# BoloniniD/CSWin-UNet

Measured on AMD Instinct MI355X. Metric: training images/sec (224x224, cswin_tiny), higher is better.
Workload: dtype f32; 1 GPU; cswin_tiny_224_lite, synthetic 224x224 9-class, bs=24/GPU, fp32 matmul, fwd + 0.4CE+0.6Dice + bwd + SGD(momentum) step, drop_path 0.2; global_batch=24, img_size=224, parallelism=dp1, hip_graph=True

## Files before the change

cswin_unet_amd/_lib.py:

```python
import ctypes
import os
from ctypes import c_char_p, c_double, c_float, c_int, c_long, c_size_t, c_void_p

import torch

_HERE = os.path.dirname(os.path.abspath(__file__))
LIB_PATH = os.path.join(_HERE, "libcswin_hip.so")

P, I, F, SZ, L, D = c_void_p, c_int, c_float, c_size_t, c_long, c_double

ABI_VERSION = 4

SIGNATURES = {
    "cswin_last_error": (c_char_p, []),
    "cswin_abi_version": (I, []),
    "cswin_device_ok": (I, []),
    "cswin_attn_fwd": (I, [P, P, P, P, P, P, I, I, I, I, P, P, I, F, F, ctypes.c_ulonglong, P, I, P]),
    "cswin_attn_bwd_workspace": (SZ, [I, I, I, I, P, P, I]),
    "cswin_attn_bwd": (I, [P, P, P, P, P, P, P, P, P, P, SZ, I, I, I, I, P, P, I, F, P, F, ctypes.c_ulonglong, P, I, P]),
    "cswin_img2windows": (I, [P, P, I, I, I, I, I, I, P]),
    "cswin_windows2img": (I, [P, P, I, I, I, I, I, I, P]),
    "cswin_layernorm_fwd": (I, [P, P, P, P, P, P, I, I, F, I, P]),
    "cswin_layernorm_bwd_workspace": (SZ, [I, I]),
    "cswin_layernorm_bwd": (I, [P, P, P, P, P, P, P, P, P, P, SZ, I, I, P, P, P]),
    "cswin_linear_fwd": (I, [P, P, I, P, P, P, P, P, P, I, I, I, I, I, I, P]),
    "cswin_linear_bwd_data": (I, [P, P, P, P, I, P, P, I, P, I, I, I, I, I, P]),
    "cswin_linear_bwd_weight_workspace": (SZ, [I, I, I]),
    "cswin_linear_bwd_weight": (I, [P, P, P, I, P, I, P, P, P, SZ, I, I, I, P, I, P]),
    "cswin_linear_bwd_weight_batch": (I, [P, I, P, P, I, P]),
    "cswin_linear_bwd_tail": (I, [P, P, P, I, I, I, P, I, P, P, I, P]),
    "cswin_rows_sum_multi": (I, [P, I, P]),
    "cswin_conv_tok_fwd": (I, [P, P, P, P, I, I, I, I, I, I, I, I, I, P]),
    "cswin_conv_tok_bwd_data": (I, [P, P, P, I, I, I, I, I, I, I, I, I, P]),
    "cswin_conv_tok_bwd_weight_workspace": (SZ, [I, I, I, I, I, I, I, I]),
    "cswin_conv_tok_bwd_weight": (I, [P, P, P, P, P, SZ, I, I, I, I, I, I, I, I, I, P, I, P]),
    "cswin_conv_weight_permute": (I, [P, P, P, I, I, I, I, P]),
    "cswin_conv_weight_unpermute": (I, [P, P, I, I, I, I, P]),
    "cswin_conv_weight_flipT": (I, [P, P, I, I, I, P]),
    "cswin_nchw_to_tokens": (I, [P, P, I, I, I, I, I, P]),
    "cswin_tokens_to_nchw": (I, [P, P, I, I, I, I, I, P]),
    "cswin_carafe_fwd": (I, [P, P, P, P, P, I, I, I, I, I, P]),
    "cswin_carafe_bwd_workspace": (SZ, [I, I, I, I, I]),
    "cswin_carafe_bwd": (I, [P, P, P, P, P, P, P, SZ, I, I, I, I, I, P, P]),
    "cswin_loss_workspace": (SZ, [I, I, L]),
    "cswin_loss_sums": (I, [P, P, P, P, SZ, I, I, L, I, P]),
    "cswin_loss_finalize": (I, [P, P, P, D, I, F, F, P, P]),
    "cswin_loss_bwd": (I, [P, P, P, P, P, F, F, I, I, L, I, P]),
    "cswin_dropout": (I, [P, P, P, P, L, L, F, ctypes.c_ulonglong, P, P]),
    "cswin_sgd_flat": (I, [P, P, P, L, P, F, F, F, P, P]),
    "cswin_multi_copy": (I, [P, I, P]),
    "cswin_pack_bf16": (I, [P, P, L, P]),
    "cswin_pack_bf16_scaled": (I, [P, P, L, F, P]),
    "cswin_unpack_bf16": (I, [P, P, L, P]),
}



class WgradDesc(ctypes.Structure):
    _fields_ = [("dy", c_void_p), ("x", c_void_p), ("row_scale", c_void_p), ("dw", c_void_p), ("dbias", c_void_p),
                ("workspace", c_void_p), ("ws_bytes", c_size_t), ("rows_per_sample", c_int), ("M", c_int), ("N", c_int),
                ("K", c_int), ("precision", c_int), ("io_bf16", c_int)]


class ReduceJob(ctypes.Structure):
    _fields_ = [("part", c_void_p), ("out", c_void_p), ("out2", c_void_p), ("n_first", ctypes.c_longlong),
                ("n", ctypes.c_longlong), ("stride", ctypes.c_longlong), ("rows", c_int), ("reserved", c_int),
                ("conv_kk", c_int), ("conv_cin", c_int)]


_lib = None

PREC_FP32, PREC_BF16 = 0, 1
_state = {"precision": PREC_FP32, "act_bf16": True}


def precision():
    return _state["precision"]


def act_bf16():
    return _state["precision"] == PREC_BF16 and _state["act_bf16"]


def set_act_bf16(on):
    prev = _state["act_bf16"]
    _state["act_bf16"] = bool(on)
    return prev


_shadows = []


class _Shadow:

    def __init__(self, owner_obj, owner, seen):
        import weakref
        self.ref = weakref.ref(owner_obj)
        self.base, self.nbytes, self.seen = owner.data_ptr(), owner.numel() * 4, seen


def register_shadow(owner_obj, owner):
    _shadows[:] = [e for e in _shadows if e.ref() is not None and e.base != owner.data_ptr()]
    _shadows.append(_Shadow(owner_obj, owner, {p.data_ptr(): p._version for p in owner_obj.params}))


def shadow_ptr(w):
    if not _shadows or w is None:
        return None
    a = w.data_ptr()
    for e in _shadows:
        if e.base <= a < e.base + e.nbytes:
            opt = e.ref()
            if opt is None:
                return None
            if e.seen.get(a) != w._version:
                opt.refresh_shadow()
                e.seen.clear()
                e.seen.update({p.data_ptr(): p._version for p in opt.params})
                e.seen[a] = w._version
            return c_void_p(opt.flat_param16.data_ptr() + (a - e.base) // 2)
    return None


def shadows_current(opt):
    if _state["precision"] != PREC_BF16:
        return
    for e in _shadows:
        if e.ref() is opt:
            if any(e.seen.get(p.data_ptr()) != p._version for p in opt.params):
                opt.refresh_shadow()
                e.seen.clear()
                e.seen.update({p.data_ptr(): p._version for p in opt.params})
            return


def set_precision(mode):
    prev = _state["precision"]
    _state["precision"] = int(mode)
    if int(mode) == PREC_BF16 and prev != PREC_BF16:
        for e in _shadows:
            opt = e.ref()
            if opt is not None:
                opt.refresh_shadow()
    return prev


class CswinHipError(RuntimeError):
    pass


def lib():
    global _lib
    if _lib is None:
        if not os.path.exists(LIB_PATH):
            raise CswinHipError(f"{LIB_PATH} not found: build it with `python -c 'import __graft_entry__ as g; g.build()'` "
                                f"(or `make -C cswin_unet_amd/csrc`). There is no fallback path.")
        handle = ctypes.CDLL(LIB_PATH)
        for name, (res, args) in SIGNATURES.items():
            try:
                fn = getattr(handle, name)
            except AttributeError as e:
                raise CswinHipError(f"{LIB_PATH} does not export {name}") from e
            fn.restype, fn.argtypes = res, args
        have = handle.cswin_abi_version()
        if have != ABI_VERSION:
            raise CswinHipError(f"{LIB_PATH} was built for C ABI version {have}, this package binds version {ABI_VERSION}: rebuild it "
                                f"(`make -C cswin_unet_amd/csrc`)")
        _lib = handle
    return _lib


def call(name, *args):
    h = lib()
    rc = getattr(h, name)(*args)
    if rc != 0:
        raise CswinHipError(f"{name} failed ({rc}): {h.cswin_last_error().decode()}")


def ptr(t):
    return None if t is None else c_void_p(t.data_ptr())


def stream():
    return c_void_p(torch.cuda.current_stream().cuda_stream)


def dev_f32(t, what="tensor"):
    if t is None:
        return None
    if not t.is_cuda:
        raise CswinHipError(f"{what} is on {t.device}: the cswin_unet_amd ops run on a HIP device only (no CPU fallback)")
    if t.dtype != torch.float32:
        raise CswinHipError(f"{what} has dtype {t.dtype}; the HIP path computes in fp32")
    return t if t.is_contiguous() else t.contiguous()
```

cswin_unet_amd/csrc/carafe.hip:

```cpp
#include "common.h"
#include <stdlib.h>

namespace {

__host__ __device__ inline int carafe_lpr(int Cz) {
    int l = 1;
    while (2 * l <= Cz / 4 && 2 * l <= 64) l *= 2;
    return l;
}

template <int S>
__global__ __launch_bounds__(256) void carafe_fwd_kernel(const float* __restrict__ e, const float* __restrict__ z,
                                                          const float* __restrict__ bias, float* __restrict__ out,
                                                          float* __restrict__ wt_save, int B, int H, int W, int Cz) {
    constexpr int S2 = S * S;
    const int lpr = carafe_lpr(Cz);
    const int groups = 256 / lpr;
    const int sub = threadIdx.x % lpr, grp = threadIdx.x / lpr;
    const long items = (long)B * H * W * S2;
    for (long it = (long)blockIdx.x * groups + grp; it < items; it += (long)gridDim.x * groups) {
        const int s = (int)(it % S2);
        const long pix = it / S2;
        const int w = (int)(pix % W);
        const int h = (int)((pix / W) % H);
        const int b = (int)(pix / ((long)W * H));
        float wt[9];
        float mx = -INFINITY;
#pragma unroll
        for (int k = 0; k < 9; ++k) {
            wt[k] = e[pix * (9 * S2) + k * S2 + s];
            mx = fmaxf(mx, wt[k]);
        }
        float sum = 0.f;
#pragma unroll
        for (int k = 0; k < 9; ++k) {
            wt[k] = __expf(wt[k] - mx);
            sum += wt[k];
        }
        const float inv = 1.0f / sum;
#pragma unroll
        for (int k = 0; k < 9; ++k) wt[k] *= inv;
        if (wt_save && sub == 0) {
#pragma unroll
            for (int k = 0; k < 9; ++k) wt_save[pix * (9 * S2) + k * S2 + s] = wt[k];
        }
        const int sy = s / S, sx = s - sy * S;
        const long orow = ((long)b * H * S + h * S + sy) * (W * S) + w * S + sx;
        for (int c = 4 * sub; c < Cz; c += 4 * lpr) {
            f32x4 acc = bias ? *reinterpret_cast<const f32x4*>(bias + c) : f32x4{0.f, 0.f, 0.f, 0.f};
#pragma unroll
            for (int k = 0; k < 9; ++k) {
                const int hh = h + k / 3 - 1, ww = w + k % 3 - 1;
                if ((unsigned)hh < (unsigned)H && (unsigned)ww < (unsigned)W)
                    acc += wt[k] * *reinterpret_cast<const f32x4*>(z + (((long)b * H + hh) * W + ww) * Cz + c);
            }
            *reinterpret_cast<f32x4*>(out + orow * Cz + c) = acc;
        }
    }
}

template <int S>
__global__ __launch_bounds__(256) void carafe_bwd_e_kernel(const float* __restrict__ dout, const float* __restrict__ z,
                                                            const float* __restrict__ wt_save, float* __restrict__ de,
                                                            float* __restrict__ dbias_part, int B, int H, int W, int Cz) {
    __shared__ float bred[2 * 1024];
    f32x4 bacc[2] = {{0.f, 0.f, 0.f, 0.f}, {0.f, 0.f, 0.f, 0.f}};
    constexpr int S2 = S * S;
    const int lpr = carafe_lpr(Cz);
    const int groups = 256 / lpr;
    const int sub = threadIdx.x % lpr, grp = threadIdx.x / lpr;
    const long items = (long)B * H * W * S2;
    const long items_pad = (items + groups - 1) / groups * groups;
    for (long it0 = (long)blockIdx.x * groups + grp; it0 < items_pad; it0 += (long)gridDim.x * groups) {
        const bool live = it0 < items;
        const long it = live ? it0 : items - 1;
        const int s = (int)(it % S2);
        const long pix = it / S2;
        const int w = (int)(pix % W);
        const int h = (int)((pix / W) % H);
        const int b = (int)(pix / ((long)W * H));
        const int sy = s / S, sx = s - sy * S;
        const long orow = ((long)b * H * S + h * S + sy) * (W * S) + w * S + sx;
        float dwt[9];
#pragma unroll
        for (int k = 0; k < 9; ++k) dwt[k] = 0.f;
        int ci = 0;
        for (int c = 4 * sub; c < Cz; c += 4 * lpr, ++ci) {
            const f32x4 g = *reinterpret_cast<const f32x4*>(dout + orow * Cz + c);
            if (live && dbias_part) {
                if (ci == 0) bacc[0] += g;
                else bacc[1] += g;
            }
#pragma unroll
            for (int k = 0; k < 9; ++k) {
                const int hh = h + k / 3 - 1, ww = w + k % 3 - 1;
                if ((unsigned)hh < (unsigned)H && (unsigned)ww < (unsigned)W) {
                    const f32x4 zv = *reinterpret_cast<const f32x4*>(z + (((long)b * H + hh) * W + ww) * Cz + c);
                    dwt[k] += g[0] * zv[0] + g[1] * zv[1] + g[2] * zv[2] + g[3] * zv[3];
                }
            }
        }
#pragma unroll
        for (int k = 0; k < 9; ++k)
            for (int o = lpr >> 1; o > 0; o >>= 1) dwt[k] += __shfl_xor(dwt[k], o, 64);
        if (sub == 0 && live) {
            float wt[9], dot = 0.f;
#pragma unroll
            for (int k = 0; k < 9; ++k) {
                wt[k] = wt_save[pix * (9 * S2) + k * S2 + s];
                dot += wt[k] * dwt[k];
            }
#pragma unroll
            for (int k = 0; k < 9; ++k) de[pix * (9 * S2) + k * S2 + s] = wt[k] * (dwt[k] - dot);
        }
    }
    if (dbias_part) {
        const int span = 4 * lpr;
#pragma unroll
        for (int q = 0; q < 2; ++q)
#pragma unroll
            for (int e = 0; e < 4; ++e) bred[(q * groups + grp) * span + 4 * sub + e] = bacc[q][e];
        __syncthreads();
        for (int c = threadIdx.x; c < Cz; c += 256) {
            const int q = c / span, cc = c - q * span;
            float t = 0.f;
            for (int g2 = 0; g2 < groups; ++g2) t += bred[(q * groups + g2) * span + cc];
            dbias_part[(long)blockIdx.x * Cz + c] = t;
        }
    }
}

template <int S>
__global__ __launch_bounds__(256) void carafe_bwd_z_kernel(const float* __restrict__ dout,
                                                            const float* __restrict__ wt_save, float* __restrict__ dz,
                                                            int B, int H, int W, int Cz) {
    constexpr int S2 = S * S;
    const int lpr = carafe_lpr(Cz);
    const int groups = 256 / lpr;
    const int sub = threadIdx.x % lpr, grp = threadIdx.x / lpr;
    const long items = (long)B * H * W;
    for (long pix = (long)blockIdx.x * groups + grp; pix < items; pix += (long)gridDim.x * groups) {
        const int w = (int)(pix % W);
        const int h = (int)((pix / W) % H);
        const int b = (int)(pix / ((long)W * H));
        for (int c = 4 * sub; c < Cz; c += 4 * lpr) {
            f32x4 acc = {0.f, 0.f, 0.f, 0.f};
#pragma unroll
            for (int k = 0; k < 9; ++k) {
                const int h2 = h - (k / 3 - 1), w2 = w - (k % 3 - 1);
                if ((unsigned)h2 < (unsigned)H && (unsigned)w2 < (unsigned)W) {
                    const long p2 = ((long)b * H + h2) * W + w2;
#pragma unroll
                    for (int s = 0; s < S2; ++s) {
                        const float wv = wt_save[p2 * (9 * S2) + k * S2 + s];
                        const long orow = ((long)b * H * S + h2 * S + s / S) * (W * S) + w2 * S + s % S;
                        acc += wv * *reinterpret_cast<const f32x4*>(dout + orow * Cz + c);
                    }
                }
            }
            *reinterpret_cast<f32x4*>(dz + pix * Cz + c) = acc;
        }
    }
}

constexpr int C4_T = 8;
constexpr int C4_HALO = C4_T + 2;
constexpr int C4_NP = C4_HALO * C4_HALO;

__device__ __forceinline__ f32x4 carafe_mfma4(float a, float b, f32x4 c) { return __builtin_amdgcn_mfma_f32_16x16x4f32(a, b, c, 0, 0, 0); }

constexpr int C4_WAVES = 8;

__global__ __launch_bounds__(64 * C4_WAVES) void carafe4_bwd_fused_kernel(const float* __restrict__ dout, const float* __restrict__ z,
                                                                 const float* __restrict__ wt_save, float* __restrict__ de,
                                                                 float* __restrict__ dz, float* __restrict__ dbias_part,
                                                                 int B, int H, int W, int tiles_x, int tiles_y) {
    constexpr int S = 4, S2 = 16, Cz = 16;
    __shared__ __attribute__((aligned(16))) float Gs[C4_NP * 9 * Cz];
    __shared__ __attribute__((aligned(16))) float zt[C4_NP * Cz];
    __shared__ float bred[C4_WAVES][Cz];
    const int tid = threadIdx.x, lane = tid & 63, wave = tid >> 6;
    const int li = lane & 15, kq = lane >> 4;
    int t = blockIdx.x;
    const int tx = t % tiles_x; t /= tiles_x;
    const int ty = t % tiles_y;
    const int b = t / tiles_y;
    const int h0 = ty * C4_T - 1, w0 = tx * C4_T - 1;

    for (int i = tid; i < C4_NP * (Cz / 4); i += 64 * C4_WAVES) {
        const int pl = i >> 2, c4 = i & 3;
        const int h = h0 + pl / C4_HALO, w = w0 + pl % C4_HALO;
        f32x4 v = {0.f, 0.f, 0.f, 0.f};
        if ((unsigned)h < (unsigned)H && (unsigned)w < (unsigned)W)
            v = *reinterpret_cast<const f32x4*>(z + (((long)b * H + h) * W + w) * Cz + 4 * c4);
        *reinterpret_cast<f32x4*>(&zt[pl * Cz + 4 * c4]) = v;
    }
    __syncthreads();

    float bsum = 0.f;
    constexpr int PB = 4;
    for (int pl0 = wave * PB; pl0 < C4_NP; pl0 += C4_WAVES * PB) {
        bool inside[PB], interior[PB];
        long pix[PB];
        float av[PB][4], dv[PB][4], wv[PB][4];
        f32x4 db[PB];
#pragma unroll
        for (int u = 0; u < PB; ++u) {
            const int pl = pl0 + u;
            const int ph = pl / C4_HALO, pw = pl - ph * C4_HALO;
            const int h = h0 + ph, w = w0 + pw;
            inside[u] = pl < C4_NP && (unsigned)h < (unsigned)H && (unsigned)w < (unsigned)W;
            interior[u] = inside[u] && ph >= 1 && ph <= C4_T && pw >= 1 && pw <= C4_T;
            pix[u] = ((long)b * H + h) * W + w;
            db[u] = f32x4{0.f, 0.f, 0.f, 0.f};
#pragma unroll
            for (int j = 0; j < 4; ++j) av[u][j] = dv[u][j] = wv[u][j] = 0.f;
            if (!inside[u]) continue;
            const float* wp = wt_save + pix[u] * (9 * S2);
            const float* drow = dout + (((long)b * H * S + h * S) * (W * S) + w * S) * Cz;
            const long hstride = (long)W * S * Cz;
#pragma unroll
            for (int j = 0; j < 4; ++j) {
                if (li < 9) av[u][j] = wp[li * S2 + 4 * j + kq];
                dv[u][j] = drow[j * hstride + kq * Cz + li];
            }
            if (interior[u]) {
                db[u] = *reinterpret_cast<const f32x4*>(drow + (li >> 2) * hstride + (li & 3) * Cz + 4 * kq);
#pragma unroll
                for (int r = 0; r < 4; ++r)
                    if (4 * kq + r < 9) wv[u][r] = wp[(4 * kq + r) * S2 + li];
            }
        }
#pragma unroll
        for (int u = 0; u < PB; ++u) {
            const int pl = pl0 + u;
            if (pl >= C4_NP) continue;
            float* Gp = &Gs[pl * 9 * Cz];
            if (!inside[u]) {
                for (int i = lane; i < 9 * Cz; i += 64) Gp[i] = 0.f;
                continue;
            }
            f32x4 g = {0.f, 0.f, 0.f, 0.f};
#pragma unroll
            for (int j = 0; j < 4; ++j) g = carafe_mfma4(av[u][j], dv[u][j], g);
#pragma unroll
            for (int r = 0; r < 4; ++r)
                if (4 * kq + r < 9) Gp[(4 * kq + r) * Cz + li] = g[r];
            if (!interior[u]) continue;
            bsum += dv[u][0] + dv[u][1] + dv[u][2] + dv[u][3];
            const int ph = pl / C4_HALO, pw = pl - ph * C4_HALO;
            f32x4 za = {0.f, 0.f, 0.f, 0.f};
            if (li < 9) {
                const int nh = ph + li / 3 - 1, nw = pw + li % 3 - 1;
                za = *reinterpret_cast<const f32x4*>(&zt[(nh * C4_HALO + nw) * Cz + 4 * kq]);
            }
            f32x4 dw = {0.f, 0.f, 0.f, 0.f};
#pragma unroll
            for (int j = 0; j < 4; ++j) dw = carafe_mfma4(za[j], db[u][j], dw);
            float dot = 0.f;
#pragma unroll
            for (int r = 0; r < 4; ++r) dot += wv[u][r] * dw[r];
            dot += __shfl_xor(dot, 16, 64);
            dot += __shfl_xor(dot, 32, 64);
            float* dep = de + pix[u] * (9 * S2);
#pragma unroll
            for (int r = 0; r < 4; ++r)
                if (4 * kq + r < 9) dep[(4 * kq + r) * S2 + li] = wv[u][r] * (dw[r] - dot);
        }
    }
    bsum += __shfl_xor(bsum, 16, 64);
    bsum += __shfl_xor(bsum, 32, 64);
    if (lane < Cz) bred[wave][lane] = bsum;
    __syncthreads();
    if (tid < Cz && dbias_part) {
        float t2 = 0.f;
#pragma unroll
        for (int k = 0; k < C4_WAVES; ++k) t2 += bred[k][tid];
        dbias_part[(long)blockIdx.x * Cz + tid] = t2;
    }

    if (tid < 256) {
        const int n = tid >> 2, c4 = tid & 3;
        const int ph = 1 + n / C4_T, pw = 1 + n % C4_T;
        const int h = h0 + ph, w = w0 + pw;
        if (h < H && w < W) {
            f32x4 acc = {0.f, 0.f, 0.f, 0.f};
#pragma unroll
            for (int k = 0; k < 9; ++k) {
                const int sh = ph - (k / 3 - 1), sw = pw - (k % 3 - 1);
                acc += *reinterpret_cast<const f32x4*>(&Gs[((sh * C4_HALO + sw) * 9 + k) * Cz + 4 * c4]);
            }
            *reinterpret_cast<f32x4*>(dz + (((long)b * H + h) * W + w) * Cz + 4 * c4) = acc;
        }
    }
}

__global__ __launch_bounds__(256) void colsum_partial_kernel(const float* __restrict__ x, float* __restrict__ partial,
                                                              long rows, int C) {
    __shared__ float red[256];
    const int lanes = min(C, 256);
    const int rgroups = 256 / lanes;
    const int c0 = threadIdx.x % lanes, rg = threadIdx.x / lanes;
    for (int c = c0; c < C; c += lanes) {
        float s = 0.f;
        if (rg < rgroups)
            for (long r = (long)blockIdx.x * rgroups + rg; r < rows; r += (long)gridDim.x * rgroups) s += x[r * C + c];
        red[threadIdx.x] = s;
        __syncthreads();
        if (rg == 0) {
            float t = 0.f;
            for (int k = 0; k < rgroups; ++k) t += red[k * lanes + c0];
            partial[(long)blockIdx.x * C + c] = t;
        }
        __syncthreads();
    }
}

int colsum_blocks(long rows, int C) {
    int lanes = C < 256 ? C : 256;
    int rg = 256 / lanes;
    long b = (rows + rg * 64 - 1) / (rg * 64);
    return (int)(b < 1 ? 1 : (b > 512 ? 512 : b));
}

int grid_for(long items, int groups) {
    long b = (items + groups - 1) / groups;
    return (int)(b < 1 ? 1 : (b > 8192 ? 8192 : b));
}

bool carafe_args_ok(int B, int H, int W, int Cz, int S) {
    if (B <= 0 || H <= 0 || W <= 0 || Cz <= 0 || (S != 2 && S != 4)) return false;
    return Cz % 4 == 0 && Cz >= 4;
}

}

extern "C" {

int cswin_carafe_fwd(const float* e, const float* z, const float* bias, float* out, float* wt_save, int B, int H, int W,
                     int Cz, int S, void* stream) {
    CSWIN_REQUIRE(e && z && out, CSWIN_ERR_SHAPE, "carafe_fwd: null pointer");
    CSWIN_REQUIRE(carafe_args_ok(B, H, W, Cz, S), CSWIN_ERR_UNSUPPORTED, "carafe_fwd: unsupported shape B=%d H=%d W=%d Cz=%d S=%d (Cz %% 4 == 0, S in {2,4})", B, H, W, Cz, S);
    const int groups = 256 / carafe_lpr(Cz);
    hipStream_t st = (hipStream_t)stream;
    const long items = (long)B * H * W * S * S;
    if (S == 2) hipLaunchKernelGGL(carafe_fwd_kernel<2>, dim3(grid_for(items, groups)), dim3(256), 0, st, e, z, bias, out, wt_save, B, H, W, Cz);
    else hipLaunchKernelGGL(carafe_fwd_kernel<4>, dim3(grid_for(items, groups)), dim3(256), 0, st, e, z, bias, out, wt_save, B, H, W, Cz);
    CSWIN_LAUNCH_CHECK();
    return CSWIN_OK;
}

static bool carafe4_fused_ok(int H, int W, int Cz, int S) { return S == 4 && Cz == 16 && H % C4_T == 0 && W % C4_T == 0; }

size_t cswin_carafe_bwd_workspace(int B, int H, int W, int Cz, int S) {
    size_t generic = (size_t)colsum_blocks((long)B * H * W * S * S, Cz) * Cz * sizeof(float);
    size_t in_e = Cz <= 512 ? (size_t)grid_for((long)B * H * W * S * S, 256 / carafe_lpr(Cz)) * Cz * sizeof(float) : 0;
    if (in_e > generic) generic = in_e;
    size_t fused = carafe4_fused_ok(H, W, Cz, S) ? (size_t)B * (H / C4_T) * (W / C4_T) * Cz * sizeof(float) : 0;
    return generic > fused ? generic : fused;
}

int cswin_carafe_bwd(const float* dout, const float* z, const float* wt_save, float* de, float* dz, float* dbias,
                     void* workspace, size_t ws_bytes, int B, int H, int W, int Cz, int S, cswin_reduce_job* deferred, void* stream) {
    if (deferred) *deferred = cswin_reduce_job{};
    CSWIN_REQUIRE(dout && z && wt_save && de && dz, CSWIN_ERR_SHAPE, "carafe_bwd: null pointer");
    CSWIN_REQUIRE(carafe_args_ok(B, H, W, Cz, S), CSWIN_ERR_UNSUPPORTED, "carafe_bwd: unsupported shape");
    CSWIN_REQUIRE(!dbias || (workspace && ws_bytes >= cswin_carafe_bwd_workspace(B, H, W, Cz, S)), CSWIN_ERR_WORKSPACE, "carafe_bwd: workspace too small");
    const int groups = 256 / carafe_lpr(Cz);
    hipStream_t st = (hipStream_t)stream;
    const long items = (long)B * H * W * S * S, pixels = (long)B * H * W;
    const bool no_fused = cswin_tuning().carafe_generic != 0;
    if (carafe4_fused_ok(H, W, Cz, S) && !no_fused) {
        const int tx = W / C4_T, ty = H / C4_T, nblk = B * tx * ty;
        hipLaunchKernelGGL(carafe4_bwd_fused_kernel, dim3(nblk), dim3(64 * C4_WAVES), 0, st, dout, z, wt_save, de, dz,
                           dbias ? (float*)workspace : nullptr, B, H, W, tx, ty);
        CSWIN_LAUNCH_CHECK();
        if (dbias) {
            reduce_now_or_defer(cswin_reduce_job{(const float*)workspace, dbias, nullptr, 0, Cz, Cz, nblk, 0, 0, 0}, deferred, st);
            CSWIN_LAUNCH_CHECK();
        }
        return CSWIN_OK;
    }
    const bool bias_in_e = dbias && Cz <= 512;
    float* bpart = bias_in_e ? (float*)workspace : nullptr;
    const int eblk = grid_for(items, groups);
    if (S == 2) {
        hipLaunchKernelGGL(carafe_bwd_e_kernel<2>, dim3(eblk), dim3(256), 0, st, dout, z, wt_save, de, bpart, B, H, W, Cz);
        hipLaunchKernelGGL(carafe_bwd_z_kernel<2>, dim3(grid_for(pixels, groups)), dim3(256), 0, st, dout, wt_save, dz, B, H, W, Cz);
    } else {
        hipLaunchKernelGGL(carafe_bwd_e_kernel<4>, dim3(eblk), dim3(256), 0, st, dout, z, wt_save, de, bpart, B, H, W, Cz);
        hipLaunchKernelGGL(carafe_bwd_z_kernel<4>, dim3(grid_for(pixels, groups)), dim3(256), 0, st, dout, wt_save, dz, B, H, W, Cz);
    }
    CSWIN_LAUNCH_CHECK();
    if (bias_in_e) {
        reduce_now_or_defer(cswin_reduce_job{(const float*)workspace, dbias, nullptr, 0, Cz, Cz, eblk, 0, 0, 0}, deferred, st);
        CSWIN_LAUNCH_CHECK();
    } else if (dbias) {
        int nblk = colsum_blocks(items, Cz);
        hipLaunchKernelGGL(colsum_partial_kernel, dim3(nblk), dim3(256), 0, st, dout, (float*)workspace, items, Cz);
        reduce_now_or_defer(cswin_reduce_job{(const float*)workspace, dbias, nullptr, 0, Cz, Cz, nblk, 0, 0, 0}, deferred, st);
        CSWIN_LAUNCH_CHECK();
    }
    return CSWIN_OK;
}

}
```

cswin_unet_amd/csrc/common.h:

```cpp
#pragma once
#include "tuning.h"
#include <hip/hip_runtime.h>
#include <stddef.h>
#include <stdint.h>
#include <stdio.h>

typedef float f32x4 __attribute__((ext_vector_type(4)));
typedef unsigned u32x2 __attribute__((ext_vector_type(2)));
typedef unsigned u32x4 __attribute__((ext_vector_type(4)));
typedef float f32x16 __attribute__((ext_vector_type(16)));

#define CSWIN_ABI_VERSION 4
#define CSWIN_OK 0
#define CSWIN_ERR_SHAPE (-1)
#define CSWIN_ERR_ALIGN (-2)
#define CSWIN_ERR_WORKSPACE (-3)
#define CSWIN_ERR_HIP (-4)
#define CSWIN_ERR_UNSUPPORTED (-5)

void cswin_set_error(const char* fmt, ...);

#define CSWIN_REQUIRE(cond, code, ...)          \
    do {                                        \
        if (!(cond)) {                          \
            cswin_set_error(__VA_ARGS__);       \
            return (code);                      \
        }                                       \
    } while (0)

#define CSWIN_LAUNCH_CHECK()                                                   \
    do {                                                                       \
        hipError_t e__ = hipGetLastError();                                    \
        if (e__ != hipSuccess) {                                               \
            cswin_set_error("%s:%d HIP launch error: %s", __FILE__, __LINE__,  \
                            hipGetErrorString(e__));                           \
            return CSWIN_ERR_HIP;                                              \
        }                                                                      \
    } while (0)

static inline int cdiv(long a, long b) { return (int)((a + b - 1) / b); }

__device__ __forceinline__ float wave_sum(float v) {
#pragma unroll
    for (int o = 32; o > 0; o >>= 1) v += __shfl_xor(v, o, 64);
    return v;
}
__device__ __forceinline__ float wave_max(float v) {
#pragma unroll
    for (int o = 32; o > 0; o >>= 1) v = fmaxf(v, __shfl_xor(v, o, 64));
    return v;
}

__device__ __forceinline__ void gelu_parts(float x, float& cdf, float& e) {
    const float u = fabsf(x) * 0.70710678118654752f;
    const float t = __builtin_amdgcn_rcpf(fmaf(0.3275911f, u, 1.0f));
    e = __expf(-u * u);
    const float poly = t * fmaf(t, fmaf(t, fmaf(t, fmaf(t, 1.061405429f, -1.453152027f), 1.421413741f), -0.284496736f), 0.254829592f);
    const float pe = poly * e;
    cdf = x < 0.f ? 0.5f * pe : fmaf(-0.5f, pe, 1.0f);
}
__device__ __forceinline__ float gelu_f(float x) {
    float cdf, e;
    gelu_parts(x, cdf, e);
    return x * cdf;
}
__device__ __forceinline__ float gelu_grad_f(float x) {
    float cdf, e;
    gelu_parts(x, cdf, e);
    return fmaf(x * 0.3989422804014327f, e, cdf);
}

extern "C" {
typedef struct cswin_reduce_job {
    const float* part;
    float* out;
    float* out2;
    long long n_first, n, stride;
    int rows, reserved;
    int conv_kk, conv_cin;
} cswin_reduce_job;
}

static inline int reduce_job_vec_ok(const cswin_reduce_job& j) {
    return ((uintptr_t)j.part % 16 == 0) && j.stride % 4 == 0 && j.n % 4 == 0 && (!j.out2 || j.n_first % 4 == 0);
}

constexpr int RS_COLS = 64, RS_G = 16;
__device__ __forceinline__ void rows_sum_block(const cswin_reduce_job& job, long blk, float (*red)[RS_COLS + 1]) {
    const int c4 = threadIdx.x & 15, g = threadIdx.x >> 4;
    const long i0 = blk * RS_COLS + 4 * c4;
    f32x4 s0 = {0.f, 0.f, 0.f, 0.f}, s1 = s0, s2 = s0, s3 = s0;
    if (i0 < job.n) {
        const float* base = job.part + i0;
        if (job.reserved & 1) {
            int r = g;
            for (; r + 3 * RS_G < job.rows; r += 4 * RS_G) {
                s0 += *reinterpret_cast<const f32x4*>(base + (long)r * job.stride);
                s1 += *reinterpret_cast<const f32x4*>(base + (long)(r + RS_G) * job.stride);
                s2 += *reinterpret_cast<const f32x4*>(base + (long)(r + 2 * RS_G) * job.stride);
                s3 += *reinterpret_cast<const f32x4*>(base + (long)(r + 3 * RS_G) * job.stride);
            }
            for (; r < job.rows; r += RS_G) s0 += *reinterpret_cast<const f32x4*>(base + (long)r * job.stride);
        } else {
            for (int r = g; r < job.rows; r += RS_G)
#pragma unroll
                for (int e = 0; e < 4; ++e)
                    if (i0 + e < job.n) s0[e] += base[(long)r * job.stride + e];
        }
    }
    s0 = (s0 + s1) + (s2 + s3);
#pragma unroll
    for (int e = 0; e < 4; ++e) red[g][4 * c4 + e] = s0[e];
    __syncthreads();
    const long i = blk * RS_COLS + threadIdx.x;
    if (threadIdx.x < RS_COLS && i < job.n) {
        float t = 0.f;
#pragma unroll
        for (int k = 0; k < RS_G; ++k) t += red[k][threadIdx.x];
        if (job.out2 && i >= job.n_first) job.out2[i - job.n_first] = t;
        else job.out[i] = t;
    }
}

__device__ __forceinline__ void rows_sum_conv_block(const cswin_reduce_job& j, long blk, float (*red)[RS_COLS + 1]) {
    const int kk = j.conv_kk, Cin = j.conv_cin;
    float* out = j.out;
    const int c4 = threadIdx.x & 15, g = threadIdx.x >> 4;
    const long i0 = blk * RS_COLS + 4 * c4;
    f32x4 s0 = {0.f, 0.f, 0.f, 0.f}, s1 = s0;
    if (i0 < j.n) {
        const float* base = j.part + i0;
        if (j.reserved & 1) {
            int r = g;
            for (; r + RS_G < j.rows; r += 2 * RS_G) {
                s0 += *reinterpret_cast<const f32x4*>(base + (long)r * j.stride);
                s1 += *reinterpret_cast<const f32x4*>(base + (long)(r + RS_G) * j.stride);
            }
            for (; r < j.rows; r += RS_G) s0 += *reinterpret_cast<const f32x4*>(base + (long)r * j.stride);
        } else {
            for (int r = g; r < j.rows; r += RS_G)
#pragma unroll
                for (int e = 0; e < 4; ++e)
                    if (i0 + e < j.n) s0[e] += base[(long)r * j.stride + e];
        }
    }
    s0 += s1;
#pragma unroll
    for (int e = 0; e < 4; ++e) red[g][4 * c4 + e] = s0[e];
    __syncthreads();
    const long i = blk * RS_COLS + threadIdx.x;
    if (threadIdx.x < RS_COLS && i < j.n) {
        float t = 0.f;
#pragma unroll
        for (int k = 0; k < RS_G; ++k) t += red[k][threadIdx.x];
        if (j.out2 && i >= j.n_first) j.out2[i - j.n_first] = t;
        else if (i < j.n_first) {
            const long co = i / ((long)kk * Cin);
            const int rem = (int)(i - co * kk * Cin), tap = rem / Cin, ci = rem - tap * Cin;
            out[(co * Cin + ci) * kk + tap] = t;
        }
    }
}

extern "C" {
typedef struct cswin_wgrad_desc {
    const float* dy;
    const float* x;
    const float* row_scale;
    float* dw;
    float* dbias;
    void* workspace;
    size_t ws_bytes;
    int rows_per_sample, M, N, K;
    int precision;
    int io_bf16;
} cswin_wgrad_desc;
}

constexpr int CSWIN_MAX_REDUCE_JOBS = 48;
struct ReduceJobs {
    cswin_reduce_job j[CSWIN_MAX_REDUCE_JOBS];
    int first_block[CSWIN_MAX_REDUCE_JOBS + 1];
    int njobs;
};

constexpr int RS_FEW_ROWS = 16, RS_FEW_COLS = 1024;
__device__ __forceinline__ void rows_sum_few(const cswin_reduce_job& job, long blk) {
    const long i0 = blk * RS_FEW_COLS + 4 * threadIdx.x;
    if (i0 >= job.n) return;
    const float* base = job.part + i0;
    f32x4 s0 = {0.f, 0.f, 0.f, 0.f}, s1 = s0;
    int r = 0;
    for (; r + 1 < job.rows; r += 2) {
        s0 += *reinterpret_cast<const f32x4*>(base + (long)r * job.stride);
        s1 += *reinterpret_cast<const f32x4*>(base + (long)(r + 1) * job.stride);
    }
    if (r < job.rows) s0 += *reinterpret_cast<const f32x4*>(base + (long)r * job.stride);
    s0 += s1;
    if (job.out2 && i0 >= job.n_first) *reinterpret_cast<f32x4*>(job.out2 + (i0 - job.n_first)) = s0;
    else *reinterpret_cast<f32x4*>(job.out + i0) = s0;
}
static inline int reduce_job_few_ok(const cswin_reduce_job& j) {
    return !j.conv_kk && reduce_job_vec_ok(j) && j.rows <= RS_FEW_ROWS && j.n >= 4 * RS_FEW_COLS && ((uintptr_t)j.out % 16 == 0) &&
           (!j.out2 || ((uintptr_t)j.out2 % 16 == 0));
}

static __global__ __launch_bounds__(256) void rows_sum_kernel(cswin_reduce_job job) {
    __shared__ float red[RS_G][RS_COLS + 1];
    if (job.conv_kk) rows_sum_conv_block(job, blockIdx.x, red);
    else if (job.reserved & 2) rows_sum_few(job, blockIdx.x);
    else rows_sum_block(job, blockIdx.x, red);
}

static inline void launch_rows_sum(const float* part, float* out, float* out2, long n_first, long n, int rows, long stride,
                                   hipStream_t st) {
    cswin_reduce_job job = {part, out, out2, n_first, n, stride, rows, 0, 0, 0};
    const int few = reduce_job_few_ok(job);
    job.reserved = reduce_job_vec_ok(job) | (few ? 2 : 0);
    const long cols = few ? RS_FEW_COLS : RS_COLS;
    hipLaunchKernelGGL(rows_sum_kernel, dim3((unsigned)((n + cols - 1) / cols)), dim3(256), 0, st, job);
}

__device__ __forceinline__ void rows_sum_dispatch(const cswin_reduce_job* j, const int* first_block, int njobs, int blk,
                                                  float (*red)[RS_COLS + 1]) {
    int lo = 0, hi = njobs - 1;
    while (lo < hi) {
        const int mid = (lo + hi + 1) >> 1;
        if (blk >= first_block[mid]) lo = mid;
        else hi = mid - 1;
    }
    const int k = lo;
    if (j[k].conv_kk) rows_sum_conv_block(j[k], blk - first_block[k], red);
    else if (j[k].reserved & 2) rows_sum_few(j[k], blk - first_block[k]);
    else rows_sum_block(j[k], blk - first_block[k], red);
}

static __global__ __launch_bounds__(256) void rows_sum_multi_kernel(ReduceJobs J) {
    __shared__ float red[RS_G][RS_COLS + 1];
    rows_sum_dispatch(J.j, J.first_block, J.njobs, (int)blockIdx.x, red);
}

constexpr int CSWIN_TAIL_RIDER_JOBS = 16;
struct ReduceRiders {
    cswin_reduce_job j[CSWIN_TAIL_RIDER_JOBS];
    int first_block[CSWIN_TAIL_RIDER_JOBS + 1];
    int njobs;
};
static inline int fill_reduce_table(const cswin_reduce_job* jobs, int njobs, cswin_reduce_job* out, int* first_block) {
    int blocks = 0;
    for (int i = 0; i < njobs; ++i) {
        if (!(jobs[i].part && jobs[i].out && jobs[i].n > 0 && jobs[i].rows > 0)) return -1;
        if ((jobs[i].conv_kk == 0) != (jobs[i].conv_cin == 0) || jobs[i].conv_kk < 0) return -1;
        out[i] = jobs[i];
        const int few = reduce_job_few_ok(jobs[i]);
        out[i].reserved = reduce_job_vec_ok(jobs[i]) | (few ? 2 : 0);
        first_block[i] = blocks;
        blocks += few ? (int)((jobs[i].n + RS_FEW_COLS - 1) / RS_FEW_COLS) : (int)((jobs[i].n + RS_COLS - 1) / RS_COLS);
    }
    first_block[njobs] = blocks;
    return blocks;
}

static inline void reduce_now_or_defer(const cswin_reduce_job& job, cswin_reduce_job* deferred, hipStream_t st) {
    if (deferred) *deferred = job;
    else launch_rows_sum(job.part, job.out, job.out2, (long)job.n_first, (long)job.n, job.rows, (long)job.stride, st);
}
```

cswin_unet_amd/csrc/gemm.hip:

```cpp
#include <stdlib.h>

#include <type_traits>
#include "common.h"
#include "gemm_epilogue.h"

int cswin_gemm16(int mode, int epi_mode, const void* A, const void* B, const void* epilogue, int M, int NO, int R, void* stream);
int cswin_wgrad16_batch(const cswin_wgrad_desc* d, int n, const int* splits, const int* rows_per_split, const cswin_reduce_job* pending,
                        int npending, void* stream, long long* stamps);

namespace {

constexpr int BKMAX = 64;

typedef __bf16 bf16x8 __attribute__((ext_vector_type(8)));
typedef __bf16 bf16x4 __attribute__((ext_vector_type(4)));

#define CSWIN_CHECK_PRECISION(p, who) CSWIN_REQUIRE((p) == 0 || (p) == 1, CSWIN_ERR_UNSUPPORTED, who ": precision %d (0 = fp32, 1 = bf16 operands)", (p))

struct PlainSrc {
    const float* p; long ld; int rows, cols;
    const float* row_scale; int rows_per_sample;
    int bf16;
    struct Row { const float* base; float s; };
    __device__ Row row(int i) const {
// ... 709 lines not shown
    choose_split(M, N, K, &s0, &rps);
    choose_split(M, N, K, &s1, &rps, 1024);
    return (size_t)(s0 > s1 ? s0 : s1) * ((size_t)N * K + N) * sizeof(float);
}

int cswin_linear_bwd_weight_batch(const cswin_wgrad_desc* d, int n, cswin_reduce_job* deferred, const cswin_reduce_job* pending, int npending,
                                  void* stream);
int cswin_rows_sum_multi(const cswin_reduce_job* jobs, int njobs, void* stream);
}
namespace {
struct TailExtras { const float* dy; const float* w; float* dx; int M, N, K; const cswin_reduce_job* jobs; int njobs; };
int wgrad_batch_impl(const cswin_wgrad_desc* d, int n, cswin_reduce_job* deferred, const TailExtras* extra, void* stream);
}
extern "C" {

int cswin_linear_bwd_weight(const float* dy, const float* x, const float* x2, int k_split, const float* row_scale,
                            int rows_per_sample, float* dw, float* dbias, void* workspace, size_t ws_bytes, int M,
                            int N, int K, cswin_reduce_job* deferred, int precision, void* stream) {
    CSWIN_CHECK_PRECISION(precision, "linear_bwd_weight");
    CSWIN_REQUIRE(dy && x && dw && M > 0 && N > 0 && K > 0, CSWIN_ERR_SHAPE, "linear_bwd_weight: bad arguments");
    CSWIN_REQUIRE(!x2 || (k_split > 0 && k_split < K), CSWIN_ERR_SHAPE, "linear_bwd_weight: bad concat split");
    CSWIN_REQUIRE(!row_scale || rows_per_sample > 0, CSWIN_ERR_SHAPE, "linear_bwd_weight: rows_per_sample must be > 0");
    size_t need = cswin_linear_bwd_weight_workspace(M, N, K);
    CSWIN_REQUIRE(workspace && ws_bytes >= need, CSWIN_ERR_WORKSPACE, "linear_bwd_weight: workspace %zu < %zu", ws_bytes, need);
    hipStream_t st = (hipStream_t)stream;
    if (precision == 1 && !x2 && N % 4 == 0 && K % 4 == 0 && aligned16(dy) && aligned16(x) && aligned16(workspace)) {
        cswin_wgrad_desc d1 = {dy, x, row_scale, dw, dbias, workspace, ws_bytes, rows_per_sample, M, N, K, 1, 0};
        cswin_reduce_job job;
        int rc = cswin_linear_bwd_weight_batch(&d1, 1, &job, nullptr, 0, stream);
        if (rc) return rc;
        reduce_now_or_defer(job, deferred, st);
        CSWIN_LAUNCH_CHECK();
        return CSWIN_OK;
    }
    int splits, rps;
    choose_split(M, N, K, &splits, &rps);
    float* slab = (float*)workspace;
    const long slab_stride = (long)N * K + N;
    Epilogue e = plain_epilogue(slab, K);
    e.split_stride = slab_stride;
    e.colsum = dbias ? slab + (long)N * K : nullptr;
    e.colsum_stride = (int)slab_stride;
    PlainSrc A = {dy, N, M, N, row_scale, rows_per_sample};
    if (x2) {
        ConcatSrc B = {x, x2, k_split, K - k_split, M, K, k_split};
        bool vec = (N % 4 == 0) && (K % 4 == 0) && (k_split % 4 == 0) && aligned16(dy) && aligned16(x) && aligned16(x2);
        if (vec) launch_gemm<false, false, 4, EPI_PLAIN, true>(A, B, e, N, K, M, splits, rps, precision, st);
        else launch_gemm<false, false, 1, EPI_PLAIN, true>(A, B, e, N, K, M, splits, rps, precision, st);
    } else {
        PlainSrc B = {x, K, M, K, nullptr, 1};
        bool vec = (N % 4 == 0) && (K % 4 == 0) && aligned16(dy) && aligned16(x);
        if (row_scale) {
            if (vec) launch_gemm<false, false, 4, EPI_PLAIN, true>(A, B, e, N, K, M, splits, rps, precision, st);
            else launch_gemm<false, false, 1, EPI_PLAIN, true>(A, B, e, N, K, M, splits, rps, precision, st);
        } else {
            if (vec) launch_gemm<false, false, 4, EPI_PLAIN, false>(A, B, e, N, K, M, splits, rps, precision, st);
            else launch_gemm<false, false, 1, EPI_PLAIN, false>(A, B, e, N, K, M, splits, rps, precision, st);
        }
    }
    CSWIN_LAUNCH_CHECK();
    long n = (long)N * K;
    cswin_reduce_job job = {slab, dw, dbias, n, n + (dbias ? N : 0), slab_stride, splits, 0};
    reduce_now_or_defer(job, deferred, st);
    CSWIN_LAUNCH_CHECK();
    return CSWIN_OK;
}

int cswin_linear_bwd_weight_batch(const cswin_wgrad_desc* d, int n, cswin_reduce_job* deferred, const cswin_reduce_job* pending, int npending,
                                  void* stream) {
    CSWIN_REQUIRE(npending >= 0 && npending <= CSWIN_TAIL_RIDER_JOBS && (npending == 0 || pending), CSWIN_ERR_SHAPE,
                  "linear_bwd_weight_batch: 0..%d pending reductions", CSWIN_TAIL_RIDER_JOBS);
    TailExtras r = {nullptr, nullptr, nullptr, 0, 0, 0, pending, npending};
    return wgrad_batch_impl(d, n, deferred, npending > 0 ? &r : nullptr, stream);
}

int cswin_linear_bwd_tail(const float* dy, const float* w, float* dx, int M, int N, int K, const cswin_wgrad_desc* d, int n,
                          cswin_reduce_job* deferred, const cswin_reduce_job* pending, int npending, void* stream) {
    CSWIN_REQUIRE(dy && w && dx && M > 0 && N > 0 && K > 0, CSWIN_ERR_SHAPE, "linear_bwd_tail: bad data-gradient arguments");
    CSWIN_REQUIRE(npending >= 0 && npending <= CSWIN_TAIL_RIDER_JOBS && (npending == 0 || pending), CSWIN_ERR_SHAPE,
                  "linear_bwd_tail: 0..%d pending reductions", CSWIN_TAIL_RIDER_JOBS);
    TailExtras r = {dy, w, dx, M, N, K, pending, npending};
    return wgrad_batch_impl(d, n, deferred, &r, stream);
}

}
namespace {
int wgrad_batch_impl(const cswin_wgrad_desc* d, int n, cswin_reduce_job* deferred, const TailExtras* extra, void* stream) {
    CSWIN_REQUIRE(d && deferred && n >= 1 && n <= WGRAD_BATCH, CSWIN_ERR_SHAPE, "linear_bwd_weight_batch: 1..%d problems and their deferred slots", WGRAD_BATCH);
    bool fast = true;
    const int precision = d[0].precision;
    CSWIN_CHECK_PRECISION(precision, "linear_bwd_weight_batch");
    for (int i = 0; i < n; ++i) {
        CSWIN_REQUIRE(d[i].precision == precision, CSWIN_ERR_UNSUPPORTED, "linear_bwd_weight_batch: problems of one launch share one precision");
        CSWIN_REQUIRE(d[i].io_bf16 == 0 || (precision == 1 && (d[i].io_bf16 & ~3) == 0), CSWIN_ERR_UNSUPPORTED, "linear_bwd_weight_batch: bf16 storage needs precision 1");
        CSWIN_REQUIRE(d[i].dy && d[i].x && d[i].dw && d[i].M > 0 && d[i].N > 0 && d[i].K > 0, CSWIN_ERR_SHAPE, "linear_bwd_weight_batch: bad problem %d", i);
        CSWIN_REQUIRE(!d[i].row_scale || d[i].rows_per_sample > 0, CSWIN_ERR_SHAPE, "linear_bwd_weight_batch: rows_per_sample must be > 0");
        size_t need = cswin_linear_bwd_weight_workspace(d[i].M, d[i].N, d[i].K);
        CSWIN_REQUIRE(d[i].workspace && d[i].ws_bytes >= need, CSWIN_ERR_WORKSPACE, "linear_bwd_weight_batch: workspace %zu < %zu", d[i].ws_bytes, need);
        fast = fast && d[i].N % 4 == 0 && d[i].K % 4 == 0 && aligned16(d[i].dy) && aligned16(d[i].x) && aligned16(d[i].workspace);
    }
    const bool has_dgrad = extra && extra->dy;
    const bool merge_on = cswin_tuning().gemm_tail_merge != 0;
    const bool ride = extra && merge_on && fast && precision == 0 &&
                      (!has_dgrad || (extra->N % 4 == 0 && extra->K % 4 == 0 && aligned16(extra->dy) && aligned16(extra->w) && aligned16(extra->dx)));
    const bool w16_path = fast && precision == 1 && (cswin_tuning().wgrad16_on || d[0].io_bf16 || (n > 1 && d[1].io_bf16) || (n > 2 && d[2].io_bf16) || (n > 3 && d[3].io_bf16));
    const bool jobs_ride16 = extra && merge_on && w16_path && extra->njobs > 0;
    if (extra && !ride) {
        if (has_dgrad) {
            int rc = cswin_linear_bwd_data(extra->dy, extra->w, extra->dx, nullptr, 0, nullptr, nullptr, 1, nullptr, extra->M, extra->N,
                                           extra->K, precision == 1 ? 1 : 0, 0, stream);
            if (rc) return rc;
        }
        if (extra->njobs > 0 && !jobs_ride16) {
            int rc = cswin_rows_sum_multi(extra->jobs, extra->njobs, stream);
            if (rc) return rc;
        }
    }
    if (!fast) {
        for (int i = 0; i < n; ++i) CSWIN_REQUIRE(d[i].io_bf16 == 0, CSWIN_ERR_ALIGN, "linear_bwd_weight_batch: bf16 storage needs N, K multiples of 4 and 16-B alignment");
        for (int i = 0; i < n; ++i) {
            int rc = cswin_linear_bwd_weight(d[i].dy, d[i].x, nullptr, 0, d[i].row_scale, d[i].rows_per_sample, d[i].dw, d[i].dbias,
                                             d[i].workspace, d[i].ws_bytes, d[i].M, d[i].N, d[i].K, &deferred[i], precision, stream);
            if (rc) return rc;
        }
        return CSWIN_OK;
    }
    if (w16_path) {
        int splits[WGRAD_BATCH], rps[WGRAD_BATCH];
        double work_total = 0.0;
        for (int i = 0; i < n; ++i) work_total += (double)d[i].M * cdiv(d[i].N, 128) * cdiv(d[i].K, 128);
        for (int i = 0; i < n; ++i) {
            const int M = d[i].M, N = d[i].N, K = d[i].K;
            const long slab = ((long)N * K + N) * (long)sizeof(float);
            const int tiles = cdiv(N, 128) * cdiv(K, 128);
            const int w16_wgs = cswin_tuning().w16_wgs, w16_even = cswin_tuning().w16_even;
            int s = w16_even ? (w16_wgs / n) / tiles : (int)(w16_wgs * ((double)M * tiles / work_total) / tiles + 0.5);
            const int cap = (int)(d[i].ws_bytes / slab);
            if (s > cap) s = cap;
            if (s > M / 64) s = M / 64;
            if (s < 1) s = 1;
            rps[i] = cdiv(cdiv(M, s), 32) * 32;
            splits[i] = cdiv(M, rps[i]);
            const long nk = (long)N * K;
            deferred[i] = cswin_reduce_job{(const float*)d[i].workspace, d[i].dw, d[i].dbias, nk, nk + (d[i].dbias ? N : 0), nk + N, splits[i], 0};
        }
        CSWIN_REQUIRE(cswin_wgrad16_batch(d, n, splits, rps, jobs_ride16 ? extra->jobs : nullptr, jobs_ride16 ? extra->njobs : 0, stream, g_stamps) == 0,
                      CSWIN_ERR_SHAPE, "linear_bwd_weight_batch: bad pending reduction");
        CSWIN_LAUNCH_CHECK();
        return CSWIN_OK;
    }
    WgradBatch b = {};
    int blocks = 0;
    for (int i = 0; i < n; ++i) {
        const int M = d[i].M, N = d[i].N, K = d[i].K;
        int splits, rps;
        const int batch_env = cswin_tuning().gemm_batch_wgs;
        const int batch_even = cswin_tuning().gemm_batch_even;
        const int total_wgs = batch_env > 0 ? (batch_env < 1024 ? batch_env : 1024) * n : 1024;
        int batch_target = total_wgs / n;
        if (!batch_even) {
            double work = 0.0;
            for (int j = 0; j < n; ++j) work += (double)d[j].M * cdiv(d[j].N, 64) * cdiv(d[j].K, 64);
            batch_target = (int)(total_wgs * ((double)M * cdiv(N, 64) * cdiv(K, 64) / work) + 0.5);
            if (batch_target > 1024) batch_target = 1024;
            if (batch_target < 1) batch_target = 1;
        }
        choose_split(M, N, K, &splits, &rps, batch_target);
        CSWIN_REQUIRE((size_t)splits * ((size_t)N * K + N) * sizeof(float) <= d[i].ws_bytes, CSWIN_ERR_WORKSPACE,
                      "linear_bwd_weight_batch: %d slabs do not fit problem %d's workspace", splits, i);
        float* slab = (float*)d[i].workspace;
        const long slab_stride = (long)N * K + N;
        Epilogue e = plain_epilogue(slab, K);
        e.split_stride = slab_stride;
        e.colsum = d[i].dbias ? slab + (long)N * K : nullptr;
        e.colsum_stride = (int)slab_stride;
        e.vec_store = epilogue_vec_ok(e, K);
        b.A[i] = PlainSrc{d[i].dy, N, M, N, d[i].row_scale, d[i].row_scale ? d[i].rows_per_sample : 1};
        b.B[i] = PlainSrc{d[i].x, K, M, K, nullptr, 1};
        b.e[i] = e;
        b.M[i] = N; b.N[i] = K; b.R[i] = M; b.rps[i] = rps;
        b.tm[i] = cdiv(N, 64); b.tn[i] = cdiv(K, 64);
        b.first[i] = blocks;
        blocks += b.tm[i] * b.tn[i] * splits;
        const long nk = (long)N * K;
        deferred[i] = cswin_reduce_job{slab, d[i].dw, d[i].dbias, nk, nk + (d[i].dbias ? N : 0), slab_stride, splits, 0};
    }
    b.first[n] = blocks;
    b.n = n;
    if (ride) {
        BlockTail t = {};
        if (has_dgrad) {
            Epilogue e = plain_epilogue(extra->dx, extra->K);
            e.vec_store = epilogue_vec_ok(e, extra->K);
            t.dA = PlainSrc{extra->dy, extra->N, extra->M, extra->N, nullptr, 1, 0};
            t.dB = PlainSrc{extra->w, extra->K, extra->N, extra->K, nullptr, 1, 0};
            t.de = e;
            t.dM = extra->M; t.dN = extra->K; t.dR = extra->N; t.drps = cdiv(extra->N, BKMAX) * BKMAX;
            t.dtm = cdiv(extra->M, 64); t.dtn = cdiv(extra->K, 64);
            t.nd = t.dtm * t.dtn;
        }
        t.w = b;
        int rblocks = 0;
        if (extra->njobs > 0) {
            rblocks = fill_reduce_table(extra->jobs, extra->njobs, t.r.j, t.r.first_block);
            CSWIN_REQUIRE(rblocks >= 0, CSWIN_ERR_SHAPE, "linear_bwd_tail: bad pending reduction");
            t.r.njobs = extra->njobs;
        }
        static_assert(sizeof(BlockTail) <= 4096, "kernel argument block");
        hipLaunchKernelGGL(gemm_block_tail_kernel, dim3(blocks + t.nd + rblocks), dim3(512), 0, (hipStream_t)stream, t);
    } else if (precision == 1) {
        hipLaunchKernelGGL(gemm_wgrad_batch_kernel<1>, dim3(blocks), dim3(512), 0, (hipStream_t)stream, b);
    } else {
        hipLaunchKernelGGL(gemm_wgrad_batch_kernel<0>, dim3(blocks), dim3(512), 0, (hipStream_t)stream, b);
    }
    CSWIN_LAUNCH_CHECK();
    return CSWIN_OK;
}
}
extern "C" {

int cswin_conv_tok_fwd(const float* x, const float* w_perm, const float* bias, float* y, int B, int H, int W, int Cin,
                       int Cout, int ks, int stride, int pad, int precision, void* stream) {
    CSWIN_CHECK_PRECISION(precision, "conv_tok_fwd");
    CSWIN_REQUIRE(x && w_perm && y && B > 0 && H > 0 && W > 0 && Cin > 0 && Cout > 0, CSWIN_ERR_SHAPE, "conv_tok_fwd: bad arguments");
    CSWIN_REQUIRE(Cin % 4 == 0 && aligned16(x) && aligned16(w_perm), CSWIN_ERR_ALIGN, "conv_tok_fwd: Cin %% 4 and 16-B alignment required");
    int OH = (H + 2 * pad - ks) / stride + 1, OW = (W + 2 * pad - ks) / stride + 1;
    int M = B * OH * OW, R = ks * ks * Cin;
    ConvSrc A = {x, B, H, W, Cin, OH, OW, ks, stride, pad, M, R};
    PlainSrc Bm = {w_perm, R, Cout, R, nullptr, 1};
    Epilogue e = plain_epilogue(y, Cout);
    e.bias = bias;
    launch_gemm<true, true, 4, EPI_PLAIN, false>(A, Bm, e, M, Cout, R, 1, cdiv(R, BKMAX) * BKMAX, precision, (hipStream_t)stream);
    CSWIN_LAUNCH_CHECK();
    return CSWIN_OK;
}

int cswin_conv_tok_bwd_data(const float* dy, const float* w_permT, float* dx, int B, int H, int W, int Cin, int Cout,
                            int ks, int stride, int pad, int precision, void* stream) {
    CSWIN_CHECK_PRECISION(precision, "conv_tok_bwd_data");
    CSWIN_REQUIRE(dy && w_permT && dx, CSWIN_ERR_SHAPE, "conv_tok_bwd_data: null pointer");
    CSWIN_REQUIRE(Cin % 4 == 0 && Cout % 4 == 0 && aligned16(dy) && aligned16(w_permT), CSWIN_ERR_ALIGN, "conv_tok_bwd_data: channels %% 4 and 16-B alignment required");
    int OH = (H + 2 * pad - ks) / stride + 1, OW = (W + 2 * pad - ks) / stride + 1;
    if (ks == 3 && stride == 2 && pad == 1) {
        GemmBatch<ConvTS2Src, TapRowsSrc> b = {};
        int blocks = 0, n = 0, rmax = 0;
        for (int py = 0; py < 2; ++py)
            for (int px = 0; px < 2; ++px) {
                const int H2 = (H - py + 1) / 2, W2 = (W - px + 1) / 2;
                if (H2 <= 0 || W2 <= 0) continue;
                int kys = 0, kxs = 0, taps = 0, nt = 0;
                for (int ky = (py ? 0 : 1); ky < 3; ky += 2)
                    for (int kx = (px ? 0 : 1); kx < 3; kx += 2) {
                        kys |= ky << (2 * nt);
                        kxs |= kx << (2 * nt);
                        taps |= (ky * 3 + kx) << (4 * nt);
                        ++nt;
                    }
                const int Mc = B * H2 * W2, Rc = nt * Cout;
                b.A[n] = ConvTS2Src{dy, B, H, W, Cout, OH, OW, py, px, H2, W2, kys, kxs, Mc, Rc};
                b.B[n] = TapRowsSrc{w_permT, Cout, Cin, taps, Rc, Cin};
                Epilogue e = plain_epilogue(dx, Cin);
                e.rm_on = 1; e.rm_H = H; e.rm_W = W; e.rm_H2 = H2; e.rm_W2 = W2; e.rm_py = py; e.rm_px = px;
                e.vec_store = epilogue_vec_ok(e, Cin);
                b.e[n] = e;
                b.M[n] = Mc; b.N[n] = Cin; b.R[n] = Rc; b.rps[n] = cdiv(Rc, BKMAX) * BKMAX;
                b.tm[n] = cdiv(Mc, 64); b.tn[n] = cdiv(Cin, 64);
                b.first[n] = blocks;
                blocks += b.tm[n] * b.tn[n];
                rmax = Rc > rmax ? Rc : rmax;
                ++n;
            }
        if (n > 0) {
            b.first[n] = blocks;
            b.n = n;
            hipStream_t st = (hipStream_t)stream;
            const int kw = (blocks < 320 && rmax >= 512) ? 4 : ((blocks < 640 && rmax >= 256) ? 2 : 1);
            if (precision == 1) {
                hipLaunchKernelGGL((gemm_conv_s2_dgrad_batch_kernel<2, 1>), dim3(blocks), dim3(512), 0, st, b);
            } else if (kw == 4) {
                hipLaunchKernelGGL((gemm_conv_s2_dgrad_batch_kernel<4, 0>), dim3(blocks), dim3(1024), 0, st, b);
            } else if (kw == 2) {
                hipLaunchKernelGGL((gemm_conv_s2_dgrad_batch_kernel<2, 0>), dim3(blocks), dim3(512), 0, st, b);
            } else {
                hipLaunchKernelGGL((gemm_conv_s2_dgrad_batch_kernel<1, 0>), dim3(blocks), dim3(256), 0, st, b);
            }
        }
        CSWIN_LAUNCH_CHECK();
        return CSWIN_OK;
    }
    int M = B * H * W, R = ks * ks * Cout;
    ConvTSrc A = {dy, B, H, W, Cout, OH, OW, ks, stride, pad, M, R};
    PlainSrc Bm = {w_permT, Cin, R, Cin, nullptr, 1};
    Epilogue e = plain_epilogue(dx, Cin);
    launch_gemm<true, false, 4, EPI_PLAIN, false>(A, Bm, e, M, Cin, R, 1, cdiv(R, BKMAX) * BKMAX, precision, (hipStream_t)stream);
    CSWIN_LAUNCH_CHECK();
    return CSWIN_OK;
}

size_t cswin_conv_tok_bwd_weight_workspace(int B, int H, int W, int Cin, int Cout, int ks, int stride, int pad) {
    int OH = (H + 2 * pad - ks) / stride + 1, OW = (W + 2 * pad - ks) / stride + 1;
    return cswin_linear_bwd_weight_workspace(B * OH * OW, Cout, ks * ks * Cin);
}

int cswin_conv_tok_bwd_weight(const float* dy, const float* x, float* dw_perm, float* dbias, void* workspace,
                              size_t ws_bytes, int B, int H, int W, int Cin, int Cout, int ks, int stride, int pad,
                              int torch_layout, cswin_reduce_job* deferred, int precision, void* stream) {
    CSWIN_CHECK_PRECISION(precision, "conv_tok_bwd_weight");
    CSWIN_REQUIRE(dy && x && dw_perm, CSWIN_ERR_SHAPE, "conv_tok_bwd_weight: null pointer");
    CSWIN_REQUIRE(Cin % 4 == 0 && Cout % 4 == 0 && aligned16(dy) && aligned16(x), CSWIN_ERR_ALIGN, "conv_tok_bwd_weight: channels %% 4 and 16-B alignment required");
    int OH = (H + 2 * pad - ks) / stride + 1, OW = (W + 2 * pad - ks) / stride + 1;
    int M = B * OH * OW, K = ks * ks * Cin;
    size_t need = cswin_linear_bwd_weight_workspace(M, Cout, K);
    CSWIN_REQUIRE(workspace && ws_bytes >= need, CSWIN_ERR_WORKSPACE, "conv_tok_bwd_weight: workspace %zu < %zu", ws_bytes, need);
    hipStream_t st = (hipStream_t)stream;
    int splits, rps;
    choose_split(M, Cout, K, &splits, &rps);
    float* slab = (float*)workspace;
    const long slab_stride = (long)Cout * K + Cout;
    Epilogue e = plain_epilogue(slab, K);
    e.split_stride = slab_stride;
    e.colsum = dbias ? slab + (long)Cout * K : nullptr;
    e.colsum_stride = (int)slab_stride;
    PlainSrc A = {dy, Cout, M, Cout, nullptr, 1};
    ConvSrc Bm = {x, B, H, W, Cin, OH, OW, ks, stride, pad, M, K};
    launch_gemm<false, false, 4, EPI_PLAIN, false>(A, Bm, e, Cout, K, M, splits, rps, precision, st);
    CSWIN_LAUNCH_CHECK();
    long n = (long)Cout * K;
    cswin_reduce_job job = {slab, dw_perm, dbias, n, n + (dbias ? Cout : 0), slab_stride, splits, 0, torch_layout ? ks * ks : 0, torch_layout ? Cin : 0};
    if (deferred) {
        *deferred = job;
        return CSWIN_OK;
    }
    if (torch_layout) {
        job.reserved = reduce_job_vec_ok(job);
        hipLaunchKernelGGL(rows_sum_kernel, dim3((unsigned)((job.n + RS_COLS - 1) / RS_COLS)), dim3(256), 0, st, job);
    } else {
        launch_rows_sum(slab, dw_perm, dbias, n, n + (dbias ? Cout : 0), splits, slab_stride, st);
    }
    CSWIN_LAUNCH_CHECK();
    return CSWIN_OK;
}

int cswin_rows_sum_multi(const cswin_reduce_job* jobs, int njobs, void* stream) {
    CSWIN_REQUIRE(jobs && njobs > 0 && njobs <= CSWIN_MAX_REDUCE_JOBS, CSWIN_ERR_SHAPE, "rows_sum_multi: 1..%d jobs", CSWIN_MAX_REDUCE_JOBS);
    ReduceJobs J = {};
    const int blocks = fill_reduce_table(jobs, njobs, J.j, J.first_block);
    CSWIN_REQUIRE(blocks >= 0, CSWIN_ERR_SHAPE, "rows_sum_multi: bad job (part / out / n / rows, or conv_kk without conv_cin)");
    J.njobs = njobs;
    hipLaunchKernelGGL(rows_sum_multi_kernel, dim3(blocks), dim3(256), 0, (hipStream_t)stream, J);
    CSWIN_LAUNCH_CHECK();
    return CSWIN_OK;
}

}
```

cswin_unet_amd/csrc/layout.hip:

```cpp
#include "common.h"

namespace {

__global__ void nchw_to_tok_kernel(const float* __restrict__ x, float* __restrict__ y, int B, int C, long HW, int Cpad) {
    const long total = (long)B * HW * Cpad;
    for (long o = (long)blockIdx.x * blockDim.x + threadIdx.x; o < total; o += (long)gridDim.x * blockDim.x) {
        const int c = (int)(o % Cpad);
        const long bp = o / Cpad;
        const long p = bp % HW, b = bp / HW;
        y[o] = c < C ? x[(b * C + c) * HW + p] : 0.f;
    }
}

__global__ __launch_bounds__(256) void tok_to_nchw_kernel(const float* __restrict__ x, float* __restrict__ y, int B, int C,
                                                           long HW, int Cpad) {
    __shared__ float tile[64][17];
    const long ptiles = (HW + 63) / 64;
    for (long t = blockIdx.x; t < (long)B * ptiles; t += gridDim.x) {
        const long b = t / ptiles, p0 = (t % ptiles) * 64;
        for (int c0 = 0; c0 < C; c0 += 16) {
            for (int i = threadIdx.x; i < 64 * 16; i += 256) {
                const int pp = i / 16, cc = i % 16;
                tile[pp][cc] = (p0 + pp < HW && c0 + cc < Cpad) ? x[(b * HW + p0 + pp) * Cpad + c0 + cc] : 0.f;
            }
            __syncthreads();
            for (int i = threadIdx.x; i < 64 * 16; i += 256) {
                const int cc = i / 64, pp = i % 64;
                if (p0 + pp < HW && c0 + cc < C) y[(b * C + c0 + cc) * HW + p0 + pp] = tile[pp][cc];
            }
            __syncthreads();
        }
    }
}

__global__ void conv_w_permute_kernel(const float* __restrict__ w, float* __restrict__ wp, float* __restrict__ wpt,
                                      int Cout, int Cin, int kk, int Cpad) {
    const long total = (long)Cout * kk * Cpad;
    for (long o = (long)blockIdx.x * blockDim.x + threadIdx.x; o < total; o += (long)gridDim.x * blockDim.x) {
        const int ci = (int)(o % Cpad);
        const int tap = (int)((o / Cpad) % kk);
        const int co = (int)(o / ((long)Cpad * kk));
        const float v = ci < Cin ? w[((long)co * Cin + ci) * kk + tap] : 0.f;
        if (wp) wp[o] = v;
        if (wpt) wpt[((long)tap * Cout + co) * Cpad + ci] = v;
    }
}

__global__ void conv_w_unpermute_kernel(const float* __restrict__ dwp, float* __restrict__ dw, int Cout, int Cin, int kk,
                                        int Cpad) {
    const long total = (long)Cout * Cin * kk;
    for (long o = (long)blockIdx.x * blockDim.x + threadIdx.x; o < total; o += (long)gridDim.x * blockDim.x) {
        const int tap = (int)(o % kk);
        const int ci = (int)((o / kk) % Cin);
        const int co = (int)(o / ((long)kk * Cin));
        dw[o] = dwp[((long)co * kk + tap) * Cpad + ci];
    }
}

__global__ void conv_w_flipT_kernel(const float* __restrict__ w, float* __restrict__ wf, int Cout, int Cin, int kk) {
    const long total = (long)Cin * kk * Cout;
    for (long o = (long)blockIdx.x * blockDim.x + threadIdx.x; o < total; o += (long)gridDim.x * blockDim.x) {
        const int co = (int)(o % Cout);
        const int tap = (int)((o / Cout) % kk);
        const int ci = (int)(o / ((long)Cout * kk));
        wf[o] = w[((long)co * Cin + ci) * kk + (kk - 1 - tap)];
    }
}

int grid1d(long total) {
    long b = (total + 255) / 256;
    return (int)(b < 1 ? 1 : (b > 4096 ? 4096 : b));
}

__device__ __forceinline__ unsigned long long mix64(unsigned long long z) {
    z += 0x9E3779B97F4A7C15ull;
    z = (z ^ (z >> 30)) * 0xBF58476D1CE4E5B9ull;
    z = (z ^ (z >> 27)) * 0x94D049BB133111EBull;
    return z ^ (z >> 31);
}

__global__ __launch_bounds__(256) void dropout_kernel(const float* __restrict__ x, const float* __restrict__ residual,
                                                       const float* __restrict__ row_scale, float* __restrict__ y, long n,
                                                       long elems_per_sample, float p, unsigned long long seed,
                                                       const unsigned long long* __restrict__ epoch) {
    if (epoch) seed += *epoch;
    const unsigned thr = (unsigned)(p * 65536.0f);
    const float inv_keep = 1.0f / (1.0f - p);
    const long n4 = n / 4;
    for (long i = (long)blockIdx.x * 256 + threadIdx.x; i < n4; i += (long)gridDim.x * 256) {
        const unsigned long long r = mix64(mix64(seed) ^ (unsigned long long)i);
        const f32x4 xv = reinterpret_cast<const f32x4*>(x)[i];
        f32x4 o = residual ? reinterpret_cast<const f32x4*>(residual)[i] : f32x4{0.f, 0.f, 0.f, 0.f};
        const float rs = (row_scale ? row_scale[(4 * i) / elems_per_sample] : 1.0f) * inv_keep;
#pragma unroll
        for (int e = 0; e < 4; ++e) o[e] += (((unsigned)(r >> (16 * e)) & 0xFFFFu) >= thr) ? rs * xv[e] : 0.f;
        reinterpret_cast<f32x4*>(y)[i] = o;
    }
}

}

extern "C" {

int cswin_dropout(const float* x, const float* residual, const float* row_scale, float* y, long n, long elems_per_sample,
                  float p, unsigned long long seed, const unsigned long long* seed_epoch, void* stream) {
    CSWIN_REQUIRE(x && y && n > 0 && n % 4 == 0 && elems_per_sample > 0 && elems_per_sample % 4 == 0, CSWIN_ERR_SHAPE,
                  "dropout: n and elems_per_sample must be positive multiples of 4");
    CSWIN_REQUIRE(p >= 0.f && p < 1.f, CSWIN_ERR_SHAPE, "dropout: p = %f outside [0, 1)", p);
    CSWIN_REQUIRE(((((uintptr_t)x) | ((uintptr_t)y) | ((uintptr_t)residual)) & 15) == 0, CSWIN_ERR_ALIGN, "dropout: 16-B alignment required");
    long b = (n / 4 + 255) / 256;
    hipLaunchKernelGGL(dropout_kernel, dim3((int)(b > 8192 ? 8192 : b)), dim3(256), 0, (hipStream_t)stream, x, residual, row_scale, y, n,
                       elems_per_sample, p, seed, seed_epoch);
    CSWIN_LAUNCH_CHECK();
    return CSWIN_OK;
}


int cswin_nchw_to_tokens(const float* x, float* y, int B, int C, int H, int W, int Cpad, void* stream) {
    CSWIN_REQUIRE(x && y && B > 0 && C > 0 && Cpad >= C && H > 0 && W > 0, CSWIN_ERR_SHAPE, "nchw_to_tokens: bad arguments");
    hipLaunchKernelGGL(nchw_to_tok_kernel, dim3(grid1d((long)B * H * W * Cpad)), dim3(256), 0, (hipStream_t)stream, x, y, B, C, (long)H * W, Cpad);
    CSWIN_LAUNCH_CHECK();
    return CSWIN_OK;
}

int cswin_tokens_to_nchw(const float* x, float* y, int B, int C, int H, int W, int Cpad, void* stream) {
    CSWIN_REQUIRE(x && y && B > 0 && C > 0 && Cpad >= C && H > 0 && W > 0, CSWIN_ERR_SHAPE, "tokens_to_nchw: bad arguments");
    long tiles = (long)B * (((long)H * W + 63) / 64);
    hipLaunchKernelGGL(tok_to_nchw_kernel, dim3((int)(tiles > 8192 ? 8192 : tiles)), dim3(256), 0, (hipStream_t)stream, x, y, B, C, (long)H * W, Cpad);
    CSWIN_LAUNCH_CHECK();
    return CSWIN_OK;
}

int cswin_conv_weight_permute(const float* w, float* w_perm, float* w_permT, int Cout, int Cin, int ks, int Cpad, void* stream) {
    CSWIN_REQUIRE(w && (w_perm || w_permT) && Cout > 0 && Cin > 0 && ks > 0 && Cpad >= Cin, CSWIN_ERR_SHAPE, "conv_weight_permute: bad arguments");
    hipLaunchKernelGGL(conv_w_permute_kernel, dim3(grid1d((long)Cout * ks * ks * Cpad)), dim3(256), 0, (hipStream_t)stream, w, w_perm, w_permT, Cout, Cin, ks * ks, Cpad);
    CSWIN_LAUNCH_CHECK();
    return CSWIN_OK;
}

int cswin_conv_weight_flipT(const float* w, float* wf, int Cout, int Cin, int ks, void* stream) {
    CSWIN_REQUIRE(w && wf && Cout > 0 && Cin > 0 && ks > 0, CSWIN_ERR_SHAPE, "conv_weight_flipT: bad arguments");
    hipLaunchKernelGGL(conv_w_flipT_kernel, dim3(grid1d((long)Cout * Cin * ks * ks)), dim3(256), 0, (hipStream_t)stream, w, wf, Cout, Cin, ks * ks);
    CSWIN_LAUNCH_CHECK();
    return CSWIN_OK;
}

int cswin_conv_weight_unpermute(const float* dw_perm, float* dw, int Cout, int Cin, int ks, int Cpad, void* stream) {
    CSWIN_REQUIRE(dw_perm && dw && Cout > 0 && Cin > 0 && ks > 0 && Cpad >= Cin, CSWIN_ERR_SHAPE, "conv_weight_unpermute: bad arguments");
    hipLaunchKernelGGL(conv_w_unpermute_kernel, dim3(grid1d((long)Cout * Cin * ks * ks)), dim3(256), 0, (hipStream_t)stream, dw_perm, dw, Cout, Cin, ks * ks, Cpad);
    CSWIN_LAUNCH_CHECK();
    return CSWIN_OK;
}

}
```

cswin_unet_amd/networks/cswin_unet.py:

```python
import math

import numpy as np
import torch
import torch.nn as nn
import torch.utils.checkpoint as checkpoint

from .. import ops
from ..layers import DropPath, TokenRearrange, trunc_normal_


def _square_side(n_tokens):
    side = int(math.isqrt(n_tokens))
    if side * side != n_tokens:
        raise ValueError(f"token count {n_tokens} is not a square map")
    return side


class Mlp(nn.Module):
    def __init__(self, in_features, hidden_features=None, out_features=None, act_layer=nn.GELU, drop=0.):
        super().__init__()
        out_features = out_features or in_features
        hidden_features = hidden_features or in_features
        self.fc1 = nn.Linear(in_features, hidden_features)
        self.act = act_layer()
        self.fc2 = nn.Linear(hidden_features, out_features)
        self.drop = nn.Dropout(drop)
        if not isinstance(self.act, nn.GELU) or getattr(self.act, "approximate", "none") != "none":
            raise NotImplementedError("the HIP Mlp kernel fuses the exact (erf) GELU only")

    def forward(self, x, residual=None, row_scale=None):
        p = self.drop.p if self.training else 0.0
        return ops.mlp(x, self.fc1.weight, self.fc1.bias, self.fc2.weight, self.fc2.bias, residual, row_scale, drop_p=p)


class LePEAttention(nn.Module):

    def __init__(self, dim, resolution, idx, split_size, dim_out=None, num_heads=9, attn_drop=0., proj_drop=0.,
                 qk_scale=None):
        super().__init__()
        if idx not in (-1, 0, 1):
            raise ValueError(f"ERROR MODE {idx}")
        self.dim, self.dim_out = dim, dim_out or dim
        self.resolution, self.split_size, self.num_heads, self.idx = resolution, split_size, num_heads, idx
        self.scale = qk_scale or (dim // num_heads) ** -0.5
        self.H_sp = resolution if idx in (-1, 0) else split_size
        self.W_sp = resolution if idx in (-1, 1) else split_size
        self.get_v = nn.Conv2d(dim, dim, kernel_size=3, stride=1, padding=1, groups=dim)
        self.attn_drop = nn.Dropout(attn_drop)

    def forward(self, qkv):
        q, k, v = qkv[0], qkv[1], qkv[2]
        if q.shape[1] != self.resolution * self.resolution:
            raise AssertionError("flatten img_tokens has wrong size")
        packed = torch.cat([q, k, v], dim=-1)
        return ops.stripe_attention(packed, self.resolution, self.split_size, [self.idx], [self.num_heads],
                                    [self.get_v.weight], [self.get_v.bias], self.scale,
                                    attn_drop=self.attn_drop.p if self.training else 0.0)


class CSWinBlock(nn.Module):
    def __init__(self, dim, reso, num_heads, split_size, mlp_ratio=4., qkv_bias=False, qk_scale=None, drop=0.,
                 attn_drop=0., drop_path=0., act_layer=nn.GELU, norm_layer=nn.LayerNorm, last_stage=False):
        super().__init__()
        self.dim, self.num_heads, self.patches_resolution = dim, num_heads, reso
        self.split_size, self.mlp_ratio = split_size, mlp_ratio
        self.qkv = nn.Linear(dim, dim * 3, bias=qkv_bias)
        self.norm1 = norm_layer(dim)
        single = last_stage or reso == split_size
        self.branch_num = 1 if single else 2
        self.proj = nn.Linear(dim, dim)
        self.proj_drop = nn.Dropout(drop)
        bdim, bheads = (dim, num_heads) if single else (dim // 2, num_heads // 2)
        self.attns = nn.ModuleList(
            LePEAttention(bdim, resolution=reso, idx=(-1 if single else i), split_size=split_size, num_heads=bheads,
                          dim_out=bdim, qk_scale=qk_scale, attn_drop=attn_drop, proj_drop=drop)
            for i in range(self.branch_num))
        self.drop_path = DropPath(drop_path) if drop_path > 0. else nn.Identity()
        self.mlp = Mlp(in_features=dim, hidden_features=int(dim * mlp_ratio), out_features=dim, act_layer=act_layer,
                       drop=drop)
        self.norm2 = norm_layer(dim)

    def _keep_scales(self, x):
        dp = self.drop_path
        if isinstance(dp, DropPath) and self.training and dp.drop_prob > 0.:
            preset = getattr(self, "_dp_preset", None)
            if preset:
                return preset[0], preset[1]
            return dp.sample_scale(x.shape[0], x.device), dp.sample_scale(x.shape[0], x.device)
        return None, None

    def forward(self, x):
        B, L, C = x.shape
        if L != self.patches_resolution ** 2:
            raise AssertionError("flatten img_tokens has wrong size")
        a = self.attns
        ad = a[0].attn_drop.p if self.training else 0.0
        if type(self.norm1) is not nn.LayerNorm or type(self.norm2) is not nn.LayerNorm:
            raise NotImplementedError("the HIP block fuses nn.LayerNorm only")
        rs1, rs2 = self._keep_scales(x)
        if self.training and (self.proj_drop.p > 0 or self.mlp.drop.p > 0):
            n1, n2 = self.norm1, self.norm2
            qkv = ops.linear(ops.layer_norm(x, n1.weight, n1.bias, n1.eps), self.qkv.weight, self.qkv.bias)
            att = ops.stripe_attention(qkv, self.patches_resolution, self.split_size, [m.idx for m in a], [m.num_heads for m in a],
                                       [m.get_v.weight for m in a], [m.get_v.bias for m in a], a[0].scale, attn_drop=ad)
            x = ops.dropout(ops.linear(att, self.proj.weight, self.proj.bias), self.proj_drop.p, residual=x, row_scale=rs1)
            return self.mlp(ops.layer_norm(x, n2.weight, n2.bias, n2.eps), residual=x, row_scale=rs2)
        return ops.cswin_block(x, self.patches_resolution, self.split_size, [m.idx for m in a], [m.num_heads for m in a],
                               a[0].scale, self.norm1, self.qkv, self.proj, self.norm2, self.mlp.fc1, self.mlp.fc2,
                               [m.get_v.weight for m in a], [m.get_v.bias for m in a], rs1, rs2, attn_drop=ad)


def img2windows(img, H_sp, W_sp):
    return ops.img2windows(img, H_sp, W_sp)


def windows2img(img_splits_hw, H_sp, W_sp, H, W):
    return ops.windows2img(img_splits_hw, H_sp, W_sp, H, W)


class Merge_Block(nn.Module):
    def __init__(self, dim, dim_out, norm_layer=nn.LayerNorm):
        super().__init__()
        self.conv = nn.Conv2d(dim, dim_out, 3, 2, 1)
        self.norm = norm_layer(dim_out)

    def forward(self, x):
        side = _square_side(x.shape[1])
        y = ops.conv_tokens(x, self.conv.weight, self.conv.bias, side, side, 2, 1)
        return ops.layer_norm(y, self.norm.weight, self.norm.bias, self.norm.eps)


class _CarafeBase(nn.Module):
    def __init__(self, dim, dim_out, kernel_size, up_factor):
        super().__init__()
        if kernel_size != 3:
            raise NotImplementedError("the HIP reassembly kernel is written for the 3x3 neighbourhood the reference uses")
        self.kernel_size, self.up_factor = kernel_size, up_factor
        self.down = nn.Conv2d(dim, dim // 4, 1)
        self.encoder = nn.Conv2d(dim // 4, up_factor ** 2 * kernel_size ** 2, kernel_size, 1, kernel_size // 2)
        self.out = nn.Conv2d(dim, dim_out, 1)

    def kernel_logits(self, x, side):
        mid = ops.linear(x, self.down.weight.flatten(1), self.down.bias)
        return ops.conv_tokens(mid, self.encoder.weight, self.encoder.bias, side, side, 1, 1)

    def forward(self, x):
        side = _square_side(x.shape[1])
        mid, z = ops.linear_pair(x, self.down.weight.flatten(1), self.down.bias, self.out.weight.flatten(1), None)
        e = ops.conv_tokens(mid, self.encoder.weight, self.encoder.bias, side, side, 1, 1)
        return ops.carafe_reassemble(e, z, self.out.bias, side, side, self.up_factor)


class CARAFE(_CarafeBase):
    def __init__(self, dim, dim_out, kernel_size=3, up_factor=2):
        super().__init__(dim, dim_out, kernel_size, up_factor)


class CARAFE4(_CarafeBase):
    def __init__(self, dim, dim_out, kernel_size=3, up_factor=4):
        super().__init__(dim, dim_out, kernel_size, up_factor)


class _SumInputChannels(torch.autograd.Function):

    @staticmethod
    def forward(ctx, w):
        ctx.cin = w.shape[1]
        return w.sum(1, keepdim=True)

    @staticmethod
    def backward(ctx, g):
        return g.repeat(1, ctx.cin, 1, 1)


class _PatchEmbed(nn.Sequential):

    def forward(self, img):
        conv, norm = self[0], self[2]
        w = conv.weight
        if img.shape[1] == 1 and w.shape[1] > 1:
            w = _SumInputChannels.apply(w)
        tok = ops.patch_embed_conv(img, w, conv.bias, conv.stride[0], conv.padding[0])
        return ops.layer_norm(tok, norm.weight, norm.bias, norm.eps)


class CSWinTransformer(nn.Module):

    def __init__(self, img_size=224, patch_size=16, in_chans=3, num_classes=8, embed_dim=64, depth=[1, 2, 9, 1],
                 split_size=[1, 2, 7, 7], num_heads=12, mlp_ratio=4., qkv_bias=True, qk_scale=None, drop_rate=0.,
                 attn_drop_rate=0., drop_path_rate=0, hybrid_backbone=None, norm_layer=nn.LayerNorm, use_chk=False):
        super().__init__()
        self.use_chk, self.num_classes = use_chk, num_classes
        self.num_features = self.embed_dim = embed_dim
        heads = num_heads
        E = embed_dim
        self.img_size = img_size

        self.stage1_conv_embed = _PatchEmbed(nn.Conv2d(in_chans, E, 7, 4, 2), TokenRearrange(), nn.LayerNorm(E))
        self.pos_drop = nn.Dropout(p=drop_rate)

        rates = torch.linspace(0, drop_path_rate, int(np.sum(depth))).tolist()
        first = np.concatenate([[0], np.cumsum(depth)]).astype(int)

        def make_stage(si, last=False):
            return nn.ModuleList(
                CSWinBlock(dim=E << si, num_heads=heads[si], reso=img_size // (4 << si), mlp_ratio=mlp_ratio,
                           qkv_bias=qkv_bias, qk_scale=qk_scale, split_size=split_size[si], drop=drop_rate,
                           attn_drop=attn_drop_rate, drop_path=rates[first[si] + i], norm_layer=norm_layer,
                           last_stage=last)
                for i in range(depth[si]))

        self.stage1 = make_stage(0)
        self.merge1 = Merge_Block(E, 2 * E)
        self.stage2 = make_stage(1)
        self.merge2 = Merge_Block(2 * E, 4 * E)
        self.stage3 = make_stage(2)
        self.merge3 = Merge_Block(4 * E, 8 * E)
        self.stage4 = make_stage(3, last=True)
        self.norm = norm_layer(8 * E)
        self.stage_up4 = make_stage(3, last=True)
        self.upsample4 = CARAFE(8 * E, 4 * E)
        self.concat_linear4 = nn.Linear(8 * E, 4 * E)
        self.stage_up3 = make_stage(2)
        self.upsample3 = CARAFE(4 * E, 2 * E)
        self.concat_linear3 = nn.Linear(4 * E, 2 * E)
        self.stage_up2 = make_stage(1)
        self.upsample2 = CARAFE(2 * E, E)
        self.concat_linear2 = nn.Linear(2 * E, E)
        self.stage_up1 = make_stage(0)
        self.upsample1 = CARAFE4(E, E)
        self.norm_up = norm_layer(E)
        self.output = nn.Conv2d(in_channels=E, out_channels=self.num_classes, kernel_size=1, bias=False)

        self.apply(self._init_weights)

    def _init_weights(self, m):
        if isinstance(m, nn.Linear):
            trunc_normal_(m.weight, std=.02)
            if m.bias is not None:
                nn.init.constant_(m.bias, 0)
        elif isinstance(m, (nn.LayerNorm, nn.BatchNorm2d)):
            nn.init.constant_(m.bias, 0)
            nn.init.constant_(m.weight, 1.0)

    @torch.jit.ignore
    def no_weight_decay(self):
        return {'pos_embed', 'cls_token'}

    @torch.jit.ignore
    def no_weight_decay_keywords(self):
        return {'relative_position_bias_table'}

    def _run(self, blocks, x):
        for blk in blocks:
            x = checkpoint.checkpoint(blk, x, use_reentrant=False) if self.use_chk else blk(x)
        return x

    def _predraw_drop_path(self, batch, device):
        blocks = [b for st in (self.stage1, self.stage2, self.stage3, self.stage4, self.stage_up4, self.stage_up3,
                               self.stage_up2, self.stage_up1) for b in st]
        live = [b for b in blocks if isinstance(b.drop_path, DropPath) and b.drop_path.drop_prob > 0.]
        for b in blocks:
            b._dp_preset = None
        if not (self.training and live):
            return
        cache = getattr(self, "_dp_keep", None)
        if cache is None or cache.device != device or cache.shape[0] != 2 * len(live):
            cache = torch.tensor([1.0 - b.drop_path.drop_prob for b in live for _ in (0, 1)], dtype=torch.float32,
                                 device=device)[:, None]
            self._dp_keep = cache
        keep = cache
        scales = (torch.rand(keep.shape[0], batch, device=device) < keep).to(torch.float32) / keep
        for i, b in enumerate(live):
            b._dp_preset = [scales[2 * i], scales[2 * i + 1]]

    def forward_features(self, x):
        self._predraw_drop_path(x.shape[0], x.device)
        ops.clear_twins()
        x = self.stage1_conv_embed(x)
        if self.pos_drop.p > 0 and self.training:
            x = ops.dropout(x, self.pos_drop.p)
        x = self._run(self.stage1, x)
        self.x1 = x
        x = self._run(self.stage2, self.merge1(x))
        self.x2 = x
        self.enc_mid_in = None
        if getattr(self, "detach_decoder_inputs", False) and torch.is_grad_enabled():
            x = x.detach().requires_grad_()
            self.enc_mid_in = x
        x = self._run(self.stage3, self.merge2(x))
        self.x3 = x
        x = self._run(self.stage4, self.merge3(x))
        return ops.layer_norm(x, self.norm.weight, self.norm.bias, self.norm.eps)

    def forward_up_features(self, x):
        _, s1, s2, s3 = getattr(self, "dec_in", None) or (None, self.x1, self.x2, self.x3)
        for blocks, up, cl, skip in ((self.stage_up4, self.upsample4, self.concat_linear4, s3),
                                    (self.stage_up3, self.upsample3, self.concat_linear3, s2),
                                    (self.stage_up2, self.upsample2, self.concat_linear2, s1)):
            x = up(self._run(blocks, x))
            x = ops.linear(skip, cl.weight, cl.bias, x2=x)
        x = self._run(self.stage_up1, x)
        return ops.layer_norm(x, self.norm_up.weight, self.norm_up.bias, self.norm_up.eps)

    def up_x4(self, x):
        up, head = self.upsample1, self.output
        side = _square_side(x.shape[1])
        ncls = head.out_channels
        cpad = max(16, 1 << (ncls - 1).bit_length())
        w_head = head.weight.flatten(1)
        w_fused = ops.matmul_nn(w_head, up.out.weight.flatten(1))
        b_fused = ops.linear(up.out.bias[None, :], w_head)[0]
        w_fused = nn.functional.pad(w_fused, (0, 0, 0, cpad - ncls))
        b_fused = nn.functional.pad(b_fused, (0, cpad - ncls))
        mid, z = ops.linear_pair(x, up.down.weight.flatten(1), up.down.bias, w_fused, None)
        e = ops.conv_tokens(mid, up.encoder.weight, up.encoder.bias, side, side, 1, 1)
        tok = ops.carafe_reassemble(e, z, b_fused, side, side, up.up_factor)
        return ops.tokens_to_nchw(tok, ncls, up.up_factor * side, up.up_factor * side)

    def forward(self, x):
        x = self.forward_features(x)
        self.xb = x
        bound = [x, self.x1, self.x2, self.x3]
        if getattr(self, "detach_decoder_inputs", False) and torch.is_grad_enabled():
            bound = [t.detach().requires_grad_() for t in bound]
        self.dec_in = bound
        x = self.forward_up_features(bound[0])
        return self.up_x4(x)
```

cswin_unet_amd/ops.py:

```python
import ctypes
import math

import torch
from torch.autograd import Function
from torch.autograd.function import once_differentiable

from ._lib import CswinHipError, ReduceJob, WgradDesc, act_bf16, call, dev_f32, lib, precision, ptr, shadow_ptr, stream

__all__ = ["layer_norm", "linear", "linear_pair", "mlp", "stripe_attention", "cswin_block", "conv_tokens", "patch_embed_conv", "carafe_reassemble",
           "tokens_to_nchw", "matmul_nn", "ce_dice_loss", "dropout", "img2windows", "windows2img"]


MAX_REDUCE_JOBS = 48
TAIL_RIDER_JOBS = 16


class engine_backward:

    def __init__(self, opt=None):
        self._flat = opt.flat_grad if opt is not None else None
        self._slots = {p.data_ptr(): (o, p.numel()) for p, o in zip(opt.params, opt.offsets)} if opt is not None else {}
        self._queue = []
        self._given = set()

    def __enter__(self):
        global _pass
        self._outer, _pass = _pass, self
        return self

    def __exit__(self, *exc):
        global _pass
        _pass = self._outer
        if exc[0] is None:
            self.flush()
        return False

    def grad(self, param_key, shape, device):
        n = math.prod(shape)
        o, numel = self._slots.get(param_key, (0, -1)) if param_key else (0, -1)
        if numel != n:
            return torch.empty(tuple(shape), dtype=torch.float32, device=device)
        if o in self._given:
            raise CswinHipError(f"engine_backward: two ops of one backward pass use the leaf parameter at offset {o} of flat_grad; "
                                f"the first gradient is already placed there and its reduction may still be waiting")
        self._given.add(o)
        return self._flat[o:o + n].view(shape)

    def _in_flat(self, address):
        return self._flat is not None and 0 <= address - self._flat.data_ptr() < 4 * self._flat.numel()

    def reduce(self, jobs, reads):
        now = []
        for j in jobs:
            if j.part and all(self._in_flat(a) for a in (j.out, j.out2) if a):
                self._queue.append((ReduceJob.from_buffer_copy(j), reads))
            elif j.part:
                now.append(j)
        if now:
            arr = (ReduceJob * len(now))(*now)
            call("cswin_rows_sum_multi", _job_ptr(arr), len(now), stream())

    def queued_outputs(self):
        return [a for j, _ in self._queue for a in (j.out, j.out2) if a]

    def take_pending(self, maxn=TAIL_RIDER_JOBS):
        taken, self._queue = self._queue[:maxn], self._queue[maxn:]
        arr = (ReduceJob * len(taken))(*[j for j, _ in taken])
        return (_job_ptr(arr) if taken else None), len(taken), (arr, taken)

    def flush(self):
        while self._queue:
            jobs, n, _owner = self.take_pending(MAX_REDUCE_JOBS)
            call("cswin_rows_sum_multi", jobs, n, stream())


_pass = engine_backward()


def _param_keys(*ts):
    return tuple(t.data_ptr() if t is not None and t.is_leaf else 0 for t in ts)


def _job_ptr(jobs, i=0):
    return ctypes.c_void_p(ctypes.addressof(jobs) + i * ctypes.sizeof(ReduceJob))


def _fill_wgrad(d, dy, x, row_scale, dw, dbias, workspace, ws_bytes, rows_per_sample, M, N, K, io_bf16=0):
    d.dy, d.x, d.row_scale, d.dw, d.dbias = (t.data_ptr() if t is not None else None for t in (dy, x, row_scale, dw, dbias))
    d.workspace, d.ws_bytes, d.rows_per_sample, d.M, d.N, d.K = workspace, ws_bytes, rows_per_sample, M, N, K
    d.precision, d.io_bf16 = precision(), io_bf16


def _ws(nbytes, device):
    return torch.empty(max(int(nbytes), 16) // 4 + 4, dtype=torch.float32, device=device)


def _int_array(vals):
    return (ctypes.c_int * len(vals))(*vals)


def _ptr_array(tensors):
    return (ctypes.c_void_p * len(tensors))(*[t.data_ptr() for t in tensors])


class _LayerNorm(Function):
    @staticmethod
    def forward(ctx, x, gamma, beta, eps):
        x, gamma, beta = dev_f32(x, "layer_norm input"), dev_f32(gamma), dev_f32(beta)
        C = x.shape[-1]
        M = x.numel() // C
        y = torch.empty_like(x)
        mean = torch.empty(M, dtype=torch.float32, device=x.device)
        rstd = torch.empty_like(mean)
        call("cswin_layernorm_fwd", ptr(x), ptr(gamma), ptr(beta), ptr(y), ptr(mean), ptr(rstd), M, C, eps, 0, stream())
        ctx.save_for_backward(x, gamma, mean, rstd)
        ctx.keys = _param_keys(gamma, beta)
        return y

    @staticmethod
    @once_differentiable
    def backward(ctx, dy):
        x, gamma, mean, rstd = ctx.saved_tensors
        dy = dev_f32(dy)
        C = x.shape[-1]
        M = x.numel() // C
        dx = torch.empty_like(x)
        dg, db = (_pass.grad(k, gamma.shape, gamma.device) for k in ctx.keys)
        nbytes = lib().cswin_layernorm_bwd_workspace(M, C)
        ws = _ws(nbytes, x.device)
        job = (ReduceJob * 1)()
        call("cswin_layernorm_bwd", ptr(dy), ptr(x), ptr(mean), ptr(rstd), ptr(gamma), None, ptr(dx), ptr(dg), ptr(db),
             ptr(ws), nbytes, M, C, _job_ptr(job), None, stream())
        _pass.reduce(job, (ws,))
        return dx, dg, db, None


def layer_norm(x, gamma, beta, eps=1e-5):
    return _LayerNorm.apply(x, gamma, beta, eps)


def _rows_per_sample(x):
    return x.numel() // (x.shape[0] * x.shape[-1])


_twins = {}


def _twin_put(t, t16):
    _twins[t.data_ptr()] = (t, t16)


def _twin_take(t):
    e = _twins.pop(t.data_ptr(), None)
    return e[1] if e is not None and e[0]._cdata == t._cdata else None


def clear_twins():
    _twins.clear()


def _wsrc(w):
    if act_bf16() and w.shape[0] % 4 == 0 and w.shape[1] % 4 == 0:
        sp = shadow_ptr(w)
        if sp is not None:
            return sp, 4
    return ptr(w), 0


class _Linear(Function):
    @staticmethod
    def forward(ctx, x, w, b, x2, residual, row_scale):
        x, w = dev_f32(x, "linear input"), dev_f32(w, "linear weight")
        b, x2, residual, row_scale = dev_f32(b), dev_f32(x2), dev_f32(residual), dev_f32(row_scale)
        K1 = x.shape[-1]
        K = K1 + (x2.shape[-1] if x2 is not None else 0)
        N = w.shape[0]
        assert w.shape[1] == K, f"linear: weight {tuple(w.shape)} vs input features {K}"
        M = x.numel() // K1
        y = torch.empty(x.shape[:-1] + (N,), dtype=torch.float32, device=x.device)
        rps = _rows_per_sample(x) if row_scale is not None else 1
        pw, fw = _wsrc(w)
        call("cswin_linear_fwd", ptr(x), ptr(x2), K1 if x2 is not None else 0, pw, ptr(b), ptr(y), None, ptr(residual),
             ptr(row_scale), rps, M, N, K, precision(), fw, stream())
        ctx.save_for_backward(x, w, x2, row_scale)
        ctx.has_bias, ctx.has_res, ctx.rps, ctx.keys = b is not None, residual is not None, rps, _param_keys(w, b)
        return y

    @staticmethod
    @once_differentiable
    def backward(ctx, dy):
        x, w, x2, row_scale = ctx.saved_tensors
        dy = dev_f32(dy)
        K1 = x.shape[-1]
        N, K = w.shape
        M = x.numel() // K1
        need = ctx.needs_input_grad
        dx = dx2 = dw = db = None
        if need[0] or (x2 is not None and need[3]):
            dx = torch.empty_like(x)
            dx2 = torch.empty_like(x2) if x2 is not None else None
            pw, fw = _wsrc(w)
            call("cswin_linear_bwd_data", ptr(dy), pw, ptr(dx), ptr(dx2), K1 if x2 is not None else 0, None,
                 ptr(row_scale), ctx.rps, None, M, N, K, precision(), fw, stream())
        if need[1]:
            dw = _pass.grad(ctx.keys[0], w.shape, w.device)
            db = _pass.grad(ctx.keys[1], (N,), w.device) if ctx.has_bias else None
            nbytes = lib().cswin_linear_bwd_weight_workspace(M, N, K)
            ws = _ws(nbytes, w.device)
            job = (ReduceJob * 1)()
            call("cswin_linear_bwd_weight", ptr(dy), ptr(x), ptr(x2), K1 if x2 is not None else 0, ptr(row_scale), ctx.rps,
                 ptr(dw), ptr(db), ptr(ws), nbytes, M, N, K, _job_ptr(job), precision(), stream())
            _pass.reduce(job, (ws,))
        dres = dy if ctx.has_res else None
        return dx, dw, db, dx2, dres, None


def linear(x, w, b=None, x2=None, residual=None, row_scale=None):
    return _Linear.apply(x, w, b, x2, residual, row_scale)


class _LinearPair(Function):

    @staticmethod
    def forward(ctx, x, w1, b1, w2, b2):
        x, w1, b1, w2, b2 = (dev_f32(t) for t in (x, w1, b1, w2, b2))
        K = x.shape[-1]
        M = x.numel() // K
        ys = []
        for w, b in ((w1, b1), (w2, b2)):
            assert w.shape[1] == K
            y = torch.empty(x.shape[:-1] + (w.shape[0],), dtype=torch.float32, device=x.device)
            call("cswin_linear_fwd", ptr(x), None, 0, ptr(w), ptr(b), ptr(y), None, None, None, 1, M, w.shape[0], K, precision(), 0, stream())
            ys.append(y)
        ctx.save_for_backward(x, w1, w2)
        ctx.has_b = (b1 is not None, b2 is not None)
        ctx.keys = _param_keys(w1, b1, w2, b2)
        return tuple(ys)

    @staticmethod
    @once_differentiable
    def backward(ctx, dy1, dy2):
        x, w1, w2 = ctx.saved_tensors
        dy1, dy2 = dev_f32(dy1), dev_f32(dy2)
        K = x.shape[-1]
        M = x.numel() // K
        st = stream()
        dx = None
        if ctx.needs_input_grad[0]:
            dx = torch.empty_like(x)
            call("cswin_linear_bwd_data", ptr(dy1), ptr(w1), ptr(dx), None, 0, None, None, 1, None, M, w1.shape[0], K, precision(), 0, st)
            call("cswin_linear_bwd_data", ptr(dy2), ptr(w2), ptr(dx), None, 0, None, None, 1, ptr(dx), M, w2.shape[0], K, precision(), 0, st)
        grads, keep = [], []
        wg, jobs = (WgradDesc * 2)(), (ReduceJob * 2)()
        for i, (dy, w, has_b) in enumerate(((dy1, w1, ctx.has_b[0]), (dy2, w2, ctx.has_b[1]))):
            N = w.shape[0]
            dw = _pass.grad(ctx.keys[2 * i], w.shape, w.device)
            db = _pass.grad(ctx.keys[2 * i + 1], (N,), w.device) if has_b else None
            nbytes = lib().cswin_linear_bwd_weight_workspace(M, N, K)
            ws = _ws(nbytes, w.device)
            keep.append(ws)
            _fill_wgrad(wg[i], dy, x, None, dw, db, ws.data_ptr(), nbytes, 1, M, N, K)
            grads += [dw, db]
        call("cswin_linear_bwd_weight_batch", ctypes.cast(wg, ctypes.c_void_p), 2, _job_ptr(jobs), None, 0, st)
        _pass.reduce(jobs, keep)
        return (dx,) + tuple(grads)


def linear_pair(x, w1, b1, w2, b2):
    return _LinearPair.apply(x, w1, b1, w2, b2)


class _Mlp(Function):

    @staticmethod
    def forward(ctx, x, w1, b1, w2, b2, residual, row_scale, drop_p, seeds):
        x, w1, b1, w2, b2 = (dev_f32(t) for t in (x, w1, b1, w2, b2))
        residual, row_scale = dev_f32(residual), dev_f32(row_scale)
        K = x.shape[-1]
        Hd, N = w1.shape[0], w2.shape[0]
        M = x.numel() // K
        pre = torch.empty(x.shape[:-1] + (Hd,), dtype=torch.float32, device=x.device)
        act = torch.empty_like(pre)
        (p1, f1), (p2, f2) = _wsrc(w1), _wsrc(w2)
        call("cswin_linear_fwd", ptr(x), None, 0, p1, ptr(b1), ptr(pre), ptr(act), None, None, 1, M, Hd, K, precision(), f1, stream())
        y = torch.empty(x.shape[:-1] + (N,), dtype=torch.float32, device=x.device)
        rps = _rows_per_sample(x) if row_scale is not None else 1
        if drop_p > 0:
            call("cswin_dropout", ptr(act), None, None, ptr(act), act.numel(), act.numel() // act.shape[0], drop_p, seeds[0], ptr(dropout_epoch(act.device)), stream())
            call("cswin_linear_fwd", ptr(act), None, 0, p2, ptr(b2), ptr(y), None, None, None, 1, M, N, Hd, precision(), f2, stream())
            call("cswin_dropout", ptr(y), ptr(residual), ptr(row_scale), ptr(y), y.numel(), y.numel() // y.shape[0], drop_p, seeds[1], ptr(dropout_epoch(y.device)), stream())
        else:
            call("cswin_linear_fwd", ptr(act), None, 0, p2, ptr(b2), ptr(y), None, ptr(residual), ptr(row_scale), rps,
                 M, N, Hd, precision(), f2, stream())
        ctx.save_for_backward(x, w1, w2, pre, act, row_scale)
        ctx.has_res, ctx.rps, ctx.has_b1, ctx.has_b2 = residual is not None, rps, b1 is not None, b2 is not None
        ctx.keys = _param_keys(w1, b1, w2, b2)
        ctx.drop = (float(drop_p), seeds)
        return y

    @staticmethod
    @once_differentiable
    def backward(ctx, dy):
        x, w1, w2, pre, act, row_scale = ctx.saved_tensors
        dy = dev_f32(dy)
        K = x.shape[-1]
        Hd, N = w1.shape[0], w2.shape[0]
        M = x.numel() // K
        dev = x.device
        st = stream()
        drop_p, seeds = ctx.drop
        dyl, rs_gemm = dy, row_scale
        if drop_p > 0:
            dyl = torch.empty_like(dy)
            call("cswin_dropout", ptr(dy), None, ptr(row_scale), ptr(dyl), dy.numel(), dy.numel() // dy.shape[0], drop_p, seeds[1], ptr(dropout_epoch(dy.device)), st)
            rs_gemm = None
        dpre = torch.empty_like(pre)
        call("cswin_linear_bwd_data", ptr(dyl), ptr(w2), ptr(dpre), None, 0, ptr(pre), ptr(rs_gemm), ctx.rps, None, M, N,
             Hd, precision(), 0, st)
        if drop_p > 0:
            call("cswin_dropout", ptr(dpre), None, None, ptr(dpre), dpre.numel(), dpre.numel() // dpre.shape[0], drop_p, seeds[0], ptr(dropout_epoch(dpre.device)), st)
        dx = None
        if ctx.needs_input_grad[0]:
            dx = torch.empty_like(x)
            call("cswin_linear_bwd_data", ptr(dpre), ptr(w1), ptr(dx), None, 0, None, None, 1, None, M, Hd, K, precision(), 0, st)
        k1, kb1, k2, kb2 = ctx.keys
        dw2 = _pass.grad(k2, w2.shape, dev)
        db2 = _pass.grad(kb2, (N,), dev) if ctx.has_b2 else None
        nbytes = max(lib().cswin_linear_bwd_weight_workspace(M, N, Hd), lib().cswin_linear_bwd_weight_workspace(M, Hd, K))
        ws, ws1 = _ws(nbytes, dev), _ws(nbytes, dev)
        jobs = (ReduceJob * 2)()
        call("cswin_linear_bwd_weight", ptr(dyl), ptr(act), None, 0, ptr(rs_gemm), ctx.rps, ptr(dw2), ptr(db2), ptr(ws),
             nbytes, M, N, Hd, _job_ptr(jobs, 0), precision(), stream())
        dw1 = _pass.grad(k1, w1.shape, dev)
        db1 = _pass.grad(kb1, (Hd,), dev) if ctx.has_b1 else None
        call("cswin_linear_bwd_weight", ptr(dpre), ptr(x), None, 0, None, 1, ptr(dw1), ptr(db1), ptr(ws1), nbytes, M, Hd, K,
             _job_ptr(jobs, 1), precision(), stream())
        _pass.reduce(jobs, (ws, ws1))
        return dx, dw1, db1, dw2, db2, (dy if ctx.has_res else None), None, None, None


_epoch = {}


def dropout_epoch(device):
    t = _epoch.get(device)
    if t is None:
        t = _epoch[device] = torch.zeros(1, dtype=torch.int64, device=device)
    return t


def advance_dropout_epoch(device):
    dropout_epoch(device).add_(1)


def _draw_seeds(n):
    return tuple(int(v) for v in torch.randint(0, 2 ** 62, (n,)).tolist())


def mlp(x, w1, b1, w2, b2, residual=None, row_scale=None, drop_p=0.0):
    return _Mlp.apply(x, w1, b1, w2, b2, residual, row_scale, float(drop_p), _draw_seeds(2) if drop_p > 0 else (0, 0))


class _MatmulNN(Function):

    @staticmethod
    def forward(ctx, a, b):
        a, b = dev_f32(a), dev_f32(b)
        M, N = a.shape
        K = b.shape[1]
        c = torch.empty(M, K, dtype=torch.float32, device=a.device)
        call("cswin_linear_bwd_data", ptr(a), ptr(b), ptr(c), None, 0, None, None, 1, None, M, N, K, precision(), 0, stream())
        ctx.save_for_backward(a, b)
        return c

    @staticmethod
    @once_differentiable
    def backward(ctx, dc):
        a, b = ctx.saved_tensors
        dc = dev_f32(dc)
        M, N = a.shape
        K = b.shape[1]
        da = torch.empty_like(a)
        call("cswin_linear_fwd", ptr(dc), None, 0, ptr(b), None, ptr(da), None, None, None, 1, M, N, K, precision(), 0, stream())
        db = torch.empty_like(b)
        nbytes = lib().cswin_linear_bwd_weight_workspace(M, N, K)
        ws = _ws(nbytes, a.device)
        job = (ReduceJob * 1)()
        call("cswin_linear_bwd_weight", ptr(a), ptr(dc), None, 0, None, 1, ptr(db), None, ptr(ws), nbytes, M, N, K,
             _job_ptr(job), precision(), stream())
        _pass.reduce(job, (ws,))
        return da, db


def matmul_nn(a, b):
    return _MatmulNN.apply(a, b)


class _StripeAttention(Function):
    @staticmethod
    def forward(ctx, qkv, reso, split, idx, heads, scale, drop, *wb):
        q16 = qkv.dtype == torch.bfloat16 and qkv.is_cuda
        qkv = qkv.contiguous() if q16 else dev_f32(qkv, "attention qkv")
        nb = len(idx)
        ws_ = [dev_f32(t).view(t.shape[0], 9) for t in wb[:nb]]
        bs_ = [dev_f32(t) for t in wb[nb:]]
        B, L, C3 = qkv.shape
        C = C3 // 3
        if L != reso * reso:
            raise ValueError("flatten img_tokens has wrong size")
        y = torch.empty(B, L, C, dtype=torch.float32, device=qkv.device)
        y0 = torch.empty_like(y) if any(ctx.needs_input_grad) else None
        lse = torch.empty(B, sum(heads), L, dtype=torch.float32, device=qkv.device)
        call("cswin_attn_fwd", ptr(qkv), _ptr_array(ws_), _ptr_array(bs_), ptr(y), ptr(y0), ptr(lse), B, reso, C, nb,
             _int_array(heads), _int_array(idx), split, float(scale or 0.0), drop[0], drop[1], ptr(dropout_epoch(qkv.device)) if drop[0] > 0 else None,
             int(q16), stream())
        ctx.save_for_backward(qkv, lse, y0, *ws_, *bs_)
        ctx.keys = _param_keys(*wb)
        ctx.meta = (reso, split, tuple(idx), tuple(heads), float(scale or 0.0), drop)
        return y

    @staticmethod
    @once_differentiable
    def backward(ctx, dy):
        qkv, lse, y0, *wb_ = ctx.saved_tensors
        reso, split, idx, heads, scale, drop = ctx.meta
        dy = dev_f32(dy)
        nb = len(idx)
        ws_, bs_ = wb_[:nb], wb_[nb:]
        B, L, C3 = qkv.shape
        C = C3 // 3
        dqkv = torch.empty_like(qkv)
        dws = [_pass.grad(k, t.shape, t.device) for k, t in zip(ctx.keys[:nb], ws_)]
        dbs = [_pass.grad(k, t.shape, t.device) for k, t in zip(ctx.keys[nb:], bs_)]
        ha, ia = _int_array(heads), _int_array(idx)
        nbytes = lib().cswin_attn_bwd_workspace(B, reso, C, nb, ha, ia, split)
        ws = _ws(nbytes, qkv.device)
        jobs = (ReduceJob * 2)()
        call("cswin_attn_bwd", ptr(qkv), _ptr_array(ws_), _ptr_array(bs_), ptr(lse), ptr(y0), ptr(dy), ptr(dqkv), _ptr_array(dws),
             _ptr_array(dbs), ptr(ws), nbytes, B, reso, C, nb, ha, ia, split, scale, _job_ptr(jobs), drop[0], drop[1],
             ptr(dropout_epoch(qkv.device)) if drop[0] > 0 else None, int(qkv.dtype == torch.bfloat16), stream())
        _pass.reduce(jobs, (ws,))
        return (dqkv, None, None, None, None, None, None) + tuple(d.view(d.shape[0], 1, 3, 3) for d in dws) + tuple(dbs)


def _attn_drop(p):
    p = float(p)
    return (p, _draw_seeds(1)[0]) if p > 0 else (0.0, 0)


def stripe_attention(qkv, reso, split, idx, heads, lepe_w, lepe_b, scale=None, attn_drop=0.0):
    return _StripeAttention.apply(qkv, reso, split, tuple(idx), tuple(heads), scale, _attn_drop(attn_drop), *lepe_w, *lepe_b)


class _CSWinBlock(Function):

    @staticmethod
    def forward(ctx, x, reso, split, idx, heads, scale, eps1, eps2, rs1, rs2, drop, g1, b1, wqkv, bqkv, wp, bp, g2, b2, w1, bb1,
                w2, bb2, *lepe):
        x = dev_f32(x, "block input")
        B, L, C = x.shape
        if L != reso * reso:
            raise ValueError("flatten img_tokens has wrong size")
        M = B * L
        dev, st = x.device, stream()
        nb = len(idx)
        lw = [dev_f32(t).view(t.shape[0], 9) for t in lepe[:nb]]
        lb = [dev_f32(t) for t in lepe[nb:]]
        rs1, rs2 = dev_f32(rs1), dev_f32(rs2)
        E = lambda *shape: torch.empty(*shape, dtype=torch.float32, device=dev)
        s16 = act_bf16() and C % 4 == 0
        E16 = (lambda *shape: torch.empty(*shape, dtype=torch.bfloat16, device=dev)) if s16 else E
        (pq, fq), (pp, fp), (p1, f1), (p2, f2) = [_wsrc(w) if s16 else (ptr(w), 0) for w in (wqkv, wp, w1, w2)]
        io_x, io_xy = (1, 3) if s16 else (0, 0)
        h1, m1, r1 = E16(B, L, C), E(M), E(M)
        call("cswin_layernorm_fwd", ptr(x), ptr(g1), ptr(b1), ptr(h1), ptr(m1), ptr(r1), M, C, eps1, int(s16), st)
        qkv = E16(B, L, 3 * C)
        call("cswin_linear_fwd", ptr(h1), None, 0, pq, ptr(bqkv), ptr(qkv), None, None, None, 1, M, 3 * C, C, precision(), io_xy | fq, st)
        att, lse = E16(B, L, C), E(B, sum(heads), L)
        att0 = E16(B, L, C) if any(ctx.needs_input_grad) else None
        ha, ia = _int_array(heads), _int_array(idx)
        call("cswin_attn_fwd", ptr(qkv), _ptr_array(lw), _ptr_array(lb), ptr(att), ptr(att0), ptr(lse), B, reso, C, nb, ha, ia, split,
             float(scale or 0.0), drop[0], drop[1], ptr(dropout_epoch(dev)) if drop[0] > 0 else None, 7 if s16 else 0, st)
        x1 = torch.empty_like(x)
        call("cswin_linear_fwd", ptr(att), None, 0, pp, ptr(bp), ptr(x1), None, ptr(x), ptr(rs1), L, M, C, C, precision(), io_x | fp, st)
        h2, m2, r2 = E16(B, L, C), E(M), E(M)
        call("cswin_layernorm_fwd", ptr(x1), ptr(g2), ptr(b2), ptr(h2), ptr(m2), ptr(r2), M, C, eps2, int(s16), st)
        Hd = w1.shape[0]
        pre, act = E16(B, L, Hd), E16(B, L, Hd)
        call("cswin_linear_fwd", ptr(h2), None, 0, p1, ptr(bb1), ptr(pre), ptr(act), None, None, 1, M, Hd, C, precision(), io_xy | f1, st)
        y = torch.empty_like(x)
        call("cswin_linear_fwd", ptr(act), None, 0, p2, ptr(bb2), ptr(y), None, ptr(x1), ptr(rs2), L, M, C, Hd, precision(), io_x | f2, st)
        ctx.save_for_backward(x, m1, r1, h1, qkv, lse, att, att0, x1, m2, r2, h2, pre, act, rs1, rs2, g1, wqkv, wp, g2, w1, w2, *lw, *lb)
        ctx.meta = (reso, split, tuple(idx), tuple(heads), float(scale or 0.0), bqkv is not None, s16, drop)
        ctx.keys = _param_keys(g1, b1, wqkv, bqkv, wp, bp, g2, b2, w1, bb1, w2, bb2, *lepe)
        return y

    @staticmethod
    @once_differentiable
    def backward(ctx, dy):
        (x, m1, r1, h1, qkv, lse, att, att0, x1, m2, r2, h2, pre, act, rs1, rs2, g1, wqkv, wp, g2, w1, w2, *lwb) = ctx.saved_tensors
        reso, split, idx, heads, scale, has_qkv_bias, s16, drop = ctx.meta
        lw, lb = lwb[:len(idx)], lwb[len(idx):]
        dy = dev_f32(dy)
        B, L, C = x.shape
        M, Hd, nb = B * L, w1.shape[0], len(idx)
        dev, st, h = x.device, stream(), lib()
        E = lambda *shape: torch.empty(*shape, dtype=torch.float32, device=dev)
        sizes = [h.cswin_linear_bwd_weight_workspace(M, C, Hd), h.cswin_linear_bwd_weight_workspace(M, Hd, C),
                 h.cswin_layernorm_bwd_workspace(M, C), h.cswin_linear_bwd_weight_workspace(M, C, C),
                 h.cswin_linear_bwd_weight_workspace(M, 3 * C, C), h.cswin_layernorm_bwd_workspace(M, C)]
        sizes = [(n + 255) // 256 * 256 for n in sizes]
        ws = _ws(sum(sizes), dev)
        wsp = [ctypes.c_void_p(ws.data_ptr() + sum(sizes[:i])) for i in range(6)]
        jobs = (ReduceJob * 8)()
        (pq, fq), (pp, fp), (p1, f1), (p2, f2) = [_wsrc(w) if s16 else (ptr(w), 0) for w in (wqkv, wp, w1, w2)]
        E16 = lambda *shape: torch.empty(*shape, dtype=torch.bfloat16, device=dev)
        dy16 = _twin_take(dy) if s16 else None
        dpre = torch.empty_like(pre)
        call("cswin_linear_bwd_data", ptr(dy16 if dy16 is not None else dy), p2, ptr(dpre), None, 0, ptr(pre), ptr(rs2), L, None, M, C, Hd,
             precision(), ((10 if s16 else 0) | f2) | (1 if dy16 is not None else 0), st)
        wg = (WgradDesc * 4)()

        def defer_wgrad(slot, dy_, x_, rs_, dw_, db_, wsi, N_, K_, io=0):
            _fill_wgrad(wg[slot], dy_, x_, rs_, dw_, db_, wsp[wsi].value, sizes[wsi], L, M, N_, K_, io if s16 else 0)

        kg1, kb1, kwqkv, kbqkv, kwp, kbp, kg2, kb2, kw1, kbb1, kw2, kbb2, *klepe = ctx.keys
        G = lambda key, *shape: _pass.grad(key, shape, dev)
        dw2, db2 = G(kw2, *w2.shape), G(kbb2, C)
        if dy16 is not None:
            defer_wgrad(0, dy16, act, rs2, dw2, db2, 0, C, Hd, io=3)
        else:
            defer_wgrad(0, dy, act, rs2, dw2, db2, 0, C, Hd, io=2)
        dw1, db1 = G(kw1, *w1.shape), G(kbb1, Hd)
        defer_wgrad(1, dpre, h2, None, dw1, db1, 1, Hd, C, io=3)
        dh2 = torch.empty_like(x)
        call("cswin_linear_bwd_data", ptr(dpre), p1, ptr(dh2), None, 0, None, None, 1, None, M, Hd, C, precision(), (1 if s16 else 0) | f1, st)
        dx1, dg2, dbt2 = torch.empty_like(x), G(kg2, C), G(kb2, C)
        dx1_16 = E16(B, L, C) if s16 else None
        call("cswin_layernorm_bwd", ptr(dh2), ptr(x1), ptr(m2), ptr(r2), ptr(g2), ptr(dy), ptr(dx1), ptr(dg2), ptr(dbt2), wsp[2],
             sizes[2], M, C, _job_ptr(jobs, 2), ptr(dx1_16), st)
        datt = dh2
        call("cswin_linear_bwd_data", ptr(dx1_16 if s16 else dx1), pp, ptr(datt), None, 0, None, ptr(rs1), L, None, M, C, C, precision(),
             fp | (1 if s16 else 0), st)
        dwp, dbp = G(kwp, *wp.shape), G(kbp, C)
        defer_wgrad(2, dx1_16 if s16 else dx1, att, rs1, dwp, dbp, 3, C, C, io=3)
        dqkv = torch.empty_like(qkv)
        dlw = [G(k, *t.shape) for k, t in zip(klepe[:nb], lw)]
        dlb = [G(k, *t.shape) for k, t in zip(klepe[nb:], lb)]
        ha, ia = _int_array(heads), _int_array(idx)
        naw = h.cswin_attn_bwd_workspace(B, reso, C, nb, ha, ia, split)
        aws = _ws(naw, dev)
        call("cswin_attn_bwd", ptr(qkv), _ptr_array(lw), _ptr_array(lb), ptr(lse), ptr(att0), ptr(datt), ptr(dqkv),
             _ptr_array(dlw), _ptr_array(dlb), ptr(aws), naw, B, reso, C, nb, ha, ia, split, scale, _job_ptr(jobs, 6), drop[0], drop[1],
             ptr(dropout_epoch(dev)) if drop[0] > 0 else None, 7 if s16 else 0, st)
        dwqkv = G(kwqkv, *wqkv.shape)
        dbqkv = G(kbqkv, 3 * C) if has_qkv_bias else None
        defer_wgrad(3, dqkv, h1, None, dwqkv, dbqkv, 4, 3 * C, C, io=3)
        wjobs = (ReduceJob * 4)()
        dh1 = datt
        pend, npend, riders = _pass.take_pending()
        if precision() == 0:
            call("cswin_linear_bwd_tail", ptr(dqkv), pq, ptr(dh1), M, 3 * C, C, ctypes.cast(wg, ctypes.c_void_p), 4,
                 _job_ptr(wjobs), pend, npend, st)
        else:
            call("cswin_linear_bwd_weight_batch", ctypes.cast(wg, ctypes.c_void_p), 4, _job_ptr(wjobs), pend, npend, st)
            call("cswin_linear_bwd_data", ptr(dqkv), pq, ptr(dh1), None, 0, None, None, 1, None, M, 3 * C, C, precision(), (1 if s16 else 0) | fq, st)
        for slot, ji in enumerate((0, 1, 3, 4)):
            jobs[ji] = wjobs[slot]
        dx, dg1, dbt1 = torch.empty_like(x), G(kg1, C), G(kb1, C)
        dx16 = E16(B, L, C) if s16 else None
        call("cswin_layernorm_bwd", ptr(dh1), ptr(x), ptr(m1), ptr(r1), ptr(g1), ptr(dx1), ptr(dx), ptr(dg1), ptr(dbt1), wsp[5],
             sizes[5], M, C, _job_ptr(jobs, 5), ptr(dx16), st)
        if s16:
            _twin_put(dx, dx16)
        _pass.reduce(jobs, (ws, aws))
        grads = (dx, None, None, None, None, None, None, None, None, None, None, dg1, dbt1, dwqkv, dbqkv, dwp, dbp, dg2, dbt2, dw1, db1,
                 dw2, db2)
        return grads + tuple(d.view(d.shape[0], 1, 3, 3) for d in dlw) + tuple(dlb)


def cswin_block(x, reso, split, idx, heads, scale, norm1, qkv, proj, norm2, fc1, fc2, lepe_w, lepe_b, rs1=None, rs2=None, attn_drop=0.0):
    return _CSWinBlock.apply(x, reso, split, tuple(idx), tuple(heads), scale, norm1.eps, norm2.eps, rs1, rs2, _attn_drop(attn_drop),
                             norm1.weight, norm1.bias, qkv.weight, qkv.bias, proj.weight, proj.bias, norm2.weight,
                             norm2.bias, fc1.weight, fc1.bias, fc2.weight, fc2.bias, *lepe_w, *lepe_b)


def _permute_w(w, cpad, want_t):
    Cout, Cin, ks, _ = w.shape
    wp = torch.empty(Cout, ks * ks, cpad, dtype=torch.float32, device=w.device)
    wpt = torch.empty(ks * ks, Cout, cpad, dtype=torch.float32, device=w.device) if want_t else None
    call("cswin_conv_weight_permute", ptr(w), ptr(wp), ptr(wpt), Cout, Cin, ks, cpad, stream())
    return wp, wpt


class _ConvTokens(Function):
    @staticmethod
    def forward(ctx, x, w, b, H, W, stride, pad):
        x, w, b = dev_f32(x, "conv input"), dev_f32(w), dev_f32(b)
        B, L, Cin = x.shape
        assert L == H * W and w.shape[1] == Cin
        Cout, ks = w.shape[0], w.shape[2]
        OH, OW = (H + 2 * pad - ks) // stride + 1, (W + 2 * pad - ks) // stride + 1
        need_dx = ctx.needs_input_grad[0]
        same = stride == 1 and 2 * pad == ks - 1 and Cout % 4 == 0
        wp, wpt = _permute_w(w, Cin, need_dx and not same)
        y = torch.empty(B, OH * OW, Cout, dtype=torch.float32, device=x.device)
        call("cswin_conv_tok_fwd", ptr(x), ptr(wp), ptr(b), ptr(y), B, H, W, Cin, Cout, ks, stride, pad, precision(), stream())
        ctx.save_for_backward(x, w, wpt)
        ctx.meta = (H, W, stride, pad, b is not None)
        ctx.keys = _param_keys(w, b)
        return y

    @staticmethod
    @once_differentiable
    def backward(ctx, dy):
        x, w, wpt = ctx.saved_tensors
        H, W, stride, pad, has_b = ctx.meta
        dy = dev_f32(dy)
        B, L, Cin = x.shape
        Cout, ks = w.shape[0], w.shape[2]
        st = stream()
        dx = None
        if ctx.needs_input_grad[0]:
            dx = torch.empty_like(x)
            if stride == 1 and 2 * pad == ks - 1 and Cout % 4 == 0:
                wf = torch.empty(Cin, ks * ks, Cout, dtype=torch.float32, device=x.device)
                call("cswin_conv_weight_flipT", ptr(w), ptr(wf), Cout, Cin, ks, st)
                call("cswin_conv_tok_fwd", ptr(dy), ptr(wf), None, ptr(dx), B, H, W, Cout, Cin, ks, 1, pad, precision(), st)
            else:
                if wpt is None:
                    _, wpt = _permute_w(w, Cin, True)
                call("cswin_conv_tok_bwd_data", ptr(dy), ptr(wpt), ptr(dx), B, H, W, Cin, Cout, ks, stride, pad, precision(), st)
        dw = _pass.grad(ctx.keys[0], w.shape, x.device)
        db = _pass.grad(ctx.keys[1], (Cout,), x.device) if has_b else None
        nbytes = lib().cswin_conv_tok_bwd_weight_workspace(B, H, W, Cin, Cout, ks, stride, pad)
        ws = _ws(nbytes, x.device)
        job = (ReduceJob * 1)()
        call("cswin_conv_tok_bwd_weight", ptr(dy), ptr(x), ptr(dw), ptr(db), ptr(ws), nbytes, B, H, W, Cin, Cout, ks,
             stride, pad, 1, _job_ptr(job), precision(), stream())
        _pass.reduce(job, (ws,))
        return dx, dw, db, None, None, None, None


def conv_tokens(x, w, b, H, W, stride, pad):
    return _ConvTokens.apply(x, w, b, H, W, stride, pad)


class _PatchEmbedConv(Function):

    @staticmethod
    def forward(ctx, img, w, b, stride, pad):
        img, w, b = dev_f32(img, "image"), dev_f32(w), dev_f32(b)
        B, Cin, H, W = img.shape
        Cout, ks = w.shape[0], w.shape[2]
        cpad = (Cin + 3) // 4 * 4
        st = stream()
        x = torch.empty(B, H * W, cpad, dtype=torch.float32, device=img.device)
        call("cswin_nchw_to_tokens", ptr(img), ptr(x), B, Cin, H, W, cpad, st)
        wp, _ = _permute_w(w, cpad, False)
        OH, OW = (H + 2 * pad - ks) // stride + 1, (W + 2 * pad - ks) // stride + 1
        y = torch.empty(B, OH * OW, Cout, dtype=torch.float32, device=img.device)
        call("cswin_conv_tok_fwd", ptr(x), ptr(wp), ptr(b), ptr(y), B, H, W, cpad, Cout, ks, stride, pad, precision(), st)
        ctx.save_for_backward(x, w)
        ctx.meta = (H, W, stride, pad, cpad, b is not None)
        ctx.keys = _param_keys(w, b)
        return y

    @staticmethod
    @once_differentiable
    def backward(ctx, dy):
        x, w = ctx.saved_tensors
        H, W, stride, pad, cpad, has_b = ctx.meta
        dy = dev_f32(dy)
        B = x.shape[0]
        Cout, Cin, ks, _ = w.shape
        st = stream()
        dwp = torch.empty(Cout, ks * ks, cpad, dtype=torch.float32, device=x.device)
        db = _pass.grad(ctx.keys[1], (Cout,), x.device) if has_b else None
        nbytes = lib().cswin_conv_tok_bwd_weight_workspace(B, H, W, cpad, Cout, ks, stride, pad)
        ws = _ws(nbytes, x.device)
        call("cswin_conv_tok_bwd_weight", ptr(dy), ptr(x), ptr(dwp), ptr(db), ptr(ws), nbytes, B, H, W, cpad, Cout, ks, stride,
             pad, 0, None, precision(), st)
        dw = _pass.grad(ctx.keys[0], w.shape, x.device)
        call("cswin_conv_weight_unpermute", ptr(dwp), ptr(dw), Cout, Cin, ks, cpad, st)
        return None, dw, db, None, None


def patch_embed_conv(img, w, b, stride=4, pad=2):
    return _PatchEmbedConv.apply(img, w, b, stride, pad)


class _CarafeReassemble(Function):
    @staticmethod
    def forward(ctx, e, z, bias, H, W, S):
        e, z, bias = dev_f32(e, "carafe kernel logits"), dev_f32(z, "carafe features"), dev_f32(bias)
        B, L, Cz = z.shape
        assert L == H * W and e.shape == (B, L, 9 * S * S)
        out = torch.empty(B, L * S * S, Cz, dtype=torch.float32, device=z.device)
        wt = torch.empty_like(e)
        call("cswin_carafe_fwd", ptr(e), ptr(z), ptr(bias), ptr(out), ptr(wt), B, H, W, Cz, S, stream())
        ctx.save_for_backward(z, wt)
        ctx.meta = (H, W, S, bias is not None)
        ctx.keys = _param_keys(bias)
        return out

    @staticmethod
    @once_differentiable
    def backward(ctx, dout):
        z, wt = ctx.saved_tensors
        H, W, S, has_b = ctx.meta
        dout = dev_f32(dout)
        B, L, Cz = z.shape
        de = torch.empty_like(wt)
        dz = torch.empty_like(z)
        db = _pass.grad(ctx.keys[0], (Cz,), z.device) if has_b else None
        nbytes = lib().cswin_carafe_bwd_workspace(B, H, W, Cz, S)
        ws = _ws(nbytes, z.device)
        job = (ReduceJob * 1)()
        call("cswin_carafe_bwd", ptr(dout), ptr(z), ptr(wt), ptr(de), ptr(dz), ptr(db), ptr(ws), nbytes, B, H, W, Cz, S,
             _job_ptr(job), stream())
        _pass.reduce(job, (ws,))
        return de, dz, db, None, None, None


def carafe_reassemble(e, z, bias, H, W, S):
    return _CarafeReassemble.apply(e, z, bias, H, W, S)


class _TokensToNchw(Function):
    @staticmethod
    def forward(ctx, x, C, H, W):
        x = dev_f32(x)
        B, L, Cpad = x.shape
        assert L == H * W and C <= Cpad
        y = torch.empty(B, C, H, W, dtype=torch.float32, device=x.device)
        call("cswin_tokens_to_nchw", ptr(x), ptr(y), B, C, H, W, Cpad, stream())
        ctx.meta = (C, H, W, Cpad)
        return y

    @staticmethod
    @once_differentiable
    def backward(ctx, dy):
        C, H, W, Cpad = ctx.meta
        dy = dev_f32(dy)
        B = dy.shape[0]
        dx = torch.empty(B, H * W, Cpad, dtype=torch.float32, device=dy.device)
        call("cswin_nchw_to_tokens", ptr(dy), ptr(dx), B, C, H, W, Cpad, stream())
        return dx, None, None, None


def tokens_to_nchw(x, C, H, W):
    return _TokensToNchw.apply(x, C, H, W)


def img2windows(img, H_sp, W_sp):
    img = dev_f32(img, "img2windows input")
    B, C, H, W = img.shape
    out = torch.empty(B * (H // H_sp) * (W // W_sp), H_sp * W_sp, C, dtype=torch.float32, device=img.device)
    call("cswin_img2windows", ptr(img), ptr(out), B, C, H, W, H_sp, W_sp, stream())
    return out


def windows2img(img_splits_hw, H_sp, W_sp, H, W):
    x = dev_f32(img_splits_hw, "windows2img input")
    C = x.shape[-1]
    B = int(x.shape[0] / (H * W / H_sp / W_sp))
    out = torch.empty(B, H, W, C, dtype=torch.float32, device=x.device)
    call("cswin_windows2img", ptr(x), ptr(out), B, C, H, W, H_sp, W_sp, stream())
    return out


class _CeDiceLoss(Function):
    @staticmethod
    def forward(ctx, logits, labels, w_ce, w_dice, group, probs, class_weight):
        logits = dev_f32(logits, "logits")
        class_weight = dev_f32(class_weight)
        labels = labels.contiguous()
        if labels.dtype != torch.int64:
            labels = labels.long()
        B, ncls = logits.shape[:2]
        HW = logits.numel() // (B * ncls)
        dev = logits.device
        st = stream()
        nbytes = lib().cswin_loss_workspace(B, ncls, HW)
        ws = _ws(nbytes, dev)
        sums = torch.empty(1 + 3 * ncls, dtype=torch.float32, device=dev)
        call("cswin_loss_sums", ptr(logits), ptr(labels), ptr(sums), ptr(ws), nbytes, B, ncls, HW, int(probs), st)
        world = 1
        if group is not None:
            import torch.distributed as dist
            world = dist.get_world_size(group)
            if world > 1:
                dist.all_reduce(sums, group=group)
        out = torch.empty(3, dtype=torch.float32, device=dev)
        coef = torch.empty(2 * ncls, dtype=torch.float32, device=dev)
        call("cswin_loss_finalize", ptr(sums), ptr(out), ptr(coef), float(B * HW * world), ncls, w_ce, w_dice, ptr(class_weight),
             stream())
        ctx.save_for_backward(logits, labels, coef)
        ctx.meta = (w_ce / float(B * HW), w_dice / ncls * world, int(probs))
        loss = out[0].clone()
        ctx.mark_non_differentiable(out)
        return loss, out

    @staticmethod
    @once_differentiable
    def backward(ctx, gloss, _gout):
        logits, labels, coef = ctx.saved_tensors
        ce_scale, dice_scale, probs = ctx.meta
        B, ncls = logits.shape[:2]
        HW = logits.numel() // (B * ncls)
        gloss = dev_f32(gloss.reshape(1))
        dlogits = torch.empty_like(logits)
        call("cswin_loss_bwd", ptr(logits), ptr(labels), ptr(coef), ptr(gloss), ptr(dlogits), ce_scale, dice_scale, B, ncls,
             HW, probs, stream())
        return dlogits, None, None, None, None, None, None


def ce_dice_loss(logits, labels, w_ce=0.4, w_dice=0.6, group=None, inputs_are_probs=False, class_weight=None):
    if inputs_are_probs and w_ce != 0.0:
        raise ValueError("ce_dice_loss: cross entropy needs logits; with inputs_are_probs pass w_ce=0")
    return _CeDiceLoss.apply(logits, labels, float(w_ce), float(w_dice), group, bool(inputs_are_probs), class_weight)


class _Dropout(Function):
    @staticmethod
    def forward(ctx, x, residual, row_scale, p, seed):
        x, residual, row_scale = dev_f32(x, "dropout input"), dev_f32(residual), dev_f32(row_scale)
        y = torch.empty_like(x)
        eps = x.numel() // x.shape[0]
        call("cswin_dropout", ptr(x), ptr(residual), ptr(row_scale), ptr(y), x.numel(), eps, float(p), int(seed), ptr(dropout_epoch(x.device)), stream())
        ctx.save_for_backward(row_scale)
        ctx.meta = (float(p), int(seed), eps, residual is not None)
        return y

    @staticmethod
    @once_differentiable
    def backward(ctx, dy):
        (row_scale,) = ctx.saved_tensors
        p, seed, eps, has_res = ctx.meta
        dy = dev_f32(dy)
        dx = torch.empty_like(dy)
        call("cswin_dropout", ptr(dy), None, ptr(row_scale), ptr(dx), dy.numel(), eps, p, seed, ptr(dropout_epoch(dy.device)), stream())
        return dx, (dy if has_res else None), None, None, None


def dropout(x, p, residual=None, row_scale=None, seed=None):
    if seed is None:
        seed = int(torch.randint(0, 2 ** 62, (1,)).item())
    return _Dropout.apply(x, residual, row_scale, p, seed)
```

include/cswin_hip.h:

```cpp
#ifndef CSWIN_HIP_H
#define CSWIN_HIP_H

#include <stddef.h>

#ifdef __cplusplus
extern "C" {
#endif

#define CSWIN_ABI_VERSION 4

#define CSWIN_OK 0
#define CSWIN_ERR_SHAPE (-1)
#define CSWIN_ERR_ALIGN (-2)
#define CSWIN_ERR_WORKSPACE (-3)
#define CSWIN_ERR_HIP (-4)
#define CSWIN_ERR_UNSUPPORTED (-5)

typedef struct cswin_reduce_job {
    const float* part;
    float* out;
    float* out2;
    long long n_first, n, stride;
    int rows, reserved;
    int conv_kk, conv_cin;
} cswin_reduce_job;

const char* cswin_last_error(void);
int cswin_abi_version(void);
int cswin_device_ok(void);

int cswin_attn_fwd(const float* qkv, const float* const* lepe_w, const float* const* lepe_b, float* y, float* y0, float* lse,
                   int B, int reso, int C, int nbranch, const int* heads, const int* idx, int split, float scale,
                   float drop_p, unsigned long long drop_seed, const unsigned long long* drop_epoch, int qkv_bf16, void* stream);
size_t cswin_attn_bwd_workspace(int B, int reso, int C, int nbranch, const int* heads, const int* idx, int split);
int cswin_attn_bwd(const float* qkv, const float* const* lepe_w, const float* const* lepe_b, const float* lse,
                   const float* y0, const float* dy, float* dqkv, float* const* dlepe_w, float* const* dlepe_b,
                   void* workspace, size_t ws_bytes, int B, int reso, int C, int nbranch, const int* heads, const int* idx,
                   int split, float scale, cswin_reduce_job* deferred, float drop_p, unsigned long long drop_seed,
                   const unsigned long long* drop_epoch, int qkv_bf16, void* stream);

int cswin_img2windows(const float* img, float* out, int B, int C, int H, int W, int H_sp, int W_sp, void* stream);
int cswin_windows2img(const float* win, float* out, int B, int C, int H, int W, int H_sp, int W_sp, void* stream);

int cswin_layernorm_fwd(const float* x, const float* gamma, const float* beta, float* y, float* mean, float* rstd,
                        int M, int C, float eps, int y_bf16, void* stream);
size_t cswin_layernorm_bwd_workspace(int M, int C);
int cswin_layernorm_bwd(const float* dy, const float* x, const float* mean, const float* rstd, const float* gamma,
                        const float* dres, float* dx, float* dgamma, float* dbeta, void* workspace, size_t ws_bytes,
                        int M, int C, cswin_reduce_job* deferred, void* dx_bf16, void* stream);

int cswin_linear_fwd(const float* x, const float* x2, int k_split, const float* w, const float* bias, float* y,
                     float* y_act, const float* residual, const float* row_scale, int rows_per_sample, int M, int N,
                     int K, int precision, int io_bf16, void* stream);
int cswin_linear_bwd_data(const float* dy, const float* w, float* dx, float* dx2, int k_split, const float* gelu_pre,
                          const float* row_scale, int rows_per_sample, const float* add, int M, int N, int K,
                          int precision, int io_bf16, void* stream);
size_t cswin_linear_bwd_weight_workspace(int M, int N, int K);
int cswin_linear_bwd_weight(const float* dy, const float* x, const float* x2, int k_split, const float* row_scale,
                            int rows_per_sample, float* dw, float* dbias, void* workspace, size_t ws_bytes, int M,
                            int N, int K, cswin_reduce_job* deferred, int precision, void* stream);
typedef struct cswin_wgrad_desc {
    const float* dy;
    const float* x;
    const float* row_scale;
    float* dw;
    float* dbias;
    void* workspace;
    size_t ws_bytes;
    int rows_per_sample, M, N, K;
    int precision;
    int io_bf16;
} cswin_wgrad_desc;
int cswin_linear_bwd_weight_batch(const cswin_wgrad_desc* problems, int n, cswin_reduce_job* deferred, const cswin_reduce_job* pending,
                                  int npending, void* stream);
int cswin_linear_bwd_tail(const float* dy, const float* w, float* dx, int M, int N, int K, const cswin_wgrad_desc* problems, int n,
                          cswin_reduce_job* deferred, const cswin_reduce_job* pending, int npending, void* stream);
int cswin_rows_sum_multi(const cswin_reduce_job* jobs, int njobs, void* stream);

int cswin_conv_tok_fwd(const float* x, const float* w_perm, const float* bias, float* y, int B, int H, int W, int Cin,
                       int Cout, int ks, int stride, int pad, int precision, void* stream);
int cswin_conv_tok_bwd_data(const float* dy, const float* w_permT, float* dx, int B, int H, int W, int Cin, int Cout,
                            int ks, int stride, int pad, int precision, void* stream);
size_t cswin_conv_tok_bwd_weight_workspace(int B, int H, int W, int Cin, int Cout, int ks, int stride, int pad);
int cswin_conv_tok_bwd_weight(const float* dy, const float* x, float* dw, float* dbias, void* workspace,
                              size_t ws_bytes, int B, int H, int W, int Cin, int Cout, int ks, int stride, int pad,
                              int torch_layout, cswin_reduce_job* deferred, int precision, void* stream);
int cswin_conv_weight_permute(const float* w, float* w_perm, float* w_permT, int Cout, int Cin, int ks, int Cpad,
                              void* stream);
int cswin_conv_weight_unpermute(const float* dw_perm, float* dw, int Cout, int Cin, int ks, int Cpad, void* stream);
int cswin_conv_weight_flipT(const float* w, float* wf, int Cout, int Cin, int ks, void* stream);

int cswin_nchw_to_tokens(const float* x, float* y, int B, int C, int H, int W, int Cpad, void* stream);
int cswin_tokens_to_nchw(const float* x, float* y, int B, int C, int H, int W, int Cpad, void* stream);

int cswin_carafe_fwd(const float* e, const float* z, const float* bias, float* out, float* wt_save, int B, int H,
                     int W, int Cz, int S, void* stream);
size_t cswin_carafe_bwd_workspace(int B, int H, int W, int Cz, int S);
int cswin_carafe_bwd(const float* dout, const float* z, const float* wt_save, float* de, float* dz, float* dbias,
                     void* workspace, size_t ws_bytes, int B, int H, int W, int Cz, int S, cswin_reduce_job* deferred, void* stream);

size_t cswin_loss_workspace(int B, int ncls, long HW);
int cswin_loss_sums(const float* logits, const long long* labels, float* sums, void* workspace, size_t ws_bytes, int B,
                    int ncls, long HW, int inputs_are_probs, void* stream);
int cswin_loss_finalize(const float* sums, float* out3, float* coef, double n_pixels, int ncls, float w_ce,
                        float w_dice, const float* class_weight, void* stream);
int cswin_loss_bwd(const float* logits, const long long* labels, const float* coef, const float* grad_out,
                   float* dlogits, float ce_scale, float dice_scale, int B, int ncls, long HW, int inputs_are_probs,
                   void* stream);

int cswin_sgd_flat(float* p, const float* g, float* m, long n, const float* lr_dev, float momentum,
                   float weight_decay, float grad_scale, void* shadow_bf16, void* stream);
int cswin_multi_copy(const void* table, int nchunks, void* stream);

int cswin_dropout(const float* x, const float* residual, const float* row_scale, float* y, long n, long elems_per_sample,
                  float p, unsigned long long seed, const unsigned long long* seed_epoch, void* stream);
int cswin_pack_bf16(const float* src, void* dst_bf16, long n, void* stream);
int cswin_pack_bf16_scaled(const float* src, void* dst_bf16, long n, float scale, void* stream);
int cswin_unpack_bf16(const void* src_bf16, float* dst, long n, void* stream);

#ifdef __cplusplus
}
#endif
#endif
```

Measured before the change: 1885 images/sec.

## Fuse CARAFE output into NCHW, compose head weights, batch conv weight images

Adds CARAFE forward and backward kernels that read and write NCHW output directly, so a separate tokens-to-NCHW transpose is no longer needed. Adds head weight composition that folds the output projection into the segmentation head, batched conv weight image preparation, and a conv wgrad path that scatters padded-channel gradients straight into torch layout inside the reduction. The aim is fewer launches and fewer layout copies around the decoder head and conv stem. The cost is more kernel variants and strided NCHW stores in the CARAFE forward.

```diff
diff --git a/cswin_unet_amd/_lib.py b/cswin_unet_amd/_lib.py
--- a/cswin_unet_amd/_lib.py
+++ b/cswin_unet_amd/_lib.py
@@ -37,11 +37,18 @@
     "cswin_conv_weight_permute": (I, [P, P, P, I, I, I, I, P]),
     "cswin_conv_weight_unpermute": (I, [P, P, I, I, I, I, P]),
     "cswin_conv_weight_flipT": (I, [P, P, I, I, I, P]),
+    "cswin_conv_weight_images": (I, [P, I, P]),
+    "cswin_conv_tok_bwd_weight_cpad": (I, [P, P, P, P, P, SZ, I, I, I, I, I, I, I, I, I, P, I, P]),
     "cswin_nchw_to_tokens": (I, [P, P, I, I, I, I, I, P]),
     "cswin_tokens_to_nchw": (I, [P, P, I, I, I, I, I, P]),
     "cswin_carafe_fwd": (I, [P, P, P, P, P, I, I, I, I, I, P]),
     "cswin_carafe_bwd_workspace": (SZ, [I, I, I, I, I]),
     "cswin_carafe_bwd": (I, [P, P, P, P, P, P, P, SZ, I, I, I, I, I, P, P]),
+    "cswin_carafe_fwd_nchw": (I, [P, P, P, P, P, I, I, I, I, I, I, P]),
+    "cswin_carafe_bwd_nchw_ok": (I, [I, I, I, I]),
+    "cswin_carafe_bwd_nchw": (I, [P, P, P, P, P, P, P, SZ, I, I, I, I, I, I, P, P]),
+    "cswin_head_compose": (I, [P, P, P, P, P, I, I, I, I, P]),
+    "cswin_head_compose_bwd": (I, [P, P, P, P, P, P, P, P, I, I, I, P]),
     "cswin_loss_workspace": (SZ, [I, I, L]),
     "cswin_loss_sums": (I, [P, P, P, P, SZ, I, I, L, I, P]),
     "cswin_loss_finalize": (I, [P, P, P, D, I, F, F, P, P]),
@@ -66,6 +73,11 @@
     _fields_ = [("part", c_void_p), ("out", c_void_p), ("out2", c_void_p), ("n_first", ctypes.c_longlong),
                 ("n", ctypes.c_longlong), ("stride", ctypes.c_longlong), ("rows", c_int), ("reserved", c_int),
                 ("conv_kk", c_int), ("conv_cin", c_int)]
+
+
+class ConvImageJob(ctypes.Structure):
+    _fields_ = [("w", c_void_p), ("w_perm", c_void_p), ("w_permT", c_void_p), ("w_flipT", c_void_p), ("Cout", c_int),
+                ("Cin", c_int), ("ks", c_int), ("Cpad", c_int)]
 
 
 _lib = None
diff --git a/cswin_unet_amd/csrc/carafe.hip b/cswin_unet_amd/csrc/carafe.hip
--- a/cswin_unet_amd/csrc/carafe.hip
+++ b/cswin_unet_amd/csrc/carafe.hip
@@ -55,6 +55,56 @@
                     acc += wt[k] * *reinterpret_cast<const f32x4*>(z + (((long)b * H + hh) * W + ww) * Cz + c);
             }
             *reinterpret_cast<f32x4*>(out + orow * Cz + c) = acc;
+        }
+    }
+}
+
+template <int S>
+__global__ __launch_bounds__(256) void carafe_fwd_nchw_kernel(const float* __restrict__ e, const float* __restrict__ z,
+                                                               const float* __restrict__ bias, float* __restrict__ out,
+                                                               float* __restrict__ wt_save, int B, int H, int W, int Cz, int C) {
+    constexpr int S2 = S * S, PPB = 256 / S2;
+    const int sy = threadIdx.x / (PPB * S), rem = threadIdx.x % (PPB * S);
+    const int pl = rem / S, sx = rem % S, s = sy * S + sx;
+    const long npix = (long)B * H * W, plane = (long)H * S * W * S;
+    for (long p0 = (long)blockIdx.x * PPB; p0 < npix; p0 += (long)gridDim.x * PPB) {
+        const long pix = p0 + pl;
+        if (pix >= npix) continue;
+        const int w = (int)(pix % W);
+        const int h = (int)((pix / W) % H);
+        const int b = (int)(pix / ((long)W * H));
+        float wt[9];
+        float mx = -INFINITY;
+#pragma unroll
+        for (int k = 0; k < 9; ++k) {
+            wt[k] = e[pix * (9 * S2) + k * S2 + s];
+            mx = fmaxf(mx, wt[k]);
+        }
+        float sum = 0.f;
+#pragma unroll
+        for (int k = 0; k < 9; ++k) {
+            wt[k] = __expf(wt[k] - mx);
+            sum += wt[k];
+        }
+        const float inv = 1.0f / sum;
+#pragma unroll
+        for (int k = 0; k < 9; ++k) wt[k] *= inv;
+        if (wt_save) {
+#pragma unroll
+            for (int k = 0; k < 9; ++k) wt_save[pix * (9 * S2) + k * S2 + s] = wt[k];
+        }
+        float* o = out + (long)b * C * plane + ((long)h * S + sy) * (W * S) + w * S + sx;
+        for (int c = 0; c < C; c += 4) {
+            f32x4 acc = bias ? *reinterpret_cast<const f32x4*>(bias + c) : f32x4{0.f, 0.f, 0.f, 0.f};
+#pragma unroll
+            for (int k = 0; k < 9; ++k) {
+                const int hh = h + k / 3 - 1, ww = w + k % 3 - 1;
+                if ((unsigned)hh < (unsigned)H && (unsigned)ww < (unsigned)W)
+                    acc += wt[k] * *reinterpret_cast<const f32x4*>(z + (((long)b * H + hh) * W + ww) * Cz + c);
+            }
+#pragma unroll
+            for (int q = 0; q < 4; ++q)
+                if (c + q < C) o[(c + q) * plane] = acc[q];
         }
     }
 }
@@ -169,12 +219,26 @@
 
 __device__ __forceinline__ f32x4 carafe_mfma4(float a, float b, f32x4 c) { return __builtin_amdgcn_mfma_f32_16x16x4f32(a, b, c, 0, 0, 0); }
 
+__device__ __forceinline__ f32x4 lane_transpose4(f32x4 v, int kq) {
+    const bool hi = kq & 2, odd = kq & 1;
+    float s0 = hi ? v[0] : v[2], s1 = hi ? v[1] : v[3];
+    s0 = __shfl_xor(s0, 32, 64);
+    s1 = __shfl_xor(s1, 32, 64);
+    if (hi) { v[0] = s0; v[1] = s1; } else { v[2] = s0; v[3] = s1; }
+    float t0 = odd ? v[0] : v[1], t1 = odd ? v[2] : v[3];
+    t0 = __shfl_xor(t0, 16, 64);
+    t1 = __shfl_xor(t1, 16, 64);
+    if (odd) { v[0] = t0; v[2] = t1; } else { v[1] = t0; v[3] = t1; }
+    return v;
+}
+
 constexpr int C4_WAVES = 8;
 
+template <bool NCHW>
 __global__ __launch_bounds__(64 * C4_WAVES) void carafe4_bwd_fused_kernel(const float* __restrict__ dout, const float* __restrict__ z,
                                                                  const float* __restrict__ wt_save, float* __restrict__ de,
                                                                  float* __restrict__ dz, float* __restrict__ dbias_part,
-                                                                 int B, int H, int W, int tiles_x, int tiles_y) {
+                                                                 int B, int H, int W, int tiles_x, int tiles_y, int C) {
     constexpr int S = 4, S2 = 16, Cz = 16;
     __shared__ __attribute__((aligned(16))) float Gs[C4_NP * 9 * Cz];
     __shared__ __attribute__((aligned(16))) float zt[C4_NP * Cz];
@@ -222,13 +286,37 @@
 #pragma unroll
             for (int j = 0; j < 4; ++j) {
                 if (li < 9) av[u][j] = wp[li * S2 + 4 * j + kq];
-                dv[u][j] = drow[j * hstride + kq * Cz + li];
+                if (!NCHW) dv[u][j] = drow[j * hstride + kq * Cz + li];
             }
             if (interior[u]) {
-                db[u] = *reinterpret_cast<const f32x4*>(drow + (li >> 2) * hstride + (li & 3) * Cz + 4 * kq);
+                if (!NCHW) db[u] = *reinterpret_cast<const f32x4*>(drow + (li >> 2) * hstride + (li & 3) * Cz + 4 * kq);
 #pragma unroll
                 for (int r = 0; r < 4; ++r)
                     if (4 * kq + r < 9) wv[u][r] = wp[(4 * kq + r) * S2 + li];
+            }
+        }
+        if (NCHW) {
+            const int plm = pl0 + kq, phm = plm / C4_HALO, pwm = plm - phm * C4_HALO;
+            const int hm = h0 + phm, wm = w0 + pwm;
+            const bool okm = plm < C4_NP && (unsigned)hm < (unsigned)H && (unsigned)wm < (unsigned)W && li < C;
+            const float* src = dout + ((long)b * C + li) * ((long)H * S * W * S) + ((long)hm * S) * (W * S) + wm * S;
+            f32x4 X[4];
+#pragma unroll
+            for (int j = 0; j < 4; ++j)
+                X[j] = okm ? *reinterpret_cast<const f32x4*>(src + (long)j * (W * S)) : f32x4{0.f, 0.f, 0.f, 0.f};
+#pragma unroll
+            for (int j = 0; j < 4; ++j) {
+                X[j] = lane_transpose4(X[j], kq);
+#pragma unroll
+                for (int u = 0; u < PB; ++u) dv[u][j] = X[j][u];
+            }
+#pragma unroll
+            for (int u = 0; u < PB; ++u) {
+                if (!interior[u]) continue;
+                f32x4 t = {0.f, 0.f, 0.f, 0.f};
+#pragma unroll
+                for (int j = 0; j < 4; ++j) t = carafe_mfma4(dv[u][j], 4 * j + kq == li ? 1.f : 0.f, t);
+                db[u] = t;
             }
         }
 #pragma unroll
@@ -350,6 +438,18 @@
     return CSWIN_OK;
 }
 
+int cswin_carafe_fwd_nchw(const float* e, const float* z, const float* bias, float* out, float* wt_save, int B, int H, int W,
+                          int Cz, int C, int S, void* stream) {
+    CSWIN_REQUIRE(e && z && out, CSWIN_ERR_SHAPE, "carafe_fwd_nchw: null pointer");
+    CSWIN_REQUIRE(carafe_args_ok(B, H, W, Cz, S) && C > 0 && C <= Cz, CSWIN_ERR_UNSUPPORTED, "carafe_fwd_nchw: unsupported shape B=%d H=%d W=%d Cz=%d C=%d S=%d (Cz %% 4 == 0, 0 < C <= Cz, S in {2,4})", B, H, W, Cz, C, S);
+    hipStream_t st = (hipStream_t)stream;
+    const long pixels = (long)B * H * W;
+    if (S == 2) hipLaunchKernelGGL(carafe_fwd_nchw_kernel<2>, dim3(grid_for(pixels, 64)), dim3(256), 0, st, e, z, bias, out, wt_save, B, H, W, Cz, C);
+    else hipLaunchKernelGGL(carafe_fwd_nchw_kernel<4>, dim3(grid_for(pixels, 16)), dim3(256), 0, st, e, z, bias, out, wt_save, B, H, W, Cz, C);
+    CSWIN_LAUNCH_CHECK();
+    return CSWIN_OK;
+}
+
 static bool carafe4_fused_ok(int H, int W, int Cz, int S) { return S == 4 && Cz == 16 && H % C4_T == 0 && W % C4_T == 0; }
 
 size_t cswin_carafe_bwd_workspace(int B, int H, int W, int Cz, int S) {
@@ -372,8 +472,8 @@
     const bool no_fused = cswin_tuning().carafe_generic != 0;
     if (carafe4_fused_ok(H, W, Cz, S) && !no_fused) {
         const int tx = W / C4_T, ty = H / C4_T, nblk = B * tx * ty;
-        hipLaunchKernelGGL(carafe4_bwd_fused_kernel, dim3(nblk), dim3(64 * C4_WAVES), 0, st, dout, z, wt_save, de, dz,
-                           dbias ? (float*)workspace : nullptr, B, H, W, tx, ty);
+        hipLaunchKernelGGL(carafe4_bwd_fused_kernel<false>, dim3(nblk), dim3(64 * C4_WAVES), 0, st, dout, z, wt_save, de, dz,
+                           dbias ? (float*)workspace : nullptr, B, H, W, tx, ty, Cz);
         CSWIN_LAUNCH_CHECK();
         if (dbias) {
             reduce_now_or_defer(cswin_reduce_job{(const float*)workspace, dbias, nullptr, 0, Cz, Cz, nblk, 0, 0, 0}, deferred, st);
@@ -404,4 +504,27 @@
     return CSWIN_OK;
 }
 
-}
+int cswin_carafe_bwd_nchw_ok(int H, int W, int Cz, int S) { return carafe4_fused_ok(H, W, Cz, S) ? 1 : 0; }
+
+int cswin_carafe_bwd_nchw(const float* dout, const float* z, const float* wt_save, float* de, float* dz, float* dbias,
+                          void* workspace, size_t ws_bytes, int B, int H, int W, int Cz, int C, int S, cswin_reduce_job* deferred,
+                          void* stream) {
+    if (deferred) *deferred = cswin_reduce_job{};
+    CSWIN_REQUIRE(dout && z && wt_save && de && dz, CSWIN_ERR_SHAPE, "carafe_bwd_nchw: null pointer");
+    CSWIN_REQUIRE(B > 0 && H > 0 && W > 0 && C > 0 && C <= Cz && carafe4_fused_ok(H, W, Cz, S), CSWIN_ERR_UNSUPPORTED,
+                  "carafe_bwd_nchw: needs S = 4, Cz = 16, C <= 16, H and W multiples of %d (got B=%d H=%d W=%d Cz=%d C=%d S=%d)", C4_T, B, H, W, Cz, C, S);
+    CSWIN_REQUIRE(!dbias || (workspace && ws_bytes >= cswin_carafe_bwd_workspace(B, H, W, Cz, S)), CSWIN_ERR_WORKSPACE, "carafe_bwd_nchw: workspace too small");
+    CSWIN_REQUIRE(((uintptr_t)dout & 15) == 0, CSWIN_ERR_ALIGN, "carafe_bwd_nchw: dout must be 16-B aligned");
+    hipStream_t st = (hipStream_t)stream;
+    const int tx = W / C4_T, ty = H / C4_T, nblk = B * tx * ty;
+    hipLaunchKernelGGL(carafe4_bwd_fused_kernel<true>, dim3(nblk), dim3(64 * C4_WAVES), 0, st, dout, z, wt_save, de, dz,
+                       dbias ? (float*)workspace : nullptr, B, H, W, tx, ty, C);
+    CSWIN_LAUNCH_CHECK();
+    if (dbias) {
+        reduce_now_or_defer(cswin_reduce_job{(const float*)workspace, dbias, nullptr, 0, Cz, Cz, nblk, 0, 0, 0}, deferred, st);
+        CSWIN_LAUNCH_CHECK();
+    }
+    return CSWIN_OK;
+}
+
+}
diff --git a/cswin_unet_amd/csrc/common.h b/cswin_unet_amd/csrc/common.h
--- a/cswin_unet_amd/csrc/common.h
+++ b/cswin_unet_amd/csrc/common.h
@@ -84,6 +84,14 @@
 static inline int reduce_job_vec_ok(const cswin_reduce_job& j) {
     return ((uintptr_t)j.part % 16 == 0) && j.stride % 4 == 0 && j.n % 4 == 0 && (!j.out2 || j.n_first % 4 == 0);
 }
+
+__device__ __forceinline__ void reduce_conv_store(const cswin_reduce_job& j, long i, float t) {
+    const int kk = j.conv_kk, Cin = j.conv_cin & 0xFFFF, Cpar = (j.conv_cin >> 16) ? (j.conv_cin >> 16) : Cin;
+    const long co = i / ((long)kk * Cin);
+    const int rem = (int)(i - co * kk * Cin), tap = rem / Cin, ci = rem - tap * Cin;
+    if (ci < Cpar) j.out[(co * Cpar + ci) * kk + tap] = t;
+}
+__device__ __host__ __forceinline__ bool reduce_job_conv_padded(const cswin_reduce_job& j) { return j.conv_kk && (j.conv_cin >> 16); }
 
 constexpr int RS_COLS = 64, RS_G = 16;
 __device__ __forceinline__ void rows_sum_block(const cswin_reduce_job& job, long blk, float (*red)[RS_COLS + 1]) {
@@ -118,13 +126,12 @@
 #pragma unroll
         for (int k = 0; k < RS_G; ++k) t += red[k][threadIdx.x];
         if (job.out2 && i >= job.n_first) job.out2[i - job.n_first] = t;
+        else if (job.conv_kk) reduce_conv_store(job, i, t);
         else job.out[i] = t;
     }
 }
 
 __device__ __forceinline__ void rows_sum_conv_block(const cswin_reduce_job& j, long blk, float (*red)[RS_COLS + 1]) {
-    const int kk = j.conv_kk, Cin = j.conv_cin;
-    float* out = j.out;
     const int c4 = threadIdx.x & 15, g = threadIdx.x >> 4;
     const long i0 = blk * RS_COLS + 4 * c4;
     f32x4 s0 = {0.f, 0.f, 0.f, 0.f}, s1 = s0;
@@ -154,11 +161,7 @@
 #pragma unroll
         for (int k = 0; k < RS_G; ++k) t += red[k][threadIdx.x];
         if (j.out2 && i >= j.n_first) j.out2[i - j.n_first] = t;
-        else if (i < j.n_first) {
-            const long co = i / ((long)kk * Cin);
-            const int rem = (int)(i - co * kk * Cin), tap = rem / Cin, ci = rem - tap * Cin;
-            out[(co * Cin + ci) * kk + tap] = t;
-        }
+        else if (i < j.n_first) reduce_conv_store(j, i, t);
     }
 }
 
@@ -177,6 +180,17 @@
 } cswin_wgrad_desc;
 }
 
+extern "C" {
+typedef struct cswin_conv_image_job {
+    const float* w;
+    float* w_perm;
+    float* w_permT;
+    float* w_flipT;
+    int Cout, Cin, ks, Cpad;
+} cswin_conv_image_job;
+}
+constexpr int CSWIN_MAX_CONV_IMAGE_JOBS = 16;
+
 constexpr int CSWIN_MAX_REDUCE_JOBS = 48;
 struct ReduceJobs {
     cswin_reduce_job j[CSWIN_MAX_REDUCE_JOBS];
@@ -198,16 +212,19 @@
     if (r < job.rows) s0 += *reinterpret_cast<const f32x4*>(base + (long)r * job.stride);
     s0 += s1;
     if (job.out2 && i0 >= job.n_first) *reinterpret_cast<f32x4*>(job.out2 + (i0 - job.n_first)) = s0;
-    else *reinterpret_cast<f32x4*>(job.out + i0) = s0;
+    else if (job.conv_kk) {
+#pragma unroll
+        for (int e = 0; e < 4; ++e) reduce_conv_store(job, i0 + e, s0[e]);
+    } else *reinterpret_cast<f32x4*>(job.out + i0) = s0;
 }
 static inline int reduce_job_few_ok(const cswin_reduce_job& j) {
-    return !j.conv_kk && reduce_job_vec_ok(j) && j.rows <= RS_FEW_ROWS && j.n >= 4 * RS_FEW_COLS && ((uintptr_t)j.out % 16 == 0) &&
+    return (!j.conv_kk || reduce_job_conv_padded(j)) && reduce_job_vec_ok(j) && j.rows <= RS_FEW_ROWS && j.n >= 4 * RS_FEW_COLS && ((uintptr_t)j.out % 16 == 0) &&
            (!j.out2 || ((uintptr_t)j.out2 % 16 == 0));
 }
 
 static __global__ __launch_bounds__(256) void rows_sum_kernel(cswin_reduce_job job) {
     __shared__ float red[RS_G][RS_COLS + 1];
-    if (job.conv_kk) rows_sum_conv_block(job, blockIdx.x, red);
+    if (job.conv_kk && !reduce_job_conv_padded(job)) rows_sum_conv_block(job, blockIdx.x, red);
     else if (job.reserved & 2) rows_sum_few(job, blockIdx.x);
     else rows_sum_block(job, blockIdx.x, red);
 }
@@ -230,7 +247,7 @@
         else hi = mid - 1;
     }
     const int k = lo;
-    if (j[k].conv_kk) rows_sum_conv_block(j[k], blk - first_block[k], red);
+    if (j[k].conv_kk && !reduce_job_conv_padded(j[k])) rows_sum_conv_block(j[k], blk - first_block[k], red);
     else if (j[k].reserved & 2) rows_sum_few(j[k], blk - first_block[k]);
     else rows_sum_block(j[k], blk - first_block[k], red);
 }
diff --git a/cswin_unet_amd/csrc/gemm.hip b/cswin_unet_amd/csrc/gemm.hip
--- a/cswin_unet_amd/csrc/gemm.hip
+++ b/cswin_unet_amd/csrc/gemm.hip
@@ -1035,12 +1035,13 @@
     return cswin_linear_bwd_weight_workspace(B * OH * OW, Cout, ks * ks * Cin);
 }
 
-int cswin_conv_tok_bwd_weight(const float* dy, const float* x, float* dw_perm, float* dbias, void* workspace,
-                              size_t ws_bytes, int B, int H, int W, int Cin, int Cout, int ks, int stride, int pad,
-                              int torch_layout, cswin_reduce_job* deferred, int precision, void* stream) {
+static int conv_wgrad_impl(const float* dy, const float* x, float* dw_perm, float* dbias, void* workspace,
+                           size_t ws_bytes, int B, int H, int W, int Cin, int Cout, int ks, int stride, int pad,
+                           int torch_layout, int Cin_param, cswin_reduce_job* deferred, int precision, void* stream) {
     CSWIN_CHECK_PRECISION(precision, "conv_tok_bwd_weight");
     CSWIN_REQUIRE(dy && x && dw_perm, CSWIN_ERR_SHAPE, "conv_tok_bwd_weight: null pointer");
     CSWIN_REQUIRE(Cin % 4 == 0 && Cout % 4 == 0 && aligned16(dy) && aligned16(x), CSWIN_ERR_ALIGN, "conv_tok_bwd_weight: channels %% 4 and 16-B alignment required");
+    CSWIN_REQUIRE(!torch_layout || Cin < 65536, CSWIN_ERR_UNSUPPORTED, "conv_tok_bwd_weight: torch_layout needs Cin < 65536");
     int OH = (H + 2 * pad - ks) / stride + 1, OW = (W + 2 * pad - ks) / stride + 1;
     int M = B * OH * OW, K = ks * ks * Cin;
     size_t need = cswin_linear_bwd_weight_workspace(M, Cout, K);
@@ -1059,19 +1060,37 @@
     launch_gemm<false, false, 4, EPI_PLAIN, false>(A, Bm, e, Cout, K, M, splits, rps, precision, st);
     CSWIN_LAUNCH_CHECK();
     long n = (long)Cout * K;
-    cswin_reduce_job job = {slab, dw_perm, dbias, n, n + (dbias ? Cout : 0), slab_stride, splits, 0, torch_layout ? ks * ks : 0, torch_layout ? Cin : 0};
+    cswin_reduce_job job = {slab, dw_perm, dbias, n, n + (dbias ? Cout : 0), slab_stride, splits, 0, torch_layout ? ks * ks : 0,
+                            torch_layout ? (Cin | (Cin_param != Cin ? Cin_param << 16 : 0)) : 0};
     if (deferred) {
         *deferred = job;
         return CSWIN_OK;
     }
     if (torch_layout) {
-        job.reserved = reduce_job_vec_ok(job);
-        hipLaunchKernelGGL(rows_sum_kernel, dim3((unsigned)((job.n + RS_COLS - 1) / RS_COLS)), dim3(256), 0, st, job);
+        const int few = reduce_job_few_ok(job);
+        job.reserved = reduce_job_vec_ok(job) | (few ? 2 : 0);
+        const long cols = few ? RS_FEW_COLS : RS_COLS;
+        hipLaunchKernelGGL(rows_sum_kernel, dim3((unsigned)((job.n + cols - 1) / cols)), dim3(256), 0, st, job);
     } else {
         launch_rows_sum(slab, dw_perm, dbias, n, n + (dbias ? Cout : 0), splits, slab_stride, st);
     }
     CSWIN_LAUNCH_CHECK();
     return CSWIN_OK;
+}
+
+int cswin_conv_tok_bwd_weight(const float* dy, const float* x, float* dw_perm, float* dbias, void* workspace,
+                              size_t ws_bytes, int B, int H, int W, int Cin, int Cout, int ks, int stride, int pad,
+                              int torch_layout, cswin_reduce_job* deferred, int precision, void* stream) {
+    return conv_wgrad_impl(dy, x, dw_perm, dbias, workspace, ws_bytes, B, H, W, Cin, Cout, ks, stride, pad, torch_layout, Cin, deferred,
+                           precision, stream);
+}
+
+int cswin_conv_tok_bwd_weight_cpad(const float* dy, const float* x, float* dw, float* dbias, void* workspace, size_t ws_bytes,
+                                   int B, int H, int W, int Cin, int Cin_param, int Cout, int ks, int stride, int pad,
+                                   cswin_reduce_job* deferred, int precision, void* stream) {
+    CSWIN_REQUIRE(Cin_param > 0 && Cin_param <= Cin && Cin < 65536, CSWIN_ERR_SHAPE, "conv_tok_bwd_weight_cpad: 0 < Cin_param <= Cin < 65536");
+    return conv_wgrad_impl(dy, x, dw, dbias, workspace, ws_bytes, B, H, W, Cin, Cout, ks, stride, pad, 1, Cin_param, deferred, precision,
+                           stream);
 }
 
 int cswin_rows_sum_multi(const cswin_reduce_job* jobs, int njobs, void* stream) {
diff --git a/cswin_unet_amd/csrc/layout.hip b/cswin_unet_amd/csrc/layout.hip
--- a/cswin_unet_amd/csrc/layout.hip
+++ b/cswin_unet_amd/csrc/layout.hip
@@ -67,6 +67,118 @@
     }
 }
 
+constexpr int CI_ELEMS = 1024;
+struct ConvImageJobs {
+    cswin_conv_image_job j[CSWIN_MAX_CONV_IMAGE_JOBS];
+    int first_block[CSWIN_MAX_CONV_IMAGE_JOBS + 1];
+    int njobs;
+};
+
+__global__ __launch_bounds__(256) void conv_w_images_kernel(ConvImageJobs J) {
+    int k = 0;
+    while (k + 1 < J.njobs && (int)blockIdx.x >= J.first_block[k + 1]) ++k;
+    const cswin_conv_image_job& j = J.j[k];
+    const int kk = j.ks * j.ks, Cout = j.Cout, Cin = j.Cin, Cpad = j.Cpad;
+    const long base = (long)((int)blockIdx.x - J.first_block[k]) * CI_ELEMS;
+    if (j.w_perm || j.w_permT) {
+        const long total = (long)Cout * kk * Cpad;
+        for (long o = base + threadIdx.x; o < base + CI_ELEMS && o < total; o += 256) {
+            const int ci = (int)(o % Cpad);
+            const int tap = (int)((o / Cpad) % kk);
+            const int co = (int)(o / ((long)Cpad * kk));
+            const float v = ci < Cin ? j.w[((long)co * Cin + ci) * kk + tap] : 0.f;
+            if (j.w_perm) j.w_perm[o] = v;
+            if (j.w_permT) j.w_permT[((long)tap * Cout + co) * Cpad + ci] = v;
+        }
+    }
+    if (j.w_flipT) {
+        const long total = (long)Cin * kk * Cout;
+        for (long o = base + threadIdx.x; o < base + CI_ELEMS && o < total; o += 256) {
+            const int co = (int)(o % Cout);
+            const int tap = (int)((o / Cout) % kk);
+            const int ci = (int)(o / ((long)Cout * kk));
+            j.w_flipT[o] = j.w[((long)co * Cin + ci) * kk + (kk - 1 - tap)];
+        }
+    }
+}
+
+constexpr int HEAD_LDS_FLOATS = 12 * 1024;
+
+__device__ __forceinline__ const float* head_stage(const float* __restrict__ src, float* lds, int n, bool use_lds) {
+    if (!use_lds || !src) return src;
+    for (int i = threadIdx.x; i < n; i += 256) lds[i] = src[i];
+    return lds;
+}
+
+__global__ __launch_bounds__(256) void head_compose_kernel(const float* __restrict__ w_head, const float* __restrict__ w_out,
+                                                            const float* __restrict__ b_out, float* __restrict__ w_fused,
+                                                            float* __restrict__ b_fused, int ncls, int E, int C, int Cpad) {
+    __shared__ float lds[HEAD_LDS_FLOATS];
+    const bool st = ncls * E + E * C + E <= HEAD_LDS_FLOATS;
+    const float* wh = head_stage(w_head, lds, ncls * E, st);
+    const float* wo = head_stage(w_out, lds + ncls * E, E * C, st);
+    const float* bo = head_stage(b_out, lds + ncls * E + E * C, E, st);
+    __syncthreads();
+    const int total = Cpad * C + Cpad;
+    for (int o = blockIdx.x * 256 + threadIdx.x; o < total; o += gridDim.x * 256) {
+        float t = 0.f;
+        if (o < Cpad * C) {
+            const int n = o / C, c = o - n * C;
+            if (n < ncls)
+                for (int e = 0; e < E; ++e) t += wh[n * E + e] * wo[e * C + c];
+            w_fused[o] = t;
+        } else {
+            const int n = o - Cpad * C;
+            if (n < ncls && bo)
+                for (int e = 0; e < E; ++e) t += wh[n * E + e] * bo[e];
+            b_fused[n] = t;
+        }
+    }
+}
+
+__global__ __launch_bounds__(256) void head_compose_bwd_kernel(const float* __restrict__ w_head, const float* __restrict__ w_out,
+                                                                const float* __restrict__ b_out, const float* __restrict__ dw_fused,
+                                                                const float* __restrict__ db_fused, float* __restrict__ dw_head,
+                                                                float* __restrict__ dw_out, float* __restrict__ db_out, int ncls,
+                                                                int E, int C) {
+    __shared__ float lds[HEAD_LDS_FLOATS];
+    const int n_head = ncls * E, n_out = E * C;
+    const bool st = n_head + n_out + E + ncls * C + ncls <= HEAD_LDS_FLOATS;
+    const float* wh = head_stage(w_head, lds, n_head, st);
+    const float* wo = w_out;
+    const int wo_ld = st ? C + 1 : C;
+    if (st) {
+        float* d = lds + n_head;
+        for (int i = threadIdx.x; i < n_out; i += 256) d[(i / C) * wo_ld + (i % C)] = w_out[i];
+        wo = d;
+    }
+    float* rest = lds + n_head + E * (C + 1);
+    const bool st2 = st && n_head + E * (C + 1) + E + ncls * C + ncls <= HEAD_LDS_FLOATS;
+    const float* bo = head_stage(b_out, rest, E, st2);
+    const float* dwf = head_stage(dw_fused, rest + E, ncls * C, st2);
+    const float* dbf = head_stage(db_fused, rest + E + ncls * C, ncls, st2);
+    __syncthreads();
+    const int total = n_head + n_out + (db_out ? E : 0);
+    for (int o = blockIdx.x * 256 + threadIdx.x; o < total; o += gridDim.x * 256) {
+        float t = 0.f;
+        if (o < n_head) {
+            const int n = o / E, e = o - n * E;
+            for (int c = 0; c < C; ++c) t += dwf[n * C + c] * wo[e * wo_ld + c];
+            if (bo && dbf) t += dbf[n] * bo[e];
+            dw_head[o] = t;
+        } else if (o < n_head + n_out) {
+            const int i = o - n_head, e = i / C, c = i - e * C;
+            for (int n = 0; n < ncls; ++n) t += wh[n * E + e] * dwf[n * C + c];
+            dw_out[i] = t;
+        } else {
+            const int e = o - n_head - n_out;
+            if (dbf)
+                for (int n = 0; n < ncls; ++n) t += wh[n * E + e] * dbf[n];
+            db_out[e] = t;
+        }
+    }
+}
+
 int grid1d(long total) {
     long b = (total + 255) / 256;
     return (int)(b < 1 ? 1 : (b > 4096 ? 4096 : b));
@@ -152,4 +264,46 @@
     return CSWIN_OK;
 }
 
-}
+int cswin_conv_weight_images(const cswin_conv_image_job* jobs, int njobs, void* stream) {
+    CSWIN_REQUIRE(jobs && njobs > 0 && njobs <= CSWIN_MAX_CONV_IMAGE_JOBS, CSWIN_ERR_SHAPE, "conv_weight_images: 1..%d jobs", CSWIN_MAX_CONV_IMAGE_JOBS);
+    ConvImageJobs J = {};
+    int blocks = 0;
+    for (int i = 0; i < njobs; ++i) {
+        const cswin_conv_image_job& j = jobs[i];
+        CSWIN_REQUIRE(j.w && (j.w_perm || j.w_permT || j.w_flipT) && j.Cout > 0 && j.Cin > 0 && j.ks > 0 && j.Cpad >= j.Cin, CSWIN_ERR_SHAPE,
+                      "conv_weight_images: bad job %d", i);
+        J.j[i] = j;
+        J.first_block[i] = blocks;
+        const long perm = (j.w_perm || j.w_permT) ? (long)j.Cout * j.ks * j.ks * j.Cpad : 0;
+        const long flip = j.w_flipT ? (long)j.Cin * j.ks * j.ks * j.Cout : 0;
+        blocks += (int)(((perm > flip ? perm : flip) + CI_ELEMS - 1) / CI_ELEMS);
+    }
+    J.first_block[njobs] = blocks;
+    J.njobs = njobs;
+    hipLaunchKernelGGL(conv_w_images_kernel, dim3(blocks), dim3(256), 0, (hipStream_t)stream, J);
+    CSWIN_LAUNCH_CHECK();
+    return CSWIN_OK;
+}
+
+int cswin_head_compose(const float* w_head, const float* w_out, const float* b_out, float* w_fused, float* b_fused, int ncls,
+                       int E, int C, int Cpad, void* stream) {
+    CSWIN_REQUIRE(w_head && w_out && w_fused && b_fused && ncls > 0 && E > 0 && C > 0 && Cpad >= ncls, CSWIN_ERR_SHAPE, "head_compose: bad arguments");
+    hipLaunchKernelGGL(head_compose_kernel, dim3((Cpad * C + Cpad + 255) / 256), dim3(256), 0, (hipStream_t)stream, w_head, w_out,
+                       b_out, w_fused, b_fused, ncls, E, C, Cpad);
+    CSWIN_LAUNCH_CHECK();
+    return CSWIN_OK;
+}
+
+int cswin_head_compose_bwd(const float* w_head, const float* w_out, const float* b_out, const float* dw_fused,
+                           const float* db_fused, float* dw_head, float* dw_out, float* db_out, int ncls, int E, int C,
+                           void* stream) {
+    CSWIN_REQUIRE(w_head && w_out && dw_fused && dw_head && dw_out && ncls > 0 && E > 0 && C > 0 && (!db_out || b_out), CSWIN_ERR_SHAPE,
+                  "head_compose_bwd: bad arguments");
+    const int total = ncls * E + E * C + (db_out ? E : 0);
+    hipLaunchKernelGGL(head_compose_bwd_kernel, dim3((total + 255) / 256), dim3(256), 0, (hipStream_t)stream, w_head, w_out, b_out,
+                       dw_fused, db_fused, dw_head, dw_out, db_out, ncls, E, C);
+    CSWIN_LAUNCH_CHECK();
+    return CSWIN_OK;
+}
+
+}
diff --git a/cswin_unet_amd/networks/cswin_unet.py b/cswin_unet_amd/networks/cswin_unet.py
--- a/cswin_unet_amd/networks/cswin_unet.py
+++ b/cswin_unet_amd/networks/cswin_unet.py
@@ -175,11 +175,16 @@
 
 class _PatchEmbed(nn.Sequential):
 
-    def forward(self, img):
-        conv, norm = self[0], self[2]
-        w = conv.weight
+    def conv_weight(self, img):
+        w = self[0].weight
         if img.shape[1] == 1 and w.shape[1] > 1:
             w = _SumInputChannels.apply(w)
+        return w
+
+    def forward(self, img, w=None):
+        conv, norm = self[0], self[2]
+        if w is None:
+            w = self.conv_weight(img)
         tok = ops.patch_embed_conv(img, w, conv.bias, conv.stride[0], conv.padding[0])
         return ops.layer_norm(tok, norm.weight, norm.bias, norm.eps)
 
@@ -274,10 +279,10 @@
         for i, b in enumerate(live):
             b._dp_preset = [scales[2 * i], scales[2 * i + 1]]
 
-    def forward_features(self, x):
+    def forward_features(self, x, pe_weight=None):
         self._predraw_drop_path(x.shape[0], x.device)
         ops.clear_twins()
-        x = self.stage1_conv_embed(x)
+        x = self.stage1_conv_embed(x, pe_weight)
         if self.pos_drop.p > 0 and self.training:
             x = ops.dropout(x, self.pos_drop.p)
         x = self._run(self.stage1, x)
@@ -308,18 +313,26 @@
         side = _square_side(x.shape[1])
         ncls = head.out_channels
         cpad = max(16, 1 << (ncls - 1).bit_length())
-        w_head = head.weight.flatten(1)
-        w_fused = ops.matmul_nn(w_head, up.out.weight.flatten(1))
-        b_fused = ops.linear(up.out.bias[None, :], w_head)[0]
-        w_fused = nn.functional.pad(w_fused, (0, 0, 0, cpad - ncls))
-        b_fused = nn.functional.pad(b_fused, (0, cpad - ncls))
+        w_fused, b_fused = ops.head_compose(head.weight, up.out.weight, up.out.bias, cpad)
         mid, z = ops.linear_pair(x, up.down.weight.flatten(1), up.down.bias, w_fused, None)
         e = ops.conv_tokens(mid, up.encoder.weight, up.encoder.bias, side, side, 1, 1)
-        tok = ops.carafe_reassemble(e, z, b_fused, side, side, up.up_factor)
-        return ops.tokens_to_nchw(tok, ncls, up.up_factor * side, up.up_factor * side)
+        return ops.carafe_reassemble_nchw(e, z, b_fused, side, side, up.up_factor, ncls)
+
+    def _conv_specs(self, pe_weight):
+        pe = self.stage1_conv_embed[0]
+        specs = [(pe_weight, (pe_weight.shape[1] + 3) // 4 * 4, pe.stride[0], pe.padding[0])]
+        specs += [(m.conv.weight, m.conv.weight.shape[1], 2, 1) for m in (self.merge1, self.merge2, self.merge3)]
+        specs += [(u.encoder.weight, u.encoder.weight.shape[1], 1, 1)
+                  for u in (self.upsample4, self.upsample3, self.upsample2, self.upsample1)]
+        return specs
 
     def forward(self, x):
-        x = self.forward_features(x)
+        pe_weight = self.stage1_conv_embed.conv_weight(x)
+        with ops.conv_weight_images(self._conv_specs(pe_weight)):
+            return self._forward(x, pe_weight)
+
+    def _forward(self, x, pe_weight):
+        x = self.forward_features(x, pe_weight)
         self.xb = x
         bound = [x, self.x1, self.x2, self.x3]
         if getattr(self, "detach_decoder_inputs", False) and torch.is_grad_enabled():
diff --git a/cswin_unet_amd/ops.py b/cswin_unet_amd/ops.py
--- a/cswin_unet_amd/ops.py
+++ b/cswin_unet_amd/ops.py
@@ -5,10 +5,10 @@
 from torch.autograd import Function
 from torch.autograd.function import once_differentiable
 
-from ._lib import CswinHipError, ReduceJob, WgradDesc, act_bf16, call, dev_f32, lib, precision, ptr, shadow_ptr, stream
+from ._lib import ConvImageJob, CswinHipError, ReduceJob, WgradDesc, act_bf16, call, dev_f32, lib, precision, ptr, shadow_ptr, stream
 
 __all__ = ["layer_norm", "linear", "linear_pair", "mlp", "stripe_attention", "cswin_block", "conv_tokens", "patch_embed_conv", "carafe_reassemble",
-           "tokens_to_nchw", "matmul_nn", "ce_dice_loss", "dropout", "img2windows", "windows2img"]
+           "carafe_reassemble_nchw", "conv_weight_images", "head_compose", "tokens_to_nchw", "matmul_nn", "ce_dice_loss", "dropout", "img2windows", "windows2img"]
 
 
 MAX_REDUCE_JOBS = 48
@@ -585,6 +585,54 @@
                              norm2.bias, fc1.weight, fc1.bias, fc2.weight, fc2.bias, *lepe_w, *lepe_b)
 
 
+MAX_CONV_IMAGE_JOBS = 16
+_conv_images = {}
+
+
+def _same_conv(w, stride, pad):
+    return stride == 1 and 2 * pad == w.shape[2] - 1 and w.shape[0] % 4 == 0
+
+
+class conv_weight_images:
+
+    def __init__(self, specs):
+        self._specs = [sp for sp in specs if sp[0] is not None and sp[0].is_cuda and sp[0].dtype == torch.float32 and sp[0].is_contiguous()]
+
+    def __enter__(self):
+        global _conv_images
+        self._outer = _conv_images
+        images, jobs = {}, []
+        grad = torch.is_grad_enabled()
+        for w, cpad, stride, pad in self._specs[:MAX_CONV_IMAGE_JOBS]:
+            Cout, Cin, ks, _ = w.shape
+            E = lambda *shape: torch.empty(*shape, dtype=torch.float32, device=w.device)
+            same = _same_conv(w, stride, pad)
+            need_dx = grad and cpad == Cin
+            wp = E(Cout, ks * ks, cpad)
+            wpt = E(ks * ks, Cout, cpad) if need_dx and not same else None
+            wf = E(Cin, ks * ks, Cout) if need_dx and same else None
+            images[w.data_ptr()] = (w, cpad, wp, wpt, wf)
+            jobs.append(ConvImageJob(w.data_ptr(), wp.data_ptr(), wpt.data_ptr() if wpt is not None else None,
+                                     wf.data_ptr() if wf is not None else None, Cout, Cin, ks, cpad))
+        if jobs:
+            arr = (ConvImageJob * len(jobs))(*jobs)
+            call("cswin_conv_weight_images", ctypes.cast(arr, ctypes.c_void_p), len(jobs), stream())
+        _conv_images = images
+        return self
+
+    def __exit__(self, *exc):
+        global _conv_images
+        _conv_images = self._outer
+        return False
+
+
+def _images_of(w, cpad):
+    e = _conv_images.get(w.data_ptr())
+    if e is not None and e[0].shape == w.shape and e[1] == cpad:
+        return e[2:]
+    return None
+
+
 def _permute_w(w, cpad, want_t):
     Cout, Cin, ks, _ = w.shape
     wp = torch.empty(Cout, ks * ks, cpad, dtype=torch.float32, device=w.device)
@@ -602,11 +650,16 @@
         Cout, ks = w.shape[0], w.shape[2]
         OH, OW = (H + 2 * pad - ks) // stride + 1, (W + 2 * pad - ks) // stride + 1
         need_dx = ctx.needs_input_grad[0]
-        same = stride == 1 and 2 * pad == ks - 1 and Cout % 4 == 0
-        wp, wpt = _permute_w(w, Cin, need_dx and not same)
+        same = _same_conv(w, stride, pad)
+        img = _images_of(w, Cin)
+        wf = None
+        if img is not None and (img[1] is not None or same or not need_dx):
+            wp, wpt, wf = img
+        else:
+            wp, wpt = _permute_w(w, Cin, need_dx and not same)
         y = torch.empty(B, OH * OW, Cout, dtype=torch.float32, device=x.device)
         call("cswin_conv_tok_fwd", ptr(x), ptr(wp), ptr(b), ptr(y), B, H, W, Cin, Cout, ks, stride, pad, precision(), stream())
-        ctx.save_for_backward(x, w, wpt)
+        ctx.save_for_backward(x, w, wpt, wf if need_dx else None)
         ctx.meta = (H, W, stride, pad, b is not None)
         ctx.keys = _param_keys(w, b)
         return y
@@ -614,7 +667,7 @@
     @staticmethod
     @once_differentiable
     def backward(ctx, dy):
-        x, w, wpt = ctx.saved_tensors
+        x, w, wpt, wf = ctx.saved_tensors
         H, W, stride, pad, has_b = ctx.meta
         dy = dev_f32(dy)
         B, L, Cin = x.shape
@@ -623,9 +676,10 @@
         dx = None
         if ctx.needs_input_grad[0]:
             dx = torch.empty_like(x)
-            if stride == 1 and 2 * pad == ks - 1 and Cout % 4 == 0:
-                wf = torch.empty(Cin, ks * ks, Cout, dtype=torch.float32, device=x.device)
-                call("cswin_conv_weight_flipT", ptr(w), ptr(wf), Cout, Cin, ks, st)
+            if _same_conv(w, stride, pad):
+                if wf is None:
+                    wf = torch.empty(Cin, ks * ks, Cout, dtype=torch.float32, device=x.device)
+                    call("cswin_conv_weight_flipT", ptr(w), ptr(wf), Cout, Cin, ks, st)
                 call("cswin_conv_tok_fwd", ptr(dy), ptr(wf), None, ptr(dx), B, H, W, Cout, Cin, ks, 1, pad, precision(), st)
             else:
                 if wpt is None:
@@ -657,7 +711,8 @@
         st = stream()
         x = torch.empty(B, H * W, cpad, dtype=torch.float32, device=img.device)
         call("cswin_nchw_to_tokens", ptr(img), ptr(x), B, Cin, H, W, cpad, st)
-        wp, _ = _permute_w(w, cpad, False)
+        images = _images_of(w, cpad)
+        wp = images[0] if images is not None else _permute_w(w, cpad, False)[0]
         OH, OW = (H + 2 * pad - ks) // stride + 1, (W + 2 * pad - ks) // stride + 1
         y = torch.empty(B, OH * OW, Cout, dtype=torch.float32, device=img.device)
         call("cswin_conv_tok_fwd", ptr(x), ptr(wp), ptr(b), ptr(y), B, H, W, cpad, Cout, ks, stride, pad, precision(), st)
@@ -675,14 +730,14 @@
         B = x.shape[0]
         Cout, Cin, ks, _ = w.shape
         st = stream()
-        dwp = torch.empty(Cout, ks * ks, cpad, dtype=torch.float32, device=x.device)
+        dw = _pass.grad(ctx.keys[0], w.shape, x.device)
         db = _pass.grad(ctx.keys[1], (Cout,), x.device) if has_b else None
         nbytes = lib().cswin_conv_tok_bwd_weight_workspace(B, H, W, cpad, Cout, ks, stride, pad)
         ws = _ws(nbytes, x.device)
-        call("cswin_conv_tok_bwd_weight", ptr(dy), ptr(x), ptr(dwp), ptr(db), ptr(ws), nbytes, B, H, W, cpad, Cout, ks, stride,
-             pad, 0, None, precision(), st)
-        dw = _pass.grad(ctx.keys[0], w.shape, x.device)
-        call("cswin_conv_weight_unpermute", ptr(dwp), ptr(dw), Cout, Cin, ks, cpad, st)
+        job = (ReduceJob * 1)()
+        call("cswin_conv_tok_bwd_weight_cpad", ptr(dy), ptr(x), ptr(dw), ptr(db), ptr(ws), nbytes, B, H, W, cpad, Cin, Cout, ks,
+             stride, pad, _job_ptr(job), precision(), st)
+        _pass.reduce(job, (ws,))
         return None, dw, db, None, None
 
 
@@ -725,6 +780,82 @@
 
 def carafe_reassemble(e, z, bias, H, W, S):
     return _CarafeReassemble.apply(e, z, bias, H, W, S)
+
+
+class _CarafeReassembleNchw(Function):
+
+    @staticmethod
+    def forward(ctx, e, z, bias, H, W, S, C):
+        e, z, bias = dev_f32(e, "carafe kernel logits"), dev_f32(z, "carafe features"), dev_f32(bias)
+        B, L, Cz = z.shape
+        assert L == H * W and e.shape == (B, L, 9 * S * S) and 0 < C <= Cz
+        out = torch.empty(B, C, S * H, S * W, dtype=torch.float32, device=z.device)
+        wt = torch.empty_like(e)
+        call("cswin_carafe_fwd_nchw", ptr(e), ptr(z), ptr(bias), ptr(out), ptr(wt), B, H, W, Cz, C, S, stream())
+        ctx.save_for_backward(z, wt)
+        ctx.meta = (H, W, S, C, bias is not None)
+        ctx.keys = _param_keys(bias)
+        return out
+
+    @staticmethod
+    @once_differentiable
+    def backward(ctx, dout):
+        z, wt = ctx.saved_tensors
+        H, W, S, C, has_b = ctx.meta
+        dout = dev_f32(dout)
+        B, L, Cz = z.shape
+        de = torch.empty_like(wt)
+        dz = torch.empty_like(z)
+        db = _pass.grad(ctx.keys[0], (Cz,), z.device) if has_b else None
+        nbytes = lib().cswin_carafe_bwd_workspace(B, H, W, Cz, S)
+        ws = _ws(nbytes, z.device)
+        job = (ReduceJob * 1)()
+        call("cswin_carafe_bwd_nchw", ptr(dout), ptr(z), ptr(wt), ptr(de), ptr(dz), ptr(db), ptr(ws), nbytes, B, H, W, Cz, C, S,
+             _job_ptr(job), stream())
+        _pass.reduce(job, (ws,))
+        return de, dz, db, None, None, None, None
+
+
+def carafe_reassemble_nchw(e, z, bias, H, W, S, C):
+    if lib().cswin_carafe_bwd_nchw_ok(H, W, z.shape[-1], S):
+        return _CarafeReassembleNchw.apply(e, z, bias, H, W, S, C)
+    return tokens_to_nchw(carafe_reassemble(e, z, bias, H, W, S), C, S * H, S * W)
+
+
+class _HeadCompose(Function):
+
+    @staticmethod
+    def forward(ctx, w_head, w_out, b_out, cpad):
+        w_head, w_out, b_out = dev_f32(w_head, "head weight"), dev_f32(w_out, "out weight"), dev_f32(b_out)
+        ncls, E = w_head.shape[0], w_head.numel() // w_head.shape[0]
+        C = w_out.numel() // w_out.shape[0]
+        assert w_out.shape[0] == E and cpad >= ncls and (b_out is None or b_out.numel() == E)
+        wf = torch.empty(cpad, C, dtype=torch.float32, device=w_head.device)
+        bf = torch.empty(cpad, dtype=torch.float32, device=w_head.device)
+        call("cswin_head_compose", ptr(w_head), ptr(w_out), ptr(b_out), ptr(wf), ptr(bf), ncls, E, C, cpad, stream())
+        ctx.save_for_backward(w_head, w_out, b_out)
+        ctx.keys = _param_keys(w_head, w_out, b_out)
+        return wf, bf
+
+    @staticmethod
+    @once_differentiable
+    def backward(ctx, dwf, dbf):
+        w_head, w_out, b_out = ctx.saved_tensors
+        ncls, E = w_head.shape[0], w_head.numel() // w_head.shape[0]
+        C = w_out.numel() // w_out.shape[0]
+        dev = w_head.device
+        dwf = dev_f32(dwf) if dwf is not None else torch.zeros(ncls, C, dtype=torch.float32, device=dev)
+        dbf = dev_f32(dbf)
+        dwh = _pass.grad(ctx.keys[0], w_head.shape, dev)
+        dwo = _pass.grad(ctx.keys[1], w_out.shape, dev)
+        dbo = _pass.grad(ctx.keys[2], b_out.shape, dev) if b_out is not None else None
+        call("cswin_head_compose_bwd", ptr(w_head), ptr(w_out), ptr(b_out), ptr(dwf), ptr(dbf), ptr(dwh), ptr(dwo), ptr(dbo),
+             ncls, E, C, stream())
+        return dwh, dwo, dbo, None
+
+
+def head_compose(w_head, w_out, b_out, cpad):
+    return _HeadCompose.apply(w_head, w_out, b_out, int(cpad))
 
 
 class _TokensToNchw(Function):
diff --git a/include/cswin_hip.h b/include/cswin_hip.h
--- a/include/cswin_hip.h
+++ b/include/cswin_hip.h
@@ -89,6 +89,17 @@
                               void* stream);
 int cswin_conv_weight_unpermute(const float* dw_perm, float* dw, int Cout, int Cin, int ks, int Cpad, void* stream);
 int cswin_conv_weight_flipT(const float* w, float* wf, int Cout, int Cin, int ks, void* stream);
+typedef struct cswin_conv_image_job {
+    const float* w;
+    float* w_perm;
+    float* w_permT;
+    float* w_flipT;
+    int Cout, Cin, ks, Cpad;
+} cswin_conv_image_job;
+int cswin_conv_weight_images(const cswin_conv_image_job* jobs, int njobs, void* stream);
+int cswin_conv_tok_bwd_weight_cpad(const float* dy, const float* x, float* dw, float* dbias, void* workspace, size_t ws_bytes,
+                                   int B, int H, int W, int Cin, int Cin_param, int Cout, int ks, int stride, int pad,
+                                   cswin_reduce_job* deferred, int precision, void* stream);
 
 int cswin_nchw_to_tokens(const float* x, float* y, int B, int C, int H, int W, int Cpad, void* stream);
 int cswin_tokens_to_nchw(const float* x, float* y, int B, int C, int H, int W, int Cpad, void* stream);
@@ -98,6 +109,18 @@
 size_t cswin_carafe_bwd_workspace(int B, int H, int W, int Cz, int S);
 int cswin_carafe_bwd(const float* dout, const float* z, const float* wt_save, float* de, float* dz, float* dbias,
                      void* workspace, size_t ws_bytes, int B, int H, int W, int Cz, int S, cswin_reduce_job* deferred, void* stream);
+int cswin_carafe_fwd_nchw(const float* e, const float* z, const float* bias, float* out, float* wt_save, int B, int H, int W,
+                          int Cz, int C, int S, void* stream);
+int cswin_carafe_bwd_nchw_ok(int H, int W, int Cz, int S);
+int cswin_carafe_bwd_nchw(const float* dout, const float* z, const float* wt_save, float* de, float* dz, float* dbias,
+                          void* workspace, size_t ws_bytes, int B, int H, int W, int Cz, int C, int S, cswin_reduce_job* deferred,
+                          void* stream);
+
+int cswin_head_compose(const float* w_head, const float* w_out, const float* b_out, float* w_fused, float* b_fused, int ncls,
+                       int E, int C, int Cpad, void* stream);
+int cswin_head_compose_bwd(const float* w_head, const float* w_out, const float* b_out, const float* dw_fused,
+                           const float* db_fused, float* dw_head, float* dw_out, float* db_out, int ncls, int E, int C,
+                           void* stream);
 
 size_t cswin_loss_workspace(int B, int ncls, long HW);
 int cswin_loss_sums(const float* logits, const long long* labels, float* sums, void* workspace, size_t ws_bytes, int B,
```

Result: faster. 1912 images/sec (median of 6 runs) (+1.5%).
